# scheck-k/ste-gan

Measured on NVIDIA B200. Metric: GAN train samples/s, higher is better.
Workload: dtype bf16

## Files before the change

### include/stegan_b200.h

```cpp
#ifndef STEGAN_B200_H_
#define STEGAN_B200_H_

#include <stdint.h>

#ifdef __cplusplus
extern "C" {
#endif

typedef void* stg_stream_t;

enum { STG_F32 = 0, STG_BF16 = 1 };
enum { STG_ACT_NONE = 0, STG_ACT_RELU = 1, STG_ACT_LEAKY = 2, STG_ACT_TANH = 3 };
enum {
  STG_OK = 0,
  STG_EINVAL = -1,
  STG_ECUDA = -2,
  STG_EUNSUPPORTED = -3
};
enum { STG_ENGINE_AUTO = 0, STG_ENGINE_SIMT = 1, STG_ENGINE_TCGEN05 = 2, STG_ENGINE_MATVEC = 3  };

#define STG_MAX_TAPS 48

typedef struct StgConv {
  int32_t dtype;
  int32_t engine;
  int32_t n_samples;
  int32_t phases;
  int32_t t_src;
  int32_t t_dst;
  int32_t c_src;
  int32_t c_dst;
  int32_t groups;
  int32_t k, dilation, stride, pad;
  int32_t transposed;
  int32_t pair_sum;
  int32_t post_shift;
  int32_t mask_mode;
  int32_t act;
  int32_t dup_rows;
  int32_t out_f32;
  int32_t w_fwd_pack;
  const void* src;
  const void* w;
  const float* bias;
  const void* add_pre;
  const void* mask;
  const void* add_post;
  void* y_raw;
  void* y_act;
} StgConv;

int stg_conv(const StgConv* d, stg_stream_t stream);

int stg_conv_masked(const StgConv* d, const int32_t* valid_units, int32_t rows_per_unit, stg_stream_t stream);

typedef struct StgWgrad {
  int32_t dtype, engine;
  int32_t n_samples, phases, t_in, t_out, c_in, c_out, groups, k, dilation, stride, pad;
  const void* x;
  const void* dy;
  float* dw;
  float* dbias;
} StgWgrad;

int stg_conv_wgrad(const StgWgrad* d, stg_stream_t stream);
int stg_wgrad_layout(const StgWgrad* d, int* ld, int* span);

enum { STG_PACK_UNFOLD = 1 };
int stg_weightnorm_fold(const float* v, const float* g, int c_out, int cin_g, int k, int groups, int pack_groups,
                        int flags, int dtype, void* wf, void* wd, float* scale, stg_stream_t stream);
int stg_weightnorm_fold_bwd(const float* dw, int dw_ld, int dw_span, const float* v, const float* g, int c_out, int cin_g,
                            int k, int groups, float* dv, float* dg, int accumulate, stg_stream_t stream);

int stg_spectralnorm_fold(const float* w_orig, float* u, float* v, int c_out, int cin_g, int k, int groups,
                          int pack_groups, int flags, int training, int dtype, void* wf, void* wd, float* sigma_out,
                          float* scratch, float* u_used, float* v_used, stg_stream_t stream);
int stg_spectralnorm_fold_bwd(const float* dw, int dw_ld, int dw_span, const float* w_orig, const float* u, const float* v,
                              const float* sigma, int c_out, int cin_g, int k, int groups, float* dw_orig, int accumulate,
                              float* scratch, stg_stream_t stream);
typedef struct StgFoldItem {
  const float* v;
  const float* g;
  void* wf;
  void* wd;
  float* scale;
  const float* dw;
  float* dv;
  float* dg;
  int32_t c_out, cin_g, k, groups, pg, flags, dw_ld, dw_span;
  int32_t row0, tile0;
} StgFoldItem;
int stg_weightnorm_fold_multi(const StgFoldItem* items, int n_items, int total_rows, int total_tiles, int dtype,
                              stg_stream_t stream);
int stg_weightnorm_fold_bwd_multi(const StgFoldItem* items, int n_items, int total_rows, int accumulate,
                                  stg_stream_t stream);
int stg_weightnorm_fold_bwd_range(const StgFoldItem* items, int n_items, int row_base, int n_rows, int accumulate,
                                  stg_stream_t stream);

int stg_tc_pack_groups(int c_in, int c_out, int groups);

int stg_unfold(const void* src, int dtype, int B, int phases, int t_src, int t_dst, int C, int k, int dilation, int stride,
               int pad, void* out, stg_stream_t stream);
int stg_unfold_bwd(const void* dout, int dtype, int B, int phases, int t_src, int t_dst, int C, int k, int dilation,
                   int stride, int pad, float* dsrc, stg_stream_t stream);

int stg_period_first_layer(const float* x, const void* wf, const float* bias, int B, int T, int C, int period, int c_out,
                           int k, int stride, int pad, float slope, void* y, stg_stream_t stream);

int stg_embed_concat(const float* units, const float* emb, const int64_t* ids, int B, int T, int d_units, int d_emb,
                     int dtype, void* x0, stg_stream_t stream);
int stg_embed_concat_bwd(const void* dx0, const int64_t* ids, int B, int T, int d_units, int d_emb, int dtype,
                         float* demb, stg_stream_t stream);

int stg_reflect_pad_right(const float* x, int B, int T, int C, int T_pad, int dtype, void* out, stg_stream_t stream);
int stg_reflect_pad_right_bwd(const void* dout, int B, int T, int C, int T_pad, int dtype, float* dx, stg_stream_t stream);
int stg_avgpool4(const float* x, int B, int T, int C, float* out, stg_stream_t stream);
int stg_avgpool4_bwd(const float* dout, int B, int T, int C, float* dx, stg_stream_t stream);
int stg_cast(const void* src, int src_dtype, void* dst, int dst_dtype, int64_t n, stg_stream_t stream);
int stg_act_bwd(const float* dy, const float* y, int mode, int64_t n, int dtype, void* out, stg_stream_t stream);
int stg_relu_rows(const void* src, int dtype, int64_t rows, int C, int dup, void* out, stg_stream_t stream);
int stg_pair_sum_rows(const void* in, int64_t rows_out, int C, int dtype, void* out, stg_stream_t stream);
int stg_axpy_f32(float* y, const void* x, int x_dtype, float alpha, int64_t n, stg_stream_t stream);

int stg_td_loss(const float* x_real, const float* x_gen, int B, int T, int C, float* losses, const float* grad_scale,
                float* dx_gen, float* scratch, stg_stream_t stream);
int stg_td_loss_ex(const float* x_real, const float* x_gen, int B, int T, int C, int n_res, const int* wins,
                   const int* shifts, int pad_windows, int avg_window, float* losses, const float* grad_scale,
                   const float* grad_scale_dev, float* dx_gen, float* scratch, stg_stream_t stream);
int stg_td_features(const float* x, int B, int T, int C, int win, int shift, int pad_windows, int avg_window,
                    float* feats, float* scratch, stg_stream_t stream);
int stg_frame_stats(const float* x, int B, int T, int C, int win, int shift, int pad_windows, float* mean, float* power,
                    stg_stream_t stream);
int stg_window_signal(const float* x, int B, int T, int C, int win, int shift, int pad_windows, float* out,
                      stg_stream_t stream);
int stg_average_filter(const float* x, int64_t rows, int T, int window, int pad, float* out, stg_stream_t stream);

// ... 64 lines not shown
```

### ste_gan_b200/_lib.py

```python
from __future__ import annotations

import ctypes as C
import os

_HERE = os.path.dirname(os.path.abspath(__file__))
LIB_PATH = os.path.join(_HERE, "libstegan_b200.so")

F32, BF16 = 0, 1
ACT_NONE, ACT_RELU, ACT_LEAKY, ACT_TANH = 0, 1, 2, 3
ENGINE_AUTO, ENGINE_SIMT, ENGINE_TCGEN05 = 0, 1, 2
PACK_UNFOLD = 1
MAX_TAPS = 48


class StgConv(C.Structure):
    _fields_ = [(n, C.c_int32) for n in (
        "dtype", "engine", "n_samples", "phases", "t_src", "t_dst", "c_src", "c_dst", "groups", "k", "dilation",
        "stride", "pad", "transposed", "pair_sum", "post_shift", "mask_mode", "act", "dup_rows", "out_f32", "w_fwd_pack")] + [
        (n, C.c_void_p) for n in ("src", "w", "bias", "add_pre", "mask", "add_post", "y_raw", "y_act")]


class StgWgrad(C.Structure):
    _fields_ = [(n, C.c_int32) for n in (
        "dtype", "engine", "n_samples", "phases", "t_in", "t_out", "c_in", "c_out", "groups", "k", "dilation",
        "stride", "pad")] + [(n, C.c_void_p) for n in ("x", "dy", "dw", "dbias")]


class StgFoldItem(C.Structure):
    _fields_ = [(n, C.c_void_p) for n in ("v", "g", "wf", "wd", "scale", "dw", "dv", "dg")] + [
        (n, C.c_int32) for n in ("c_out", "cin_g", "k", "groups", "pg", "flags", "dw_ld", "dw_span", "row0", "tile0")]


class StgL1Item(C.Structure):
    _fields_ = [("a", C.c_void_p), ("b", C.c_void_p), ("da", C.c_void_p), ("n", C.c_int64)]


class StgMseItem(C.Structure):
    _fields_ = [("x", C.c_void_p), ("dx", C.c_void_p), ("n", C.c_int64), ("target", C.c_float), ("slot", C.c_int32)]


MAX_LOSS_ITEMS = 32
_P, _I, _L, _F = C.c_void_p, C.c_int, C.c_int64, C.c_float
_SIGS = {
    "stg_conv": [C.POINTER(StgConv), _P],
    "stg_conv_masked": [C.POINTER(StgConv), _P, C.c_int32, _P],
    "stg_conv_wgrad": [C.POINTER(StgWgrad), _P],
    "stg_conv_tc_supported": [C.POINTER(StgConv)],
    "stg_conv_route": [C.POINTER(StgConv)],
    "stg_wgrad_route": [C.POINTER(StgWgrad)],
    "stg_wgrad_tc_supported": [C.POINTER(StgWgrad)],
    "stg_weightnorm_fold": [_P, _P, _I, _I, _I, _I, _I, _I, _I, _P, _P, _P, _P],
    "stg_weightnorm_fold_bwd": [_P, _I, _I, _P, _P, _I, _I, _I, _I, _P, _P, _I, _P],
    "stg_wgrad_layout": [C.POINTER(StgWgrad), C.POINTER(C.c_int), C.POINTER(C.c_int)],
    "stg_spectralnorm_fold": [_P, _P, _P, _I, _I, _I, _I, _I, _I, _I, _I, _P, _P, _P, _P, _P, _P, _P],
    "stg_spectralnorm_fold_bwd": [_P, _I, _I, _P, _P, _P, _P, _I, _I, _I, _I, _P, _I, _P, _P],
    "stg_tc_pack_groups": [_I, _I, _I],
    "stg_l1_mean_multi": [_P, _I, _I, _P, _F, _P],
    "stg_mse_const_multi": [_P, _I, _I, _I, _P, _F, _P],
    "stg_weightnorm_fold_multi": [_P, _I, _I, _I, _I, _P],
    "stg_weightnorm_fold_bwd_multi": [_P, _I, _I, _I, _P],
    "stg_weightnorm_fold_bwd_range": [_P, _I, _I, _I, _I, _P],
    "stg_debug_set_trace": [_P],
    "stg_debug_rowshift": [_P, _P, _I, _I, _I, _P, _P],
    "stg_debug_row_classes": [_I, _P],
    "stg_debug_group_mma": [_P, _P, _I, _I, _P, _P],
    "stg_debug_conv_plan": [_P, _P],
    "stg_debug_tma_bw": [_P, C.c_longlong, _I, _I, _I, _I, _I, _P, _P],
    "stg_unfold": [_P, _I, _I, _I, _I, _I, _I, _I, _I, _I, _I, _P, _P],
    "stg_unfold_bwd": [_P, _I, _I, _I, _I, _I, _I, _I, _I, _I, _I, _P, _P],
    "stg_period_first_layer": [_P, _P, _P, _I, _I, _I, _I, _I, _I, _I, _I, C.c_float, _P, _P],
    "stg_embed_concat": [_P, _P, _P, _I, _I, _I, _I, _I, _P, _P],
    "stg_embed_concat_bwd": [_P, _P, _I, _I, _I, _I, _I, _P, _P],
    "stg_reflect_pad_right": [_P, _I, _I, _I, _I, _I, _P, _P],
    "stg_reflect_pad_right_bwd": [_P, _I, _I, _I, _I, _I, _P, _P],
    "stg_avgpool4": [_P, _I, _I, _I, _P, _P],
    "stg_avgpool4_bwd": [_P, _I, _I, _I, _P, _P],
    "stg_cast": [_P, _I, _P, _I, _L, _P],
    "stg_act_bwd": [_P, _P, _I, _L, _I, _P, _P],
    "stg_pair_sum_rows": [_P, _L, _I, _I, _P, _P],
    "stg_relu_rows": [_P, _I, _L, _I, _I, _P, _P],
    "stg_axpy_f32": [_P, _P, _I, _F, _L, _P],
    "stg_td_loss": [_P, _P, _I, _I, _I, _P, C.POINTER(C.c_float), _P, _P, _P],
    "stg_td_loss_ex": [_P, _P, _I, _I, _I, _I, C.POINTER(C.c_int), C.POINTER(C.c_int), _I, _I, _P, C.POINTER(C.c_float), _P, _P, _P, _P],
    "stg_td_features": [_P, _I, _I, _I, _I, _I, _I, _I, _P, _P, _P],
    "stg_frame_stats": [_P, _I, _I, _I, _I, _I, _I, _P, _P, _P],
    "stg_window_signal": [_P, _I, _I, _I, _I, _I, _I, _P, _P],
    "stg_average_filter": [_P, _L, _I, _I, _I, _P, _P],
    "stg_mse_const": [_P, _I, _L, _F, _P, _F, _P, _I, _P],
    "stg_l1_mean": [_P, _P, _I, _L, _P, _F, _P, _P],
    "stg_layernorm_fwd": [_P, _I, _P, _P, _I, _I, _F, _P, _P, _P],
    "stg_layernorm_bwd": [_P, _P, _I, _P, _P, _I, _I, _P, _P],
    "stg_relattn_fwd": [_P, _I, _P, _I, _I, _I, _I, _I, _F, _P, _P, _P],
    "stg_relattn_bwd": [_P, _I, _P, _P, _P, _I, _I, _I, _I, _I, _F, _P, _P],
    "stg_relattn_dense_supported": [_I, _I, _I],
    "stg_relattn_band_fwd": [_P, _I, _P, _I, _I, _I, _I, _I, _F, _P, _P, _P],
    "stg_relattn_band_bwd": [_P, _I, _P, _P, _P, _I, _I, _I, _I, _I, _F, _P, _P, _P],
    "stg_relattn_fwd_masked": [_P, _I, _P, _I, _I, _I, _I, _I, _F, _P, _P, _P, _P],
    "stg_relattn_band_fwd_masked": [_P, _I, _P, _I, _I, _I, _I, _I, _F, _P, _P, _P, _P],
    "stg_encoder_losses": [_P, _P, _P, _P, _I, _I, _I, _P, _F, _F, _P, _P, _I, _P],
    "stg_encoder_scores": [_P, _P, _P, _P, _P, _I, _I, _I, _I, _I, _P, _P, _P],
    "stg_adamw": [_P, _P, _P, _P, _L, _F, _P, _F, _F, _F, _F, _P, _F, _P, _I, _P],
}
EXPORTS = sorted(list(_SIGS) + ["stg_strerror", "stg_last_cuda_error", "stg_version", "stg_launch_count", "stg_set_sm_limit",
                                   "stg_debug_ingest_bytes"])

_lib = None


class StgError(RuntimeError):
    pass


def load(build_if_missing: bool = True):
    global _lib
    if _lib is not None:
        return _lib
    if not os.path.exists(LIB_PATH):
        if not build_if_missing:
            raise StgError(f"{LIB_PATH} is missing; run `python -m ste_gan_b200.build`")
        from . import build as _b
        _b.build()
    import torch
    lib = C.CDLL(LIB_PATH, mode=C.RTLD_GLOBAL)
    for name, argtypes in _SIGS.items():
        fn = getattr(lib, name)
        fn.argtypes = argtypes
        fn.restype = C.c_int
    lib.stg_strerror.argtypes = [C.c_int]
# ... 23 lines not shown
```

### ste_gan_b200/csrc/api.cu

```cuda
#include <stdlib.h>
#include <string.h>

#include <string>

#include "common.cuh"

namespace stg {

static thread_local std::string g_last_error;
unsigned long long g_launch_count = 0;
double g_ingest_bytes = 0.0;
int g_sm_limit = getenv("STG_SM_LIMIT") ? atoi(getenv("STG_SM_LIMIT")) : 0;

void set_cuda_error(cudaError_t e, const char* where) {
  g_last_error = std::string(cudaGetErrorName(e)) + ": " + cudaGetErrorString(e) + " at " + where;
}

int colsum(const void* dy, int dtype, int64_t rows, int C, float* out, cudaStream_t s);

static int validate_conv(const StgConv* d) {
  if (!d || !d->src || !d->w) return STG_EINVAL;
  if (d->dtype != STG_F32 && d->dtype != STG_BF16) return STG_EINVAL;
  if (d->n_samples < 1 || d->phases < 1 || d->t_src < 1 || d->t_dst < 1) return STG_EINVAL;
  if (d->groups < 1 || d->c_src % d->groups || d->c_dst % d->groups) return STG_EINVAL;
  if (d->k < 1 || d->dilation < 1 || d->stride < 1 || d->pad < 0) return STG_EINVAL;
  if (d->post_shift < 0 || d->post_shift > 1) return STG_EINVAL;
  if (d->dup_rows && d->pair_sum) return STG_EINVAL;
  if (!d->y_raw && !d->y_act) return STG_EINVAL;
  if (d->w_fwd_pack && !d->transposed) return STG_EINVAL;
  return STG_OK;
}

}

using namespace stg;

extern "C" int stg_conv(const StgConv* d, stg_stream_t stream) {
  int r = validate_conv(d);
  if (r) return r;
  cudaStream_t s = static_cast<cudaStream_t>(stream);
  switch (d->engine) {
    case STG_ENGINE_SIMT: return d->w_fwd_pack ? STG_EUNSUPPORTED : conv_simt(d, s);
    case STG_ENGINE_TCGEN05: return conv_tc(d, s);
    case STG_ENGINE_AUTO:
      if (conv_c1_supported(d)) return conv_c1(d, s);
      if (conv_tc_supported(d)) return conv_tc(d, s);
      return d->w_fwd_pack ? STG_EUNSUPPORTED : conv_simt(d, s);
    default: return STG_EINVAL;
  }
}

extern "C" int stg_conv_masked(const StgConv* d, const int32_t* valid_units, int32_t rows_per_unit, stg_stream_t stream) {
  int r = validate_conv(d);
  if (r) return r;
  if (!valid_units || rows_per_unit < 1 || d->transposed || d->pair_sum || d->phases != 1) return STG_EINVAL;
  cudaStream_t s = static_cast<cudaStream_t>(stream);
  switch (d->engine) {
    case STG_ENGINE_SIMT: return conv_simt(d, s, valid_units, rows_per_unit);
    case STG_ENGINE_TCGEN05: return conv_tc(d, s, valid_units, rows_per_unit);
    case STG_ENGINE_AUTO:
      return conv_tc_supported(d) ? conv_tc(d, s, valid_units, rows_per_unit) : conv_simt(d, s, valid_units, rows_per_unit);
    default: return STG_EINVAL;
  }
}

extern "C" int stg_conv_route(const StgConv* d) {
  if (!d || validate_conv(d) != STG_OK) return STG_EINVAL;
  if (d->engine == STG_ENGINE_SIMT) return STG_ENGINE_SIMT;
  if (d->engine == STG_ENGINE_TCGEN05) return STG_ENGINE_TCGEN05;
  if (conv_c1_supported(d)) return STG_ENGINE_MATVEC;
  return conv_tc_supported(d) ? STG_ENGINE_TCGEN05 : STG_ENGINE_SIMT;
}
extern "C" int stg_wgrad_route(const StgWgrad* d) {
  if (!d) return STG_EINVAL;
  if (d->engine == STG_ENGINE_SIMT) return STG_ENGINE_SIMT;
  if (d->engine == STG_ENGINE_TCGEN05) return STG_ENGINE_TCGEN05;
  if (wgrad_c1_supported(d)) return STG_ENGINE_MATVEC;
  return wgrad_tc_supported(d) ? STG_ENGINE_TCGEN05 : STG_ENGINE_SIMT;
}
extern "C" int stg_conv_tc_supported(const StgConv* d) { return (d && validate_conv(d) == STG_OK && conv_tc_supported(d)) ? 1 : 0; }
extern "C" int stg_tc_pack_groups(int c_in, int c_out, int groups) {
  if (groups < 1 || c_in % groups || c_out % groups) return groups;
  return tc_pack_groups(c_in, c_out, groups);
}
extern "C" int stg_wgrad_tc_supported(const StgWgrad* d) { return (d && wgrad_tc_supported(d)) ? 1 : 0; }

extern "C" int stg_conv_wgrad(const StgWgrad* d, stg_stream_t stream) {
  if (!d || !d->x || !d->dy) return STG_EINVAL;
  if (d->dtype != STG_F32 && d->dtype != STG_BF16) return STG_EINVAL;
  if (d->groups < 1 || d->c_in % d->groups || d->c_out % d->groups) return STG_EINVAL;
  cudaStream_t s = static_cast<cudaStream_t>(stream);
  int r = STG_OK;
  if (d->dw) {
    if (d->engine == STG_ENGINE_AUTO && wgrad_c1_supported(d)) return wgrad_c1(d, s);
    if (d->engine == STG_ENGINE_TCGEN05) return wgrad_tc(d, s);
    if (d->engine == STG_ENGINE_AUTO && wgrad_tc_supported(d)) return wgrad_tc(d, s);
    if (d->engine == STG_ENGINE_AUTO || d->engine == STG_ENGINE_SIMT) r = wgrad_simt(d, s);
    else r = STG_EINVAL;
    if (r) return r;
  }
  if (d->dbias) r = colsum(d->dy, d->dtype, (int64_t)d->n_samples * d->phases * d->t_out, d->c_out, d->dbias, s);
  return r;
}

extern "C" int stg_wgrad_layout(const StgWgrad* d, int* ld, int* span) {
  if (!d || !ld || !span || d->groups < 1 || d->c_in % d->groups) return STG_EINVAL;
  const bool tc = d->engine == STG_ENGINE_TCGEN05 ||
                  (d->engine == STG_ENGINE_AUTO && !wgrad_c1_supported(d) && wgrad_tc_supported(d));
  if (tc) { wgrad_tc_layout(d, ld, span); return STG_OK; }
  *span = d->c_in / d->groups;
  *ld = d->k * *span;
  return STG_OK;
}

extern "C" const char* stg_strerror(int code) {
  switch (code) {
    case STG_OK: return "ok";
    case STG_EINVAL: return "invalid argument or unsupported shape";
    case STG_ECUDA: return "CUDA error";
    case STG_EUNSUPPORTED: return "shape not supported by the requested engine";
    default: return "unknown error";
  }
}
extern "C" const char* stg_last_cuda_error(void) { return g_last_error.c_str(); }
extern "C" int stg_version(void) { return 100; }
extern "C" unsigned long long stg_launch_count(void) { return g_launch_count; }
extern "C" void stg_set_sm_limit(int n) { g_sm_limit = n > 0 ? n : 0; }
extern "C" double stg_debug_ingest_bytes(int reset) { const double v = g_ingest_bytes; if (reset) g_ingest_bytes = 0.0; return v; }

extern "C" int stg_debug_conv_plan(const StgConv* d, int* out) {
  if (!out) return STG_EINVAL;
  const int r = validate_conv(d);
  if (r != STG_OK) return r;
  return conv_tc_plan(d, out);
}

extern "C" int stg_debug_set_trace(void* buf) { conv_tc_set_trace(static_cast<long long*>(buf)); return STG_OK; }
```

### ste_gan_b200/csrc/common.cuh

```cuda
#pragma once
#include <cuda_bf16.h>
#include <cuda_runtime.h>
#include <stdint.h>

#include "../../include/stegan_b200.h"

namespace stg {

void set_cuda_error(cudaError_t e, const char* where);

#define STG_CUDA_CHECK(expr)                                   \
  do {                                                         \
    cudaError_t _e = (expr);                                   \
    if (_e != cudaSuccess) {                                   \
      ::stg::set_cuda_error(_e, #expr);                        \
      return STG_ECUDA;                                        \
    }                                                          \
  } while (0)

extern unsigned long long g_launch_count;
extern double g_ingest_bytes;
extern int g_sm_limit;
#define STG_LAUNCH_CHECK()                 \
  do {                                     \
    ++::stg::g_launch_count;               \
    STG_CUDA_CHECK(cudaGetLastError());    \
  } while (0)

using bf16 = __nv_bfloat16;

__device__ __forceinline__ float to_f(float v) { return v; }
__device__ __forceinline__ float to_f(bf16 v) { return __bfloat162float(v); }
template <typename T> __device__ __forceinline__ T from_f(float v);
template <> __device__ __forceinline__ float from_f<float>(float v) { return v; }
template <> __device__ __forceinline__ bf16 from_f<bf16>(float v) { return __float2bfloat16_rn(v); }

__device__ __forceinline__ void ld4(const float* p, float (&o)[4]) {
  float4 v = *reinterpret_cast<const float4*>(p);
  o[0] = v.x; o[1] = v.y; o[2] = v.z; o[3] = v.w;
}
__device__ __forceinline__ void ld4(const bf16* p, float (&o)[4]) {
  uint2 v = *reinterpret_cast<const uint2*>(p);
  __nv_bfloat162 a = *reinterpret_cast<__nv_bfloat162*>(&v.x);
  __nv_bfloat162 b = *reinterpret_cast<__nv_bfloat162*>(&v.y);
  o[0] = __low2float(a); o[1] = __high2float(a); o[2] = __low2float(b); o[3] = __high2float(b);
}
__device__ __forceinline__ void st4(float* p, const float (&v)[4]) {
  *reinterpret_cast<float4*>(p) = make_float4(v[0], v[1], v[2], v[3]);
}
__device__ __forceinline__ void st4(bf16* p, const float (&v)[4]) {
  __nv_bfloat162 a = __floats2bfloat162_rn(v[0], v[1]);
  __nv_bfloat162 b = __floats2bfloat162_rn(v[2], v[3]);
  uint2 u;
  u.x = *reinterpret_cast<uint32_t*>(&a);
  u.y = *reinterpret_cast<uint32_t*>(&b);
  *reinterpret_cast<uint2*>(p) = u;
}

__device__ __forceinline__ float act_apply(int act, float v) {
  switch (act) {
    case STG_ACT_RELU: return v > 0.f ? v : 0.f;
    case STG_ACT_LEAKY: return v > 0.f ? v : 0.1f * v;
    case STG_ACT_TANH: return tanhf(v);
    default: return v;
  }
}
__device__ __forceinline__ float act_grad_from_output(int mode, float m) {
  switch (mode) {
    case STG_ACT_RELU: return m > 0.f ? 1.f : 0.f;
    case STG_ACT_LEAKY: return m > 0.f ? 1.f : 0.1f;
    case STG_ACT_TANH: return 1.f - m * m;
    default: return 1.f;
  }
}

__device__ __forceinline__ float warp_sum(float v) {
#pragma unroll
  for (int o = 16; o > 0; o >>= 1) v += __shfl_xor_sync(0xffffffffu, v, o);
  return v;
}
__device__ __forceinline__ float block_sum(float v, float* red) {
  const int lane = threadIdx.x & 31, warp = threadIdx.x >> 5, nw = (blockDim.x + 31) >> 5;
  v = warp_sum(v);
  __syncthreads();
  if (lane == 0) red[warp] = v;
  __syncthreads();
  float r = (lane < nw) ? red[lane] : 0.f;
  r = warp_sum(r);
  return r;
}

static inline int64_t ceil_div64(int64_t a, int64_t b) { return (a + b - 1) / b; }
static inline int ceil_div(int a, int b) { return (a + b - 1) / b; }

int conv_simt(const StgConv* d, cudaStream_t s, const int32_t* valid_units = nullptr, int rows_per_unit = 1);
int conv_tc(const StgConv* d, cudaStream_t s, const int32_t* valid_units = nullptr, int rows_per_unit = 1);
int conv_tc_plan(const StgConv* d, int* out);
bool conv_tc_supported(const StgConv* d);
int wgrad_simt(const StgWgrad* d, cudaStream_t s);
int wgrad_tc(const StgWgrad* d, cudaStream_t s);
bool wgrad_tc_supported(const StgWgrad* d);
int tc_pack_groups(int c_in, int c_out, int groups);
bool conv_c1_supported(const StgConv* d);
int conv_c1(const StgConv* d, cudaStream_t s);
bool wgrad_c1_supported(const StgWgrad* d);
int wgrad_c1(const StgWgrad* d, cudaStream_t s);
void conv_tc_set_trace(long long* buf);
void wgrad_tc_layout(const StgWgrad* d, int* ld, int* span);

}
```

### ste_gan_b200/csrc/conv_tc.cu

```cuda
#include <stdio.h>
#include <stdlib.h>
#include <string.h>

#include "tc_common.cuh"

namespace stg {

namespace {

using namespace tc;

constexpr int TM = 128;
constexpr int KC = 64;
constexpr int MAX_STAGES = 8;
constexpr int ACC_COLS = 256;
constexpr int SUB = 32;
constexpr int SLOT = TM * SUB * 2;
constexpr int MAX_RES = 8;

struct TcEpi {
  int rows, c_dst, post_shift, mask_mode, act, dup_rows, out_f32, pair_sum;
  int n_in, n_out, has_pre, has_mask, has_post, has_raw, has_act;
  int in_sh;
  float act_slope, mask_slope;
// ... 140 lines not shown
  x.col0 = tn * p.bn;
  x.ch0 = (x.col0 / p.cd_g) * p.cs_g;
  x.wcol0 = x.col0 % p.cd_g;
  x.g0 = p.res_gfirst[x.res];
  x.n_iters = (p.res_gfirst[x.res + 1] - x.g0) * p.k_chunks;
  return x;
}
__device__ __forceinline__ int out_row(const TcP& p, const Tile& x, int m) {
  if (m >= p.mrows || x.b >= p.n_samples) return -1;
  const int hl = m / p.pack, ph = m - hl * p.pack;
  const int h = (x.h0 + hl) * p.n_res + x.res;
  return h < p.t_dst ? h * p.phases + ph : -1;
}

__device__ __forceinline__ bool row_kept(const TcEpi& e, int b, int row) {
  return (int64_t)row < (int64_t)max(e.valid_units[b], 0) * e.rows_per_unit;
}

struct EpiIn {
  float pre[16], mk[16], post[16];
};
__device__ __forceinline__ void epi_load(const TcEpi& e, int b, int row, int col, bool row_ok, EpiIn& in) {
  if (!row_ok || col >= e.c_dst) return;
  const int ncols = min(16, e.c_dst - col);
  const bool vec = (ncols == 16) && ((e.c_dst & 7) == 0);
  const int64_t off = ((int64_t)b * e.rows + row) * e.c_dst + col;
  if (e.add_pre) {
    if (vec) ld16(e.add_pre + off, in.pre); else for (int i = 0; i < 16; ++i) in.pre[i] = i < ncols ? to_f(e.add_pre[off + i]) : 0.f;
  }
  if (e.mask) {
    if (vec) ld16(e.mask + off, in.mk); else for (int i = 0; i < 16; ++i) in.mk[i] = i < ncols ? to_f(e.mask[off + i]) : 0.f;
  }
  if (e.add_post) {
    const int64_t o2 = ((int64_t)b * (e.rows >> e.post_shift) + (row >> e.post_shift)) * e.c_dst + col;
    if (vec) ld16(e.add_post + o2, in.post); else for (int i = 0; i < 16; ++i) in.post[i] = i < ncols ? to_f(e.add_post[o2 + i]) : 0.f;
  }
}
__device__ __forceinline__ void epi_store(const TcEpi& e, int b, int row, int col, float (&v)[16], const EpiIn& in, bool keep) {
  const int64_t off = ((int64_t)b * e.rows + row) * e.c_dst + col;
  const int ncols = min(16, e.c_dst - col);
  const bool vec = (ncols == 16) && ((e.c_dst & 7) == 0);
  if (e.add_pre) {
#pragma unroll
    for (int i = 0; i < 16; ++i) v[i] += in.pre[i];
  }
  if (e.mask) {
#pragma unroll
    for (int i = 0; i < 16; ++i) v[i] *= dact_fast(e, in.mk[i]);
  }
  if (e.add_post) {
#pragma unroll
    for (int i = 0; i < 16; ++i) v[i] += in.post[i];
  }
  if (!keep) {
#pragma unroll
    for (int i = 0; i < 16; ++i) v[i] = 0.f;
  }
  if (e.y_raw) {
    if (e.out_f32) {
      float* p = static_cast<float*>(e.y_raw) + off;
      if (vec) st16f(p, v); else for (int i = 0; i < ncols; ++i) p[i] = v[i];
    } else {
      bf16* p = static_cast<bf16*>(e.y_raw) + off;
      if (vec) st16(p, v); else for (int i = 0; i < ncols; ++i) p[i] = __float2bfloat16_rn(v[i]);
    }
  }
  if (e.y_act) {
    float a[16];
#pragma unroll
    for (int i = 0; i < 16; ++i) a[i] = act_fast(e, v[i]);
    const int64_t o0 = e.dup_rows ? ((int64_t)b * 2 * e.rows + 2 * row) * e.c_dst + col : off;
    if (e.out_f32) {
      float* p0 = static_cast<float*>(e.y_act) + o0;
      if (vec) st16f(p0, a); else for (int i = 0; i < ncols; ++i) p0[i] = a[i];
      if (e.dup_rows) { float* p1 = p0 + e.c_dst; if (vec) st16f(p1, a); else for (int i = 0; i < ncols; ++i) p1[i] = a[i]; }
    } else {
      bf16* p0 = static_cast<bf16*>(e.y_act) + o0;
      if (vec) st16(p0, a); else for (int i = 0; i < ncols; ++i) p0[i] = __float2bfloat16_rn(a[i]);
      if (e.dup_rows) { bf16* p1 = p0 + e.c_dst; if (vec) st16(p1, a); else for (int i = 0; i < ncols; ++i) p1[i] = __float2bfloat16_rn(a[i]); }
    }
  }
}

template <bool kStaged, bool kPair, bool kMask>
__global__ void __launch_bounds__(kStaged ? 384 : 352, (kStaged && !kPair) ? 2 : 1)
conv_tc_kernel(const __grid_constant__ TmA4 tmA4, const __grid_constant__ CUtensorMap tmW,
               const __grid_constant__ EpiMaps em, const TcP p) {
  constexpr int EPI_WARPS = 8;
  extern __shared__ uint8_t smem_raw[];
  const uint32_t smem_base = (smem_u32(smem_raw) + 1023u) & ~1023u;
  const int b_bytes = p.cu_k ? p.cu_fpc * p.cu_n * p.cu_k * 2 : (kPair ? p.bn / 2 : p.bn) * KC * 2;
  const int stage_bytes = p.a_bytes + p.max_ntaps * b_bytes;
  const TcEpi& e = p.e;
  const int rank = kPair ? __shfl_sync(0xffffffffu, (int)cluster_ctarank(), 0) : 0;
  const int tile0 = kPair ? (int)(blockIdx.x >> 1) : (int)blockIdx.x;
  const int tstep = kPair ? (int)(gridDim.x >> 1) : (int)gridDim.x;
  const uint32_t epi_base = smem_base + p.stages * stage_bytes;
  const uint32_t bias_base = epi_base + (kStaged ? ((e.n_in << e.in_sh) + p.out_ring * e.n_out) * SLOT : 0);
  const uint32_t bar_base = bias_base + (kStaged ? 2048 : 0);
  auto full_bar = [&](int s) { return bar_base + 8u * s; };
  auto empty_bar = [&](int s) { return bar_base + 8u * (MAX_STAGES + s); };
  auto tmem_full_bar = [&](int a) { return bar_base + 8u * (2 * MAX_STAGES + a); };
  auto tmem_empty_bar = [&](int a) { return bar_base + 8u * (2 * MAX_STAGES + 2 + a); };
  const uint32_t tmem_slot = bar_base + 8u * (2 * MAX_STAGES + 4);
  auto in_bar = [&](int a) { return bar_base + 8u * (2 * MAX_STAGES + 6 + a); };

  const int warp = __shfl_sync(0xffffffffu, (int)(threadIdx.x >> 5), 0), lane = threadIdx.x & 31;

  life_ev(p.trace, 30);
  pdl_trigger();
  if (warp == 0 && lane == 0) {
    for (int c = 0; c < p.n_cls; ++c) prefetch_tmap(&tmA4.m[c]);
    prefetch_tmap(&tmW);
    for (int s = 0; s < p.stages; ++s) { mbar_init(full_bar(s), 1); mbar_init(empty_bar(s), 1); }
    for (int a = 0; a < 2; ++a) { mbar_init(tmem_full_bar(a), 1); mbar_init(tmem_empty_bar(a), kPair ? 2 * EPI_WARPS : EPI_WARPS); }
    for (int a = 0; a < 8; ++a) mbar_init(in_bar(a), 1);
    fence_barrier_init();
  }
  if (warp == 1) {
    if constexpr (kPair) { tmem_alloc_2sm(tmem_slot, (uint32_t)p.tmem_cols); tmem_relinquish_2sm(); }
    else { tmem_alloc(tmem_slot, (uint32_t)p.tmem_cols); tmem_relinquish(); }
  }
  tc_fence_before();
  if constexpr (kPair) cluster_sync_all();
  else __syncthreads();
  tc_fence_after();
  life_ev(p.trace, 31);
  pdl_wait();
  life_ev(p.trace, 32);
  uint32_t tmem_base;
  asm volatile("ld.shared.b32 %0, [%1];" : "=r"(tmem_base) : "r"(tmem_slot));
  const uint32_t lead_bars = kPair ? mapa_u32(bar_base, 0) : bar_base;
  auto lead_full_bar = [&](int s) { return lead_bars + 8u * s; };
  auto lead_tmem_empty_bar = [&](int a) { return lead_bars + 8u * (2 * MAX_STAGES + 2 + a); };
  auto arrive_tmem_empty = [&](int a) {
    if constexpr (kPair) mbar_arrive_cluster(lead_tmem_empty_bar(a)); else mbar_arrive(tmem_empty_bar(a));
  };

  constexpr int WPROD = kStaged ? 11 : 10;
  if ((warp == 0 || warp == WPROD) && p.max_ntaps == 1) {
    const bool do_a = warp == 0;
    const bool lead = lane == 0;
    Tracer trc(lead && do_a ? p.trace : nullptr, 0);
    const uint32_t a_box_bytes = (uint32_t)(p.hb * p.pack * KC * 2);
    const uint32_t tx_bytes = (kPair ? 2u : 1u) * ((uint32_t)p.a_boxes * a_box_bytes + (uint32_t)b_bytes);
    const int row_step = p.hb * p.stride;
    int s = 0; uint32_t phs = 0;
#ifdef STG_PROF_LOOP
    long long prof[4] = {0, 0, 0, 0};
#endif
    for (int t = tile0; t < p.n_tiles; t += tstep) {
      const Tile x = decode_tile<kPair>(p, t, rank);
      trc.ev(1, t);
      const int n_groups = p.res_gfirst[x.res + 1] - x.g0;
      const int wc = p.b_mn == 0 ? x.col0 + (kPair ? rank * (p.bn / 2) : 0)
                   : p.b_mn == 2 ? x.wcol0 / 64 + (kPair ? rank * (p.bn / 128) : 0) : x.wcol0;
      for (int gi = 0; gi < n_groups; ++gi) {
        const int g = x.g0 + gi;
        const int row0 = x.h0 * p.stride + p.tt.g_off[g];
        const int tap = p.tt.tap_w[g];
        for (int chunk = 0; chunk < p.k_chunks; ++chunk) {
#ifdef STG_PROF_LOOP
          const long long pc0 = clock64();
#endif
          mbar_wait(empty_bar(s), phs ^ 1);
          trc.ev(4, chunk);
#ifdef STG_PROF_LOOP
          const long long pc1 = clock64();
#endif
          const uint32_t a_dst = smem_base + (uint32_t)(s * stage_bytes);
          const uint32_t fb = kPair ? lead_full_bar(s) : full_bar(s);
          const int c0 = x.ch0 + chunk * KC;
          if (do_a) {
            if (rank == 0) mbar_expect_tx_el(full_bar(s), tx_bytes);
#pragma unroll 1
            for (int bx = 0; bx < p.a_boxes; ++bx)
              tma_load_4d_el<kPair>(a_dst + bx * a_box_bytes, &tmA4.m[x.cls], fb, c0, 0, row0 + bx * row_step, x.b);
          }
#ifdef STG_PROF_LOOP
          const long long pc2 = clock64();
#endif
          if (do_a) {
          } else if (p.cu_k) {
            tma_load_3d_el<kPair>(a_dst + p.a_bytes, &tmW, fb, 0, x.col0 + chunk * p.cu_fpc * p.cu_n, tap);
          } else if (p.b_mn == 0) {
            tma_load_3d_el<kPair>(a_dst + p.a_bytes, &tmW, fb, chunk * KC, wc, tap);
          } else if (p.b_mn == 2) {
            tma_load_4d_el<kPair>(a_dst + p.a_bytes, &tmW, fb, 0, c0, wc, tap);
          } else {
#pragma unroll 1
            for (int nb = 0; nb < p.bn / 64; ++nb)
              tma_load_3d_el<kPair>(a_dst + p.a_bytes + nb * 8192, &tmW, fb, wc + nb * 64, c0, tap);
          }
          if (++s == p.stages) { s = 0; phs ^= 1u; }
#ifdef STG_PROF_LOOP
          const long long pc3 = clock64();
          prof[0] += pc1 - pc0; prof[1] += pc2 - pc1; prof[2] += pc3 - pc2; prof[3] += 1;
#endif
        }
      }
    }
#ifdef STG_PROF_LOOP
    if (lead && do_a && p.trace && blockIdx.x == 0) for (int i = 0; i < 4; ++i) p.trace[1 + 3 * 5200 + i] = prof[i];
#endif
  } else if (warp == 1 && p.max_ntaps == 1) {
    const bool lead = lane == 0;
    const uint32_t idesc = idesc_bf16_f32(kPair ? 2 * TM : TM, p.bn, 0, p.b_mn ? 1 : 0);
    const uint32_t idesc_u = idesc_bf16_f32(TM, p.cu_k ? p.cu_n : p.bn, 0, 0);
    const int cu_ks = p.cu_k == 16 ? 0 : (p.cu_k == 32 ? 1 : 2), cu_km = (1 << cu_ks) - 1;
    const uint64_t cu_bhi = smem_desc_kmajor_narrow(0, p.cu_k ? p.cu_k * 2 : 128);
    const int cu_bq = (p.cu_n * p.cu_k * 2) >> 4;
    Tracer trc(lead ? p.trace : nullptr, 1);
    const uint64_t adesc0 = smem_desc_kmajor_sw128(smem_base);
    const uint64_t bdesc0 = p.b_mn ? smem_desc_mnmajor_sw128(smem_base + p.a_bytes, 8192, 1024) : smem_desc_kmajor_sw128(smem_base + p.a_bytes);
    const uint32_t dstep = (uint32_t)stage_bytes >> 4;
    const uint32_t bstep = p.b_mn ? 128u : 2u;
    int s = 0, acc_i = 0; uint32_t phs = 0;
#ifdef STG_PROF_LOOP
    long long mprof[3] = {0, 0, 0};
#endif
    for (int t = tile0; t < p.n_tiles && rank == 0; t += tstep) {
      const Tile x = decode_tile<kPair>(p, t, rank);
      if (x.n_iters == 0) continue;
      const int as = acc_i & 1, aph = (acc_i >> 1) & 1;
      mbar_wait(tmem_empty_bar(as), aph ^ 1);
      tc_fence_after();
      trc.ev(2, t);
      const uint32_t d_tmem = tmem_base + (uint32_t)(as * p.acc_cols);
      int cu_chunk = 0;
      for (int it = 0; it < x.n_iters; ++it) {
#ifdef STG_PROF_LOOP
        const long long mc0 = clock64();
#endif
        mbar_wait(full_bar(s), phs);
        tc_fence_after();
        trc.ev(5, it);
#ifdef STG_PROF_LOOP
        const long long mc1 = clock64();
#endif
        const uint64_t ad = adesc0 + (uint64_t)((uint32_t)s * dstep), bd = bdesc0 + (uint64_t)((uint32_t)s * dstep);
        if (p.cu_k) {
          const uint32_t dcol = d_tmem + (uint32_t)(cu_chunk * p.cu_fpc * p.cu_n);
          if (++cu_chunk == p.k_chunks) cu_chunk = 0;
          const uint64_t bu = cu_bhi | (uint64_t)(((smem_base + (uint32_t)(s * stage_bytes) + (uint32_t)p.a_bytes) >> 4) & 0x3FFFu);
          const uint32_t acc0 = it >= p.k_chunks ? 1u : 0u;
#pragma unroll
          for (int i = 0; i < KC / 16; ++i) {
            const int q = i >> cu_ks, ks = i & cu_km;
            umma_bf16_el<kPair>(dcol + (uint32_t)(q * p.cu_n), ad + 2 * i, bu + (uint64_t)(q * cu_bq + 2 * ks), idesc_u, (acc0 | (uint32_t)(ks > 0)));
          }
        } else {
#pragma unroll
          for (int ks = 0; ks < KC / 16; ++ks)
            umma_bf16_el<kPair>(d_tmem, ad + 2 * ks, bd + bstep * ks, idesc, (it > 0 || ks > 0) ? 1u : 0u);
        }
        umma_commit_el<kPair>(empty_bar(s));
        if (it == x.n_iters - 1) umma_commit_el<kPair>(tmem_full_bar(as));
        if (++s == p.stages) { s = 0; phs ^= 1u; }
#ifdef STG_PROF_LOOP
        const long long mc2 = clock64();
        mprof[0] += mc1 - mc0; mprof[1] += mc2 - mc1; mprof[2] += 1;
#endif
      }
      trc.ev(3, t);
      ++acc_i;
    }
#ifdef STG_PROF_LOOP
    if (lead && p.trace && blockIdx.x == 0) for (int i = 0; i < 3; ++i) p.trace[1 + 3 * 5200 + 8 + i] = mprof[i];
#endif
  } else if (warp == 0 || warp == WPROD) {
    const bool do_a = warp == 0;
    int s = 0; uint32_t phs = 0;
    for (int t = tile0; t < p.n_tiles; t += tstep) {
      const Tile x = decode_tile<kPair>(p, t, rank);
      const int n_groups = p.res_gfirst[x.res + 1] - x.g0;
      for (int gi = 0; gi < n_groups; ++gi) {
       const int g = x.g0 + gi;
       const int nt = p.tt.g_ntaps[g], t0 = p.tt.g_tfirst[g];
       for (int chunk = 0; chunk < p.k_chunks; ++chunk) {
        mbar_wait(empty_bar(s), phs ^ 1);
        const uint32_t a_dst = smem_base + s * stage_bytes;
        if (do_a) {
          mbar_expect_tx_el(full_bar(s), (uint32_t)(p.a_boxes * p.hb * p.pack * KC * 2 + nt * b_bytes));
#pragma unroll 1
          for (int bx = 0; bx < p.a_boxes; ++bx)
            tma_load_4d_el(a_dst + bx * p.hb * p.pack * KC * 2, &tmA4.m[0], full_bar(s), x.ch0 + chunk * KC, 0,
                           (x.h0 + bx * p.hb) * p.stride + p.tt.g_off[g], x.b);
        }
#pragma unroll 1
        for (int tl = 0; tl < (do_a ? 0 : nt); ++tl) {
          if (p.cu_k) {
            tma_load_3d_el(a_dst + p.a_bytes + tl * b_bytes, &tmW, full_bar(s), 0, x.col0 + chunk * p.cu_fpc * p.cu_n,
                           p.tt.tap_w[t0 + tl]);
          } else if (!p.b_mn) {
            tma_load_3d_el(a_dst + p.a_bytes + tl * b_bytes, &tmW, full_bar(s), chunk * KC, x.col0, p.tt.tap_w[t0 + tl]);
          } else if (p.b_mn == 2) {
            tma_load_4d_el(a_dst + p.a_bytes + tl * b_bytes, &tmW, full_bar(s), 0, x.ch0 + chunk * KC, x.wcol0 / 64,
                           p.tt.tap_w[t0 + tl]);
          } else {
#pragma unroll 1
            for (int nb = 0; nb < p.bn / 64; ++nb)
              tma_load_3d_el(a_dst + p.a_bytes + tl * b_bytes + nb * 8192, &tmW, full_bar(s), x.wcol0 + nb * 64,
                             x.ch0 + chunk * KC, p.tt.tap_w[t0 + tl]);
          }
        }
        if (++s == p.stages) { s = 0; phs ^= 1u; }
       }
      }
    }
  } else if (warp == 1) {
    const uint32_t idesc = idesc_bf16_f32(TM, p.bn, 0, p.b_mn ? 1 : 0);
    const uint32_t idesc_u = idesc_bf16_f32(TM, p.cu_k ? p.cu_n : p.bn, 0, 0);
    const int cu_ks = p.cu_k == 16 ? 0 : (p.cu_k == 32 ? 1 : 2), cu_km = (1 << cu_ks) - 1;
    const uint64_t cu_bhi = smem_desc_kmajor_narrow(0, p.cu_k ? p.cu_k * 2 : 128);
    const int cu_bq = (p.cu_n * p.cu_k * 2) >> 4;
    int s = 0, acc_i = 0; uint32_t phs = 0;
    for (int t = tile0; t < p.n_tiles; t += tstep) {
      const Tile x = decode_tile<kPair>(p, t, rank);
      if (x.n_iters == 0) continue;
      const int as = acc_i & 1, aph = (acc_i >> 1) & 1;
      mbar_wait(tmem_empty_bar(as), aph ^ 1);
      tc_fence_after();
      const uint32_t d_tmem = tmem_base + (uint32_t)(as * p.acc_cols);
      int g = x.g0, chunk = 0;
      for (int it = 0; it < x.n_iters; ++it) {
        const int nt = p.tt.g_ntaps[g], t0 = p.tt.g_tfirst[g];
        mbar_wait(full_bar(s), phs);
        tc_fence_after();
        const uint32_t a_addr = smem_base + s * stage_bytes;
#pragma unroll 1
        for (int tl = 0; tl < nt; ++tl) {
          const uint64_t adesc = smem_desc_kmajor_sw128(a_addr + (uint32_t)(p.tt.tap_shift[t0 + tl] * p.pack * KC * 2));
          const uint32_t b_addr = a_addr + p.a_bytes + tl * b_bytes;
          if (p.cu_k) {
            const uint32_t dcol = d_tmem + (uint32_t)(chunk * p.cu_fpc * p.cu_n);
            const uint64_t bu = cu_bhi | (uint64_t)((b_addr >> 4) & 0x3FFFu);
            const uint32_t acc0 = (it >= p.k_chunks || tl > 0) ? 1u : 0u;
#pragma unroll
            for (int i = 0; i < KC / 16; ++i) {
              const int q = i >> cu_ks, ks = i & cu_km;
              umma_bf16_el(dcol + (uint32_t)(q * p.cu_n), adesc + 2 * i, bu + (uint64_t)(q * cu_bq + 2 * ks), idesc_u, (acc0 | (uint32_t)(ks > 0)));
            }
            continue;
          }
          const uint64_t bdesc = p.b_mn ? smem_desc_mnmajor_sw128(b_addr, 8192, 1024) : smem_desc_kmajor_sw128(b_addr);
          const uint64_t bstep = p.b_mn ? 128 : 2;
#pragma unroll
          for (int ks = 0; ks < KC / 16; ++ks)
            umma_bf16_el(d_tmem, adesc + 2 * ks, bdesc + bstep * ks, idesc, (it > 0 || tl > 0 || ks > 0) ? 1u : 0u);
        }
        umma_commit_el(empty_bar(s));
        if (it == x.n_iters - 1) umma_commit_el(tmem_full_bar(as));
        if (++s == p.stages) { s = 0; phs ^= 1u; }
        if (++chunk == p.k_chunks) { chunk = 0; ++g; }
      }
      ++acc_i;
    }
  } else if constexpr (kStaged) {
    const int n_sub = p.bn / SUB;
    const int in_mask = (1 << e.in_sh) - 1;
    auto ring = [&](int q) { return p.out_ring == 2 ? (q & 1) : q % 3; };
    auto in_slot = [&](int buf, int i) { return epi_base + (uint32_t)((buf * e.n_in + i) * SLOT); };
    auto out_slot = [&](int buf, int o) { return epi_base + (uint32_t)(((e.n_in << e.in_sh) + buf * e.n_out + o) * SLOT); };
    auto bar_full = [&](int b3) { return 2 + b3; };
    auto bar_free = [&](int b3) { return 5 + b3; };
    const int my_tiles = (p.n_tiles - tile0 + tstep - 1) / tstep;
    const int q_total = my_tiles * n_sub;
    if (warp == 10) {
      if (lane == 0) {
// ... 173 lines not shown
#pragma unroll
              for (int i = 0; i < 32; ++i) v[i] = fmaxf(v[i], e.act_slope * v[i]);
#pragma unroll
              for (int j = 0; j < 4; ++j) sts128(sl + sw64(r_in, j), pack8(&v[8 * j]));
            }
          }
          fence_proxy_async();
          asm volatile("bar.arrive %0, 160;" ::"r"(bar_full(obuf)) : "memory");
          trc.ev(12, s);
        }
        qbase += n_sub;
        if (x.n_iters > 0) ++acc_i;
      }
    }
  } else {
    const int ew = warp - 2;
    const int sub = warp & 3;
    const int half = ew >> 2;
    const int n_chunks = p.bn / 16;
    const int c_lo = (half == 0) ? 0 : (n_chunks + 1) / 2, c_hi = (half == 0) ? (n_chunks + 1) / 2 : n_chunks;
    int acc_i = 0;
    for (int t = tile0; t < p.n_tiles; t += tstep) {
      const Tile x = decode_tile<kPair>(p, t, rank);
      const int as = acc_i & 1, aph = (acc_i >> 1) & 1;
      const int arow = out_row(p, x, sub * 32 + lane);
      const bool row_ok = arow >= 0 && (!e.pair_sum || (lane & 1) == 0);
      const int orow = e.pair_sum ? (arow >> 1) : arow;
      const bool keep = !kMask || (row_ok && row_kept(e, x.b, orow));
      EpiIn inA, inB;
      if (c_lo < c_hi) epi_load(e, x.b, orow, x.col0 + c_lo * 16, row_ok, inA);
      if (x.n_iters > 0) {
        mbar_wait(tmem_full_bar(as), aph);
        tc_fence_after();
      }
      const uint32_t t_addr = tmem_base + ((uint32_t)(sub * 32) << 16) + (uint32_t)(as * p.acc_cols);
      auto process = [&](int c, const EpiIn& in) {
        float v[16];
        if (x.n_iters > 0) {
          tmem_ld16(t_addr + (uint32_t)(c * 16), v);
        } else {
#pragma unroll
          for (int i = 0; i < 16; ++i) v[i] = 0.f;
        }
        const int col = x.col0 + c * 16;
        if (col >= e.c_dst) return;
        if (e.bias) {
#pragma unroll
          for (int i = 0; i < 16; ++i) v[i] += (col + i < e.c_dst) ? e.bias[col + i] : 0.f;
        }
        if (e.pair_sum) {
#pragma unroll
          for (int i = 0; i < 16; ++i) v[i] += __shfl_xor_sync(0xffffffffu, v[i], 1);
        }
        if (row_ok) epi_store(e, x.b, orow, col, v, in, keep);
      };
#pragma unroll 1
      for (int c = c_lo; c < c_hi; c += 2) {
        if (c + 1 < c_hi) epi_load(e, x.b, orow, x.col0 + (c + 1) * 16, row_ok, inB);
        process(c, inA);
        if (c + 1 < c_hi) {
          if (c + 2 < c_hi) epi_load(e, x.b, orow, x.col0 + (c + 2) * 16, row_ok, inA);
          process(c + 1, inB);
        }
      }
      if (x.n_iters > 0) {
        tc_fence_before();
        __syncwarp();
        if (lane == 0) arrive_tmem_empty(as);
        ++acc_i;
      }
    }
  }
  tc_fence_before();
  if constexpr (kPair) {
    cluster_sync_all();
    if (warp == 1) tmem_dealloc_2sm(tmem_base, (uint32_t)p.tmem_cols);
  } else {
    __syncthreads();
    if (warp == 1) tmem_dealloc(tmem_base, (uint32_t)p.tmem_cols);
  }
  life_ev(p.trace, 33);
}

}

PFN_encodeTiled get_encode_tiled() {
  static PFN_encodeTiled fn = nullptr;
  if (!fn) {
    void* ptr = nullptr;
    cudaDriverEntryPointQueryResult q;
    if (cudaGetDriverEntryPoint("cuTensorMapEncodeTiled", &ptr, cudaEnableDefault, &q) == cudaSuccess &&
        q == cudaDriverEntryPointSuccess)
      fn = reinterpret_cast<PFN_encodeTiled>(ptr);
  }
  return fn;
}

int make_tmap_bf16(CUtensorMap* out, const void* base, int rank, const uint64_t* dims, const uint64_t* strides_bytes,
                   const uint32_t* box, const uint32_t* elem_strides, int swizzle_bytes) {
  PFN_encodeTiled enc = get_encode_tiled();
  if (!enc) { set_cuda_error(cudaErrorNotSupported, "cuTensorMapEncodeTiled entry point"); return STG_ECUDA; }
  cuuint64_t gd[5]; cuuint64_t gs[4]; cuuint32_t bx[5]; cuuint32_t es[5];
  for (int i = 0; i < rank; ++i) { gd[i] = dims[i]; bx[i] = box[i]; es[i] = elem_strides ? elem_strides[i] : 1; }
  for (int i = 0; i + 1 < rank; ++i) gs[i] = strides_bytes[i];
  const CUtensorMapSwizzle sw = swizzle_bytes == 32 ? CU_TENSOR_MAP_SWIZZLE_32B
                              : swizzle_bytes == 64 ? CU_TENSOR_MAP_SWIZZLE_64B : CU_TENSOR_MAP_SWIZZLE_128B;
  CUresult r = enc(out, CU_TENSOR_MAP_DATA_TYPE_BFLOAT16, (cuuint32_t)rank, const_cast<void*>(base), gd, gs, bx, es,
                   CU_TENSOR_MAP_INTERLEAVE_NONE, sw, CU_TENSOR_MAP_L2_PROMOTION_L2_256B,
                   CU_TENSOR_MAP_FLOAT_OOB_FILL_NONE);
  if (r != CUDA_SUCCESS) {
    set_cuda_error(cudaErrorInvalidValue, "cuTensorMapEncodeTiled failed");
    return STG_ECUDA;
  }
  return STG_OK;
}

static int sm_count() {
  static int n = 0;
  if (!n) {
    int dev = 0;
    if (cudaGetDevice(&dev) != cudaSuccess || cudaDeviceGetAttribute(&n, cudaDevAttrMultiProcessorCount, dev) != cudaSuccess || n < 1)
      n = 148;
  }
  return (g_sm_limit > 0 && g_sm_limit < n) ? g_sm_limit : n;
}

static int pick_bn_model(int cd_g, int groups, int64_t row_tiles, int n_stages, int step) {
  static const double feed = getenv("STG_BN_FEED") ? atof(getenv("STG_BN_FEED")) : 0.0;
  static const double alpha = getenv("STG_BN_ALPHA") ? atof(getenv("STG_BN_ALPHA")) : 0.0;
  int best = 0;
  double best_t = 0;
  for (int bn = 256; bn >= step; bn -= step) {
    if (cd_g % bn) continue;
    const int64_t tiles = row_tiles * (cd_g / bn) * groups;
    const double waves = (double)((tiles + sm_count() - 1) / sm_count());
    double mma = 2.0 * bn > 200.0 ? 2.0 * bn : 200.0;
    if (feed > 0.0) { const double ld = (TM * KC * 2 + bn * KC * 2) / feed; if (ld > mma) mma = ld; }
    const double stage = mma + 60.0;
    const double epi = (bn / 32.0) * 200.0;
    const double makespan = waves * n_stages * stage + epi;
    const double smtime = (double)tiles * (n_stages * stage + epi) / sm_count();
    const double t = alpha * smtime + (1.0 - alpha) * makespan;
    if (best == 0 || t < best_t * 0.999) { best = bn; best_t = t; }
  }
  return best;
}
static bool bn_model_on() {
  static const bool on = !(getenv("STG_BN_MODEL") && atoi(getenv("STG_BN_MODEL")) == 0);
  return on;
}

static int pick_bn(int cd_g, int groups, int64_t row_tiles, int n_stages) {
  if (groups == 1 && (cd_g % 16) != 0) return cd_g <= 16 ? 16 : (cd_g <= 128 ? ((cd_g + 15) / 16) * 16 : 128);
  static const int env_bn = getenv("STG_BN") ? atoi(getenv("STG_BN")) : 0;
  static const int min_tiles = getenv("STG_MIN_TILES") ? atoi(getenv("STG_MIN_TILES")) : 128;
  if (env_bn > 0 && cd_g % env_bn == 0) return env_bn;
  if (bn_model_on()) {
    const int b = pick_bn_model(cd_g, groups, row_tiles, n_stages, 32);
    if (b > 0) return b;
  }
  int best = 0;
  for (int bn = 256; bn >= 16; bn -= 16) {
    if (cd_g % bn) continue;
    if (best != 0 && bn < 128) break;
    best = bn;
    if (row_tiles * (cd_g / bn) * groups >= min_tiles) break;
// ... 45 lines not shown
  *n_res = (d->transposed && d->stride > 1) ? d->stride : 1;
  *tiles_m = ceil_div(ceil_div(d->t_dst, *n_res), *nh);
}

static int compact_merge(int ku, int nu, int groups) {
  if ((ku != 16 && ku != 32 && ku != 64) || (nu % 16) != 0) return 0;
  for (int f = 1; f <= groups; ++f) {
    if (groups % f) continue;
    if ((ku * f) % KC == 0 && (nu * f) % KC == 0) return nu * f <= 256 ? f : 0;
  }
  return 0;
}

bool conv_tc_supported(const StgConv* d) {
  if (d->dtype != STG_BF16) return false;
  if (d->k > STG_MAX_TAPS || d->k < 1) return false;
  if ((d->c_src % 8) != 0) return false;
  if (d->phases > 64) return false;
  if (d->groups > 1) {
    if (((d->c_dst / d->groups) % 16) != 0) return false;
    if ((d->c_src / d->groups) % KC) {
      if (d->transposed && d->w_fwd_pack) return false;
      if (compact_merge(d->c_src / d->groups, d->c_dst / d->groups, d->groups) == 0) return false;
    } else if (d->transposed && !d->w_fwd_pack && d->c_src / d->groups != KC) {
      return false;
    }
  }
  if (d->transposed && !d->w_fwd_pack && d->groups == 1) return false;
  if (d->transposed && ((d->c_dst / d->groups) % 8) != 0) return false;
  if (d->transposed && d->w_fwd_pack && d->groups > 1 && ((d->c_dst / d->groups) % 64) != 0) return false;
  if (d->transposed && d->stride > MAX_RES) return false;
  if (d->transposed && d->stride > 1 && d->pair_sum) return false;
  if (!d->transposed && d->stride > 4) return false;
  if (!d->transposed && d->stride > 2 && d->phases > 1 && (TM / d->phases) * d->stride > 256) return false;
  if ((d->pair_sum || d->dup_rows || d->post_shift) && d->phases != 1) return false;
  if (d->pair_sum && (d->t_dst & 1)) return false;
  if (d->add_pre == nullptr && d->mask == nullptr && d->add_post == nullptr && d->y_raw == nullptr && d->y_act == nullptr)
    return false;
  return true;
}

int tc_pack_groups(int c_in, int c_out, int groups) {
  if (groups <= 1) return 1;
  const int cin_g = c_in / groups, cout_g = c_out / groups;
  auto side_ok = [](int c) { return c == 16 || c == 32 || (c % KC) == 0; };
  static const int env_legacy = getenv("STG_GROUP_MERGE") ? atoi(getenv("STG_GROUP_MERGE")) : 0;
  for (int m = 1; m <= groups && !env_legacy; ++m) {
    if (groups % m) continue;
    if (side_ok(cin_g * m) && side_ok(cout_g * m)) return groups / m;
  }
  for (int f = 1; f <= groups; ++f) {
    if (groups % f) continue;
    if ((cin_g * f) % KC == 0 && (cout_g * f) % KC == 0) return groups / f;
  }
  return groups;
}

static int epi_map(CUtensorMap* m, const void* base, int C, int P, int T, int B, int res, int n_res, int pack, int box_h,
                   bool dup, int box_b = 1) {
  if (dup) {
    const uint64_t dims[4] = {(uint64_t)C, 2, (uint64_t)T, (uint64_t)B};
    const uint64_t strides[3] = {(uint64_t)C * 2, (uint64_t)C * 4, (uint64_t)T * C * 4};
    const uint32_t box[4] = {SUB, 1, (uint32_t)box_h, (uint32_t)box_b};
    return make_tmap_bf16(m, base, 4, dims, strides, box, nullptr, 64);
  }
  const int h_ext = (T - res + n_res - 1) / n_res;
  const uint64_t dims[4] = {(uint64_t)C, (uint64_t)P, (uint64_t)h_ext, (uint64_t)B};
  const uint64_t strides[3] = {(uint64_t)C * 2, (uint64_t)n_res * P * C * 2, (uint64_t)T * P * C * 2};
  const uint32_t box[4] = {SUB, (uint32_t)pack, (uint32_t)box_h, (uint32_t)box_b};
  const bf16* b0 = static_cast<const bf16*>(base) + (int64_t)res * P * C;
  return make_tmap_bf16(m, b0, 4, dims, strides, box, nullptr, 64);
}

static long long* g_trace = nullptr;
void conv_tc_set_trace(long long* buf) { g_trace = buf; }
static int* g_plan_out = nullptr;
int conv_tc_plan(const StgConv* d, int* out) {
  g_plan_out = out;
  const int r = conv_tc(d, nullptr);
  g_plan_out = nullptr;
  return r;
}

int conv_tc(const StgConv* d, cudaStream_t s, const int32_t* valid_units, int rows_per_unit) {
  if (!conv_tc_supported(d)) return STG_EUNSUPPORTED;
  TcP p;
  p.trace = g_trace;
  p.phases = d->phases; p.t_dst = d->t_dst; p.stride = d->transposed ? 1 : d->stride;
  p.cs_g = d->c_src / d->groups; p.cd_g = d->c_dst / d->groups;
  int tile_groups = d->groups;
  p.cu_k = p.cu_n = p.cu_fpc = 0;
  if (d->groups > 1 && (p.cs_g % KC) != 0) {
    const int f = compact_merge(p.cs_g, p.cd_g, d->groups);
    if (f == 0) return STG_EUNSUPPORTED;
    p.cu_k = p.cs_g; p.cu_n = p.cd_g; p.cu_fpc = KC / p.cs_g;
    p.cs_g *= f; p.cd_g *= f; tile_groups = d->groups / f;
  }
  p.k_chunks = ceil_div(p.cs_g, KC);
  tile_geometry(d, &p.pack, &p.nh, &p.n_res, &p.tiles_m);
  p.mrows = p.nh * p.pack;
  p.b_mn = (d->transposed && d->w_fwd_pack) ? 1 : 0;
  const int n_stages_est = ceil_div(d->k, p.n_res) * p.k_chunks;
  p.bn = p.cu_k ? p.cd_g
       : p.b_mn ? pick_bn_mn(p.cd_g, tile_groups, (int64_t)d->n_samples * p.n_res * p.tiles_m, n_stages_est)
                : pick_bn(p.cd_g, tile_groups, (int64_t)d->n_samples * p.n_res * p.tiles_m, n_stages_est);
  if (p.bn <= 0) return STG_EUNSUPPORTED;
  p.tmem_cols = 512;
  struct Tap { int off, w; };
  Tap taps[MAX_RES][STG_MAX_TAPS]; int ntap[MAX_RES];
  if (p.n_res > 1) {
    for (int r = 0; r < p.n_res; ++r) {
      ntap[r] = 0;
      for (int j = 0; j < d->k; ++j) {
        const int num = r + d->pad - j * d->dilation;
        if (((num % d->stride) + d->stride) % d->stride != 0) continue;
        taps[r][ntap[r]++] = Tap{(num >= 0) ? num / d->stride : -((-num) / d->stride), j};
      }
    }
  } else {
    ntap[0] = d->k;
    for (int j = 0; j < d->k; ++j) taps[0][j] = Tap{d->transposed ? (d->pad - j * d->dilation) : (j * d->dilation - d->pad), j};
  }
  TcEpi& e = p.e;
  const int rows_per_phase = d->pair_sum ? d->t_dst / 2 : d->t_dst;
  e.rows = rows_per_phase * d->phases; e.c_dst = d->c_dst;
  e.post_shift = d->post_shift; e.mask_mode = d->mask_mode; e.act = d->act; e.dup_rows = d->dup_rows;
  e.out_f32 = d->out_f32; e.pair_sum = d->pair_sum; e.bias = d->bias;
  e.add_pre = static_cast<const bf16*>(d->add_pre); e.mask = static_cast<const bf16*>(d->mask);
  e.add_post = static_cast<const bf16*>(d->add_post); e.y_raw = d->y_raw; e.y_act = d->y_act;
  e.has_pre = d->add_pre != nullptr; e.has_mask = d->mask != nullptr; e.has_post = d->add_post != nullptr;
  e.has_raw = d->y_raw != nullptr; e.has_act = d->y_act != nullptr;
  e.valid_units = valid_units; e.rows_per_unit = rows_per_unit;
  e.n_in = e.has_pre + e.has_mask + e.has_post; e.n_out = e.has_raw + e.has_act;
  e.act_slope = d->act == STG_ACT_RELU ? 0.f : (d->act == STG_ACT_LEAKY ? 0.1f : 1.f);
  e.mask_slope = d->mask_mode == STG_ACT_RELU ? 0.f : (d->mask_mode == STG_ACT_LEAKY ? 0.1f : 1.f);
  const bool staged = !d->out_f32 && d->act != STG_ACT_TANH && d->mask_mode != STG_ACT_TANH && (d->c_dst % 8) == 0 &&
                      p.n_res <= MAX_STAGED_RES && (p.n_res == 1 || (!d->add_post && !d->y_act)) && (p.bn % SUB) == 0 &&
                      (!d->post_shift || (rows_per_phase % 2) == 0);

  RowCls rc[4];
  int n_rc = 0;
  int64_t cls_tiles = 0;
  static const int env_cls = getenv("STG_ROWCLS") ? atoi(getenv("STG_ROWCLS")) : 1;
  if (env_cls && staged && d->phases == 1 && p.n_res == 1 && d->stride == 1) {
    n_rc = row_classes(d->t_dst, rc);
    for (int c = 0; c < n_rc; ++c)
      cls_tiles += rc[c].tps > 0 ? (int64_t)d->n_samples * rc[c].tps : ceil_div(d->n_samples, TM / rc[c].seg);
    const int64_t classic = (int64_t)d->n_samples * p.tiles_m;
    if (n_rc < 2 || cls_tiles >= classic) n_rc = 0;
    if (n_rc) {
      const int bn2 = p.cu_k ? p.cd_g : p.b_mn ? pick_bn_mn(p.cd_g, tile_groups, cls_tiles, n_stages_est) : pick_bn(p.cd_g, tile_groups, cls_tiles, n_stages_est);
      if (bn2 > 0 && (bn2 % SUB) == 0) p.bn = bn2; else n_rc = 0;
    }
  }

  static const int env_pair = getenv("STG_PAIR") ? atoi(getenv("STG_PAIR")) : 0;
  p.n_samples = d->n_samples;
  const int n_mt = d->n_samples * p.tiles_m;
  bool pair = env_pair != 0 && p.cu_k == 0 && n_rc == 0 && n_mt >= 2 && (p.b_mn ? (p.cd_g % 64 == 0 && p.bn % 128 == 0) : (p.bn % 32 == 0));
  p.pairs_per_res = (n_mt + 1) / 2;
  int b_bytes = p.cu_k ? p.cu_fpc * p.cu_n * p.cu_k * 2 : (pair ? p.bn / 2 : p.bn) * KC * 2;
  static const int env_insh = getenv("STG_IN_DEPTH_SH") ? atoi(getenv("STG_IN_DEPTH_SH")) : -1;
  static const int smem_budget = (getenv("STG_SMEM_BUDGET_KB") ? atoi(getenv("STG_SMEM_BUDGET_KB")) : 224) * 1024;
  static const int win_min_stages = getenv("STG_WIN_MIN_STAGES") ? atoi(getenv("STG_WIN_MIN_STAGES")) : 3;
  e.in_sh = 1;
  if (staged && e.n_in > 0) {
    const int stage1 = TM * KC * 2 + (p.cu_k ? p.cu_fpc * p.cu_n * p.cu_k * 2 : p.bn * KC * 2);
    const int want = n_stages_est < 4 ? n_stages_est : 4;
    for (int sh = 3; sh >= 2; --sh) {
// ... 42 lines not shown
        }
        if (out) { out->tt.g_off[n_groups] = (short)lo; out->tt.g_tfirst[n_groups] = (unsigned char)(n_taps_out - nm); out->tt.g_ntaps[n_groups] = (unsigned char)nm; }
        ++n_groups;
      }
    }
    if (out) out->res_gfirst[p.n_res] = n_groups;
    const int win_h = p.nh + max_shift;
    int a_boxes = ceil_div(win_h * p.stride, 256), hb = ceil_div(win_h, a_boxes);
    if (a_boxes > 1) {
      const int align = 8 / (p.pack >= 8 ? 8 : (8 % p.pack == 0 ? p.pack : 1));
      hb = ceil_div(hb, align) * align;
      if ((hb * p.pack) % 8 != 0) return pl;
      while (hb * p.stride > 256) { ++a_boxes; hb = ceil_div(ceil_div(win_h, a_boxes), align) * align; }
    }
    if (hb * p.stride > 256 || p.pack > 256) return pl;
    int a_rows = a_boxes * hb * p.pack;
    if (a_rows < TM + max_shift * p.pack) a_rows = TM + max_shift * p.pack;
    pl.hb = hb; pl.a_boxes = a_boxes; pl.a_bytes = ceil_div(a_rows * KC * 2, 1024) * 1024; pl.n_groups = n_groups;
    const int stage_bytes = pl.a_bytes + ng * b_bytes;
    pl.stages = avail / stage_bytes;
    if (pl.stages > MAX_STAGES) pl.stages = MAX_STAGES;
    pl.traffic = (long long)n_groups * (a_boxes * hb * p.pack * KC * 2) + (long long)n_taps_out * b_bytes;
    pl.ok = pl.stages >= 2;
    return pl;
  };
  static const int env_ng = getenv("STG_NG") ? atoi(getenv("STG_NG")) : 0;
  Plan best{0, 0, 0, 0, 0, 0, 0, false};
  const long long base_traffic = build(1, nullptr).traffic;
  const int cands[] = {1, 2, 3, 4, 5, 6, 8, 10};
  for (int ci = 0; ci < 8; ++ci) {
    const int ng = cands[ci];
    if (env_ng > 0 && ng != env_ng && d->k >= env_ng) continue;
    if (ng > d->k && ng != 1) continue;
    Plan pl = build(ng, nullptr);
    if (!pl.ok) continue;
    if (!best.ok) { best = pl; continue; }
    if (pl.stages >= win_min_stages && pl.traffic * 100 <= base_traffic * 65 && pl.traffic < best.traffic) best = pl;
  }
  if (!best.ok) return STG_EUNSUPPORTED;
  if (pair && best.ng != 1) {
    pair = false;
    b_bytes = p.bn * KC * 2;
    best = Plan{0, 0, 0, 0, 0, 0, 0, false};
    for (int ci = 0; ci < 8; ++ci) {
      const int ng = cands[ci];
      if (env_ng > 0 && ng != env_ng && d->k >= env_ng) continue;
      if (ng > d->k && ng != 1) continue;
      Plan pl = build(ng, nullptr);
      if (!pl.ok) continue;
      if (!best.ok) { best = pl; continue; }
      if (pl.stages >= win_min_stages && pl.traffic * 100 <= base_traffic * 65 && pl.traffic < best.traffic) best = pl;
    }
    if (!best.ok) return STG_EUNSUPPORTED;
  }
  if (n_rc && best.ng != 1) n_rc = 0;
  p.n_cls = n_rc ? n_rc : 1;
  p.cls_mt0[0] = 0;
  for (int c = 0; c < p.n_cls; ++c) {
    p.cls_seg[c] = n_rc ? rc[c].seg : TM; p.cls_h0[c] = n_rc ? rc[c].h0 : 0; p.cls_tps[c] = n_rc ? rc[c].tps : p.tiles_m;
    p.cls_mt0[c + 1] = p.cls_mt0[c] + (n_rc ? (rc[c].tps > 0 ? d->n_samples * rc[c].tps : ceil_div(d->n_samples, TM / rc[c].seg)) : 0);
  }
  build(best.ng, &p);
  p.hb = best.hb; p.a_boxes = best.a_boxes; p.a_bytes = best.a_bytes; p.max_ntaps = best.ng; p.stages = best.stages;
  const int stage_bytes = p.a_bytes + p.max_ntaps * b_bytes;
  const size_t smem = (size_t)p.stages * stage_bytes + epi_bytes + 1024  + 8 * (2 * MAX_STAGES + 16) + sizeof(TapTables) + 16;
  static const bool dbg_plan = getenv("STG_DEBUG_PLAN") != nullptr;
  if (dbg_plan)
    fprintf(stderr, "[conv_tc] c %d->%d k%d s%d d%d g%d ph%d T %d->%d tr%d | bn %d staged %d ng %d stages %d hb %d a_boxes %d a_bytes %d "
            "groups %d tiles_m %d res %d smem %zu occ2 %d\n", d->c_src, d->c_dst, d->k, d->stride, d->dilation, d->groups, d->phases, d->t_src,
            d->t_dst, d->transposed, p.bn, (int)staged, p.max_ntaps, p.stages, p.hb, p.a_boxes, p.a_bytes, p.res_gfirst[p.n_res],
            p.tiles_m, p.n_res, smem, (int)occ2);
  if (g_plan_out) {
    const int tiles_n = ceil_div(d->c_dst, p.bn);
    const int64_t nt = pair ? (int64_t)p.n_res * p.pairs_per_res * tiles_n
                     : n_rc ? (int64_t)p.cls_mt0[p.n_cls] * tiles_n : (int64_t)d->n_samples * p.n_res * p.tiles_m * tiles_n;
    const int64_t slots = pair ? sm_count() / 2 : (occ2 ? 2 : 1) * sm_count();
    int* o = g_plan_out;
    o[0] = p.bn; o[1] = staged; o[2] = p.max_ntaps; o[3] = p.stages; o[4] = (int)smem; o[5] = occ2; o[6] = pair; o[7] = p.n_cls;
    o[8] = (int)nt; o[9] = (int)((nt < slots ? nt : slots) * (pair ? 2 : 1)); o[10] = p.cu_k; o[11] = p.k_chunks; o[12] = p.tmem_cols;
    o[13] = staged && e.n_in > 0 ? 1 << e.in_sh : 0; o[14] = p.out_ring; o[15] = p.n_res;
    return STG_OK;
  }

  CUtensorMap tmW;
  TmA4 tmA;
  EpiMaps em;
  memset(&em, 0, sizeof(em));
  memset(&tmA, 0, sizeof(tmA));
  for (int c = 0; c < p.n_cls; ++c) {
    const uint64_t C = d->c_src, P = d->phases, T = d->t_src, B = d->n_samples;
    const uint64_t dims[4] = {C, P, T, B};
    const uint64_t strides[3] = {C * 2, P * C * 2, T * P * C * 2};
    const uint32_t box_h = n_rc ? (uint32_t)rc[c].seg : (uint32_t)(p.hb * p.stride);
    const uint32_t box_b = n_rc && rc[c].tps == 0 ? (uint32_t)(TM / rc[c].seg) : 1u;
    const uint32_t box[4] = {(uint32_t)KC, (uint32_t)p.pack, box_h, box_b};
    const uint32_t es[4] = {1, 1, (uint32_t)p.stride, 1};
    int r = make_tmap_bf16(&tmA.m[c], d->src, 4, dims, strides, box, es);
    if (r) return r;
  }
  if (p.cu_k) {
    const uint64_t C = p.cu_k, N = d->c_dst, K = d->k;
    const uint64_t dims[3] = {C, N, K};
    const uint64_t strides[2] = {C * 2, N * C * 2};
    const uint32_t box[3] = {(uint32_t)p.cu_k, (uint32_t)(p.cu_fpc * p.cu_n), 1};
    int r = make_tmap_bf16(&tmW, d->w, 3, dims, strides, box, nullptr, p.cu_k * 2);
    if (r) return r;
  } else if (!p.b_mn) {
    const uint64_t C = p.cs_g, N = d->c_dst, K = d->k;
    const uint64_t dims[3] = {C, N, K};
    const uint64_t strides[2] = {C * 2, N * C * 2};
    const uint32_t box[3] = {(uint32_t)KC, (uint32_t)(pair ? p.bn / 2 : p.bn), 1};
    int r = make_tmap_bf16(&tmW, d->w, 3, dims, strides, box, nullptr);
    if (r) return r;
  } else if (p.cd_g % 64 == 0) {
    p.b_mn = 2;
    const uint64_t N = p.cd_g, R = d->c_src, K = d->k;
    const uint64_t dims[4] = {64, R, N / 64, K};
    const uint64_t strides[3] = {N * 2, 128, R * N * 2};
    const uint32_t box[4] = {64, (uint32_t)KC, (uint32_t)((pair ? p.bn / 2 : p.bn) / 64), 1};
    int r = make_tmap_bf16(&tmW, d->w, 4, dims, strides, box, nullptr);
    if (r) return r;
  } else {
    const uint64_t N = p.cd_g, R = d->c_src, K = d->k;
    const uint64_t dims[3] = {N, R, K};
    const uint64_t strides[2] = {N * 2, R * N * 2};
    const uint32_t box[3] = {64, (uint32_t)KC, 1};
    int r = make_tmap_bf16(&tmW, d->w, 3, dims, strides, box, nullptr);
    if (r) return r;
  }
  if (staged) {
    const int box_h = d->pair_sum ? 64 : p.nh;
    const int t_rows = rows_per_phase;
    int r = 0;
    for (int res = 0; res < (n_rc ? 0 : p.n_res); ++res) {
      if (e.has_pre) r |= epi_map(&em.pre[res], d->add_pre, d->c_dst, d->phases, t_rows, d->n_samples, res, p.n_res, p.pack, box_h, false);
      if (e.has_mask) r |= epi_map(&em.mask[res], d->mask, d->c_dst, d->phases, t_rows, d->n_samples, res, p.n_res, p.pack, box_h, false);
      if (e.has_raw) r |= epi_map(&em.raw[res], d->y_raw, d->c_dst, d->phases, t_rows, d->n_samples, res, p.n_res, p.pack, box_h, false);
    }
    if (!n_rc) {
      if (e.has_post) r |= epi_map(&em.post[0], d->add_post, d->c_dst, d->phases, t_rows >> d->post_shift, d->n_samples, 0, 1, p.pack, box_h >> d->post_shift, false);
      if (e.has_act) r |= epi_map(&em.act[0], d->y_act, d->c_dst, d->phases, t_rows, d->n_samples, 0, 1, p.pack, box_h, d->dup_rows != 0);
    }
    for (int c = 0; c < n_rc; ++c) {
      const int bh = d->pair_sum ? rc[c].seg / 2 : rc[c].seg, bb = rc[c].tps == 0 ? TM / rc[c].seg : 1;
      if (e.has_pre) r |= epi_map(&em.pre[c], d->add_pre, d->c_dst, 1, t_rows, d->n_samples, 0, 1, 1, bh, false, bb);
      if (e.has_mask) r |= epi_map(&em.mask[c], d->mask, d->c_dst, 1, t_rows, d->n_samples, 0, 1, 1, bh, false, bb);
      if (e.has_raw) r |= epi_map(&em.raw[c], d->y_raw, d->c_dst, 1, t_rows, d->n_samples, 0, 1, 1, bh, false, bb);
      if (e.has_post) r |= epi_map(&em.post[c], d->add_post, d->c_dst, 1, t_rows >> d->post_shift, d->n_samples, 0, 1, 1, bh >> d->post_shift, false, bb);
      if (e.has_act) r |= epi_map(&em.act[c], d->y_act, d->c_dst, 1, t_rows, d->n_samples, 0, 1, 1, bh, d->dup_rows != 0, bb);
    }
    if (r) return STG_ECUDA;
  }
  using Kernel = decltype(&conv_tc_kernel<true, false, false>);
  static const Kernel kernels[2][2][2] = {
      {{conv_tc_kernel<false, false, false>, conv_tc_kernel<false, false, true>},
       {conv_tc_kernel<true, false, false>, conv_tc_kernel<true, false, true>}},
      {{conv_tc_kernel<false, true, false>, conv_tc_kernel<false, true, true>},
       {conv_tc_kernel<true, true, false>, conv_tc_kernel<true, true, true>}}};
  static bool attr_set = false;
  if (!attr_set) {
    for (int i = 0; i < 8; ++i) {
      const Kernel k = kernels[i >> 2][(i >> 1) & 1][i & 1];
      STG_CUDA_CHECK(cudaFuncSetAttribute(k, cudaFuncAttributeMaxDynamicSharedMemorySize, 227 * 1024));
      if ((i >> 1) == 1)
        STG_CUDA_CHECK(cudaFuncSetAttribute(k, cudaFuncAttributePreferredSharedMemoryCarveout, cudaSharedmemCarveoutMaxShared));
    }
    attr_set = true;
  }
  const bool masked = valid_units != nullptr;
  p.tiles_n = ceil_div(d->c_dst, p.bn);
  if (pair) {
    const int64_t n_tiles = (int64_t)p.n_res * p.pairs_per_res * p.tiles_n;
    if (n_tiles > 0x7fffffff) return STG_EINVAL;
    p.n_tiles = (int)n_tiles;
    const int max_pairs = sm_count() / 2;
    const int n_pairs = p.n_tiles < max_pairs ? p.n_tiles : max_pairs;
    cudaLaunchConfig_t cfg = {};
    cfg.gridDim = dim3(2 * n_pairs); cfg.blockDim = dim3(staged ? 384 : 352); cfg.dynamicSmemBytes = smem; cfg.stream = s;
    cudaLaunchAttribute at[2];
    cfg.attrs = at; cfg.numAttrs = tc_launch_attrs(at, true);
    STG_CUDA_CHECK(cudaLaunchKernelEx(&cfg, kernels[1][staged][masked], tmA, tmW, em, p));
    STG_LAUNCH_CHECK();
    return STG_OK;
  }
  const int64_t n_tiles = n_rc ? (int64_t)p.cls_mt0[p.n_cls] * p.tiles_n : (int64_t)d->n_samples * p.n_res * p.tiles_m * p.tiles_n;
  if (n_tiles > 0x7fffffff) return STG_EINVAL;
  p.n_tiles = (int)n_tiles;
  g_ingest_bytes += (double)n_tiles * ((double)best.traffic * p.k_chunks / p.n_res + (staged ? (double)e.n_in * p.mrows * p.bn * 2 : 0.0));
  static const int env_cap = getenv("STG_GRID_CAP") ? atoi(getenv("STG_GRID_CAP")) : 0;
  const int slots = (occ2 ? 2 : 1) * sm_count();
  int grid = p.n_tiles < slots ? p.n_tiles : slots;
  if (env_cap > 0 && grid > env_cap) grid = env_cap;
  cudaLaunchConfig_t cfg = {};
  cfg.gridDim = dim3(grid); cfg.blockDim = dim3(staged ? 384 : 352); cfg.dynamicSmemBytes = smem; cfg.stream = s;
  cudaLaunchAttribute at[2];
  cfg.attrs = at; cfg.numAttrs = tc_launch_attrs(at, false);
  STG_CUDA_CHECK(cudaLaunchKernelEx(&cfg, kernels[0][staged][masked], tmA, tmW, em, p));
  STG_LAUNCH_CHECK();
  return STG_OK;
}

}
```

### ste_gan_b200/ops.py

```python
from __future__ import annotations

import ctypes as C
from typing import Optional, Tuple

import torch

from . import _lib
from ._lib import (ACT_LEAKY, ACT_NONE, ACT_RELU, ACT_TANH, BF16, ENGINE_AUTO, ENGINE_SIMT, ENGINE_TCGEN05, F32,
                   StgConv, StgWgrad, check)

Tensor = torch.Tensor
_engine_override: Optional[int] = None
profile = None
flop_log = None


def set_engine(engine: Optional[int]) -> None:
    global _engine_override
    _engine_override = engine


def code_of(dtype: torch.dtype) -> int:
    if dtype == torch.float32:
        return F32
    if dtype == torch.bfloat16:
        return BF16
    raise TypeError(f"unsupported dtype {dtype}")


def _ptr(t: Optional[Tensor]) -> Optional[int]:
    return None if t is None else t.data_ptr()


def _stream() -> int:
    return torch.cuda.current_stream().cuda_stream


def _need(t: Optional[Tensor], numel: int, dtype: Optional[torch.dtype], name: str) -> None:
    if t is None:
        return
    if not t.is_cuda:
        raise _lib.StgError(f"{name}: expected a CUDA tensor (there is no CPU fallback)")
    if not t.is_contiguous():
        raise _lib.StgError(f"{name}: expected a contiguous tensor")
    if dtype is not None and t.dtype != dtype:
        raise _lib.StgError(f"{name}: expected {dtype}, got {t.dtype}")
    if t.numel() < numel:
        raise _lib.StgError(f"{name}: buffer too small ({t.numel()} < {numel})")


def conv(src: Tensor, w: Tensor, *, n_samples: int, t_src: int, t_dst: int, c_src: int, c_dst: int, k: int,
         phases: int = 1, groups: int = 1, dilation: int = 1, stride: int = 1, pad: int = 0, transposed: bool = False,
         pair_sum: bool = False, post_shift: int = 0, mask: Optional[Tensor] = None, mask_mode: int = ACT_NONE,
         act: int = ACT_NONE, dup_rows: bool = False, bias: Optional[Tensor] = None, add_pre: Optional[Tensor] = None,
         add_post: Optional[Tensor] = None, y_raw: Optional[Tensor] = None, y_act: Optional[Tensor] = None,
         engine: int = ENGINE_AUTO, w_fwd_pack: bool = False, acct_groups: Optional[int] = None,
         valid_units: Optional[Tensor] = None, rows_per_unit: int = 1) -> None:
    dt = src.dtype
    nv = n_samples * phases
    t_out = t_dst // 2 if pair_sum else t_dst
    _need(src, nv * t_src * c_src, None, "src")
    _need(w, k * c_dst * (c_src // groups), dt, "w")
    _need(bias, c_dst, torch.float32, "bias")
    _need(add_pre, nv * t_out * c_dst, dt, "add_pre")
    _need(mask, nv * t_out * c_dst, dt, "mask")
    _need(add_post, nv * (t_out >> post_shift) * c_dst, dt, "add_post")
    outs = [t for t in (y_raw, y_act) if t is not None]
    out_f32 = dt != torch.float32 and len(outs) > 0 and all(t.dtype == torch.float32 for t in outs)
    odt = torch.float32 if out_f32 else dt
    _need(y_raw, nv * t_out * c_dst, odt, "y_raw")
    _need(y_act, nv * t_out * c_dst * (2 if dup_rows else 1), odt, "y_act")
    _need(valid_units, n_samples, torch.int32, "valid_units")
    d = StgConv(dtype=code_of(dt), engine=_engine_override if _engine_override is not None else engine,
                n_samples=n_samples, phases=phases, t_src=t_src, t_dst=t_dst, c_src=c_src, c_dst=c_dst, groups=groups,
                k=k, dilation=dilation, stride=stride, pad=pad, transposed=int(transposed), pair_sum=int(pair_sum),
                post_shift=post_shift, mask_mode=mask_mode, act=act, dup_rows=int(dup_rows), out_f32=int(out_f32),
                w_fwd_pack=int(w_fwd_pack), src=_ptr(src), w=_ptr(w), bias=_ptr(bias), add_pre=_ptr(add_pre), mask=_ptr(mask),
                add_post=_ptr(add_post), y_raw=_ptr(y_raw), y_act=_ptr(y_act))
    lib = _lib.load()

    def launch():
        if valid_units is None:
            check(lib.stg_conv(C.byref(d), _stream()), "stg_conv")
        else:
            check(lib.stg_conv_masked(C.byref(d), _ptr(valid_units), rows_per_unit, _stream()), "stg_conv_masked")

    if profile is None and flop_log is None:
        launch()
        return
    if valid_units is None:
        route = {1: "simt", 2: "tcgen05", 3: "matvec"}[lib.stg_conv_route(C.byref(d))]
    else:
        eng = d.engine if d.engine != ENGINE_AUTO else (ENGINE_TCGEN05 if lib.stg_conv_tc_supported(C.byref(d)) else ENGINE_SIMT)
        route = "tcgen05" if eng == ENGINE_TCGEN05 else "simt"
    ag = acct_groups if acct_groups is not None else groups
    flops = 2.0 * nv * t_src * c_src * k * (c_dst // ag) if transposed else 2.0 * nv * t_dst * c_dst * k * (c_src // ag)
    esz = 2 if dt == torch.bfloat16 else 4
    nbytes = esz * (nv * t_src * c_src + k * c_dst * (c_src // ag)) + sum(
        t.numel() * t.element_size() for t in (add_pre, mask, add_post, y_raw, y_act) if t is not None)
    rec = dict(kind=("dgrad" if transposed else "fwd"), engine=route, flops=flops, bytes=nbytes,
               shape=(n_samples, phases, t_src, t_dst, c_src, c_dst, k, dilation, stride, ag))
    if flop_log is not None:
        flop_log.append(rec)
    if profile is None:
        launch()
        return
    e0, e1 = torch.cuda.Event(enable_timing=True), torch.cuda.Event(enable_timing=True)
    e0.record()
    launch()
    e1.record()
    rec["ingest"] = _ingest(lib)
    fn, args = ("stg_conv", ()) if valid_units is None else ("stg_conv_masked", (_ptr(valid_units), rows_per_unit))
    profile.append(dict(rec, events=(e0, e1), desc=d, fn=fn, args=args,
                        keep=(src, w, bias, add_pre, mask, add_post, y_raw, y_act, valid_units)))


def _ingest(lib) -> float:
    return float(lib.stg_debug_ingest_bytes(1))


def conv_tc_supported(**kw) -> bool:
    d = StgConv(**kw)
    return bool(_lib.load().stg_conv_tc_supported(C.byref(d)))


def wgrad_layout(dtype: torch.dtype, *, c_in: int, c_out: int, k: int, groups: int = 1, stride: int = 1,
                 engine: int = ENGINE_AUTO) -> tuple:
    d = StgWgrad(dtype=code_of(dtype), engine=_engine_override if _engine_override is not None else engine, n_samples=1,
                 phases=1, t_in=1, t_out=1, c_in=c_in, c_out=c_out, groups=groups, k=k, dilation=1, stride=stride, pad=0)
    ld, span = C.c_int(0), C.c_int(0)
    check(_lib.load().stg_wgrad_layout(C.byref(d), C.byref(ld), C.byref(span)), "stg_wgrad_layout")
    return ld.value, span.value


def wgrad(x: Tensor, dy: Tensor, dw: Optional[Tensor], dbias: Optional[Tensor], *, n_samples: int, t_in: int,
          t_out: int, c_in: int, c_out: int, k: int, phases: int = 1, groups: int = 1, dilation: int = 1,
          stride: int = 1, pad: int = 0, engine: int = ENGINE_AUTO) -> None:
    nv = n_samples * phases
    _need(x, nv * t_in * c_in, None, "x")
    _need(dy, nv * t_out * c_out, x.dtype, "dy")
    if dw is not None:
        ld, _ = wgrad_layout(x.dtype, c_in=c_in, c_out=c_out, k=k, groups=groups, stride=stride, engine=engine)
        _need(dw, c_out * ld, torch.float32, "dw")
    _need(dbias, c_out, torch.float32, "dbias")
    d = StgWgrad(dtype=code_of(x.dtype), engine=_engine_override if _engine_override is not None else engine,
                 n_samples=n_samples, phases=phases, t_in=t_in, t_out=t_out, c_in=c_in, c_out=c_out, groups=groups,
                 k=k, dilation=dilation, stride=stride, pad=pad, x=_ptr(x), dy=_ptr(dy), dw=_ptr(dw), dbias=_ptr(dbias))
    lib = _lib.load()
    if profile is None and flop_log is None:
        check(lib.stg_conv_wgrad(C.byref(d), _stream()), "stg_conv_wgrad")
        return
    route = {1: "simt", 2: "tcgen05", 3: "matvec"}[lib.stg_wgrad_route(C.byref(d))]
    esz = 2 if x.dtype == torch.bfloat16 else 4
    rec = dict(kind="wgrad", engine=route, flops=2.0 * nv * t_out * c_out * k * (c_in // groups),
               bytes=esz * nv * (t_in * c_in + t_out * c_out) + 4 * c_out * k * (c_in // groups),
               shape=(n_samples, phases, t_in, t_out, c_in, c_out, k, dilation, stride, groups))
    if flop_log is not None:
        flop_log.append(rec)
    if profile is None:
        check(lib.stg_conv_wgrad(C.byref(d), _stream()), "stg_conv_wgrad")
        return
    e0, e1 = torch.cuda.Event(enable_timing=True), torch.cuda.Event(enable_timing=True)
    e0.record()
    check(lib.stg_conv_wgrad(C.byref(d), _stream()), "stg_conv_wgrad")
    e1.record()
    rec["ingest"] = _ingest(lib)
    profile.append(dict(rec, events=(e0, e1), desc=d, fn="stg_conv_wgrad", keep=(x, dy, dw, dbias)))


def tc_pack_groups(c_in: int, c_out: int, groups: int) -> int:
    return int(_lib.load().stg_tc_pack_groups(c_in, c_out, groups))


def round_up8(n: int) -> int:
    return (n + 7) // 8 * 8


def _pack_shapes(c_out: int, cin_g: int, k: int, groups: int, pack_groups: int, unfold: bool):
    if unfold:
        kp = round_up8(k * cin_g)
        return (c_out, kp), (kp, c_out)
    c_in = cin_g * groups
    return (k, c_out, c_in // pack_groups), (k, c_in, c_out // pack_groups)


def weightnorm_fold(v: Tensor, g: Tensor, groups: int, dtype: torch.dtype, want_dgrad: bool = True, out=None,
                    pack_groups: Optional[int] = None, unfold: bool = False):
    c_out, cin_g, k = v.shape[0], v.shape[1], v.shape[2]
    pg = groups if pack_groups is None else pack_groups
    sf, sd = _pack_shapes(c_out, cin_g, k, groups, pg, unfold)
    nf = sf[0] * sf[1] * (sf[2] if len(sf) > 2 else 1)
    _need(v, c_out * cin_g * k, torch.float32, "v"); _need(g, c_out, torch.float32, "g")
    if out is not None:
        wf, wd, scale = out
        _need(wf, nf, dtype, "wf"); _need(wd, nf, dtype, "wd"); _need(scale, c_out, torch.float32, "scale")
    else:
        wf = torch.empty(sf, device=v.device, dtype=dtype)
# ... 433 lines not shown
```

### ste_gan_b200/passes.py

```python
from __future__ import annotations

from dataclasses import dataclass, field
from typing import Dict, List, Optional, Sequence, Tuple

import torch

from . import ops
from .ops import ACT_LEAKY, ACT_NONE, ACT_RELU, ACT_TANH

Tensor = torch.Tensor


@dataclass
class Folded:
    mod: torch.nn.Module
    wf: Tensor
    wd: Optional[Tensor]
    dtype: torch.dtype
    scale: Optional[Tensor] = None
    u: Optional[Tensor] = None
    v: Optional[Tensor] = None
    sigma: Optional[Tensor] = None
    pg: int = 1
    unfold: bool = False
# ... 131 lines not shown
            nf_al = (nf + 63) // 64 * 64
            metas.append((m, pg, unf, sf, sd, nf, nf_al))
            n_pack += (2 if need_wd(m) else 1) * nf_al; n_scale += (m.out_channels + 3) // 4 * 4
        self._packs = torch.zeros(n_pack, device=dev, dtype=dtype)
        self._scales = torch.zeros(n_scale, device=dev, dtype=torch.float32)
        po = so = 0
        for (m, pg, unf, sf, sd, nf, nf_al) in metas:
            wf = self._packs[po:po + nf].view(sf); po += nf_al
            wd = None
            if need_wd(m):
                wd = self._packs[po:po + nf].view(sd); po += nf_al
            scale = self._scales[so:so + m.out_channels]; so += (m.out_channels + 3) // 4 * 4
            kp = ops.round_up8(m.kernel * m.in_channels) if unf else 0
            self.folds[id(m)] = Folded(m, wf, wd, dtype, scale=scale, pg=pg, unfold=unf, kp=kp)
        self._dw_off = {}
        for m in self.wn:
            n = dw_layout(self.folds[id(m)])[0]
            self._dw_off[id(m)] = (n_dw, n); n_dw += (n + 3) // 4 * 4
        self.arena = torch.zeros(n_dw, device=dev, dtype=torch.float32)
        items, row0, tile0 = [], 0, 0
        for m in self.wn:
            f = self.folds[id(m)]
            cin_g = m.in_channels // m.groups
            _, ld, span = dw_layout(f)
            off, n = self._dw_off[id(m)]
            gv, gg = _grad_of(m.weight_v), _grad_of(m.weight_g)
            items.append(_lib.StgFoldItem(
                v=m.weight_v.data.data_ptr(), g=m.weight_g.data.data_ptr(), wf=f.wf.data_ptr(), wd=f.wd.data_ptr() if f.wd is not None else None,
                scale=f.scale.data_ptr(), dw=self.arena[off:off + n].data_ptr(), dv=gv.data_ptr(), dg=gg.data_ptr(),
                c_out=m.out_channels, cin_g=cin_g, k=m.kernel, groups=m.groups, pg=f.pg,
                flags=_lib.PACK_UNFOLD if f.unfold else 0, dw_ld=ld, dw_span=span, row0=row0, tile0=tile0))
            row0 += m.out_channels
            if not self.need_wd:
                tile0 += m.kernel * f.pg if f.wd is not None else 0
            elif f.unfold:
                tile0 += -(-m.out_channels // 32) * -(-f.kp // 32)
            else:
                tile0 += m.kernel * f.pg * -(-(m.out_channels // f.pg) // 32) * -(-(m.in_channels // f.pg) // 32)
        self.n_items, self.total_rows, self.total_tiles = len(items), row0, (tile0 if self.need_wd else -tile0)
        self.item_row0 = [it.row0 for it in items] + [row0]
        self.table = ops.fold_table(items, dev)
        self._ptrs = [(p.data_ptr(), p.grad.data_ptr()) for m in self.wn for p in (m.weight_v, m.weight_g)]

    def _check_ptrs(self) -> None:
        cur = [(p.data_ptr(), p.grad.data_ptr() if p.grad is not None else 0) for m in self.wn for p in (m.weight_v, m.weight_g)]
        if cur != self._ptrs:
            raise RuntimeError("FoldPlan: parameter / gradient storage moved after the plan was built")

    def fold(self) -> Dict[int, Folded]:
        self._check_ptrs()
        ops.weightnorm_fold_multi(self.table, self.n_items, self.total_rows, self.total_tiles, self.dtype)
        return self.folds

    def zero(self) -> None:
        self.arena.zero_()

    def take(self, f: Folded) -> Tensor:
        ent = self._dw_off.get(id(f.mod))
        if ent is None:
            return torch.zeros(dw_layout(f)[0], device=self.device, dtype=torch.float32)
        return self.arena[ent[0]:ent[0] + ent[1]]

    def backward(self, accumulate: bool = True) -> None:
        self._check_ptrs()
        ops.weightnorm_fold_bwd_multi(self.table, self.n_items, self.total_rows, accumulate)


    def backward_range(self, item_lo: int, item_hi: int, accumulate: bool = True) -> None:
        self._check_ptrs()
        r0, r1 = self.item_row0[item_lo], self.item_row0[item_hi]
        if r1 > r0:
            ops.weightnorm_fold_bwd_range(self.table, self.n_items, r0, r1 - r0, accumulate)


def unfold_input(f: Folded, src: Tensor, B: int, t_src: int, phases: int = 1) -> Tensor:
    m = f.mod
    return ops.unfold(src, n_samples=B, phases=phases, t_src=t_src, t_dst=m.t_out(t_src), channels=m.in_channels,
                      k=m.kernel, dilation=m.dilation, stride=m.stride, pad=m.pad)


def _fwd(f: Folded, src: Tensor, B: int, t_src: int, *, phases: int = 1, act: int = ACT_NONE, want_raw: bool = False,
         want_act: bool = False, dup: bool = False, add_post: Optional[Tensor] = None, post_shift: int = 0,
         out_f32: bool = False, lengths: Optional[Tensor] = None, rate: int = 1) -> Tuple[Optional[Tensor], Optional[Tensor], int]:
    m = f.mod
    t_dst = m.t_out(t_src)
    odt = torch.float32 if out_f32 else f.dtype
    y_raw = torch.empty((B, t_dst * phases, m.out_channels), device=src.device, dtype=odt) if want_raw else None
    y_act = torch.empty((B, t_dst * phases * (2 if dup else 1), m.out_channels), device=src.device, dtype=odt) if want_act else None
    if f.unfold:
        ops.conv(src, f.wf, n_samples=B, phases=phases, t_src=t_dst, t_dst=t_dst, c_src=f.kp, c_dst=m.out_channels, k=1,
                 bias=m.bias.data, act=act, dup_rows=dup, add_post=add_post, post_shift=post_shift, y_raw=y_raw, y_act=y_act,
                 valid_units=lengths, rows_per_unit=rate)
    else:
        ops.conv(src, f.wf, n_samples=B, phases=phases, t_src=t_src, t_dst=t_dst, c_src=m.in_channels, c_dst=m.out_channels,
                 groups=f.pg, k=m.kernel, dilation=m.dilation, stride=m.stride, pad=m.pad, bias=m.bias.data, act=act,
                 dup_rows=dup, add_post=add_post, post_shift=post_shift, y_raw=y_raw, y_act=y_act, acct_groups=m.groups,
                 valid_units=lengths, rows_per_unit=rate)
    return y_raw, y_act, t_dst


def _dgrad(f: Folded, dy: Tensor, B: int, t_dy: int, t_x: int, *, phases: int = 1, mask: Optional[Tensor] = None,
           mask_mode: int = ACT_NONE, add_pre: Optional[Tensor] = None, add_post: Optional[Tensor] = None,
           pair_sum: bool = False, out_f32: bool = False) -> Tensor:
    m = f.mod
    if f.unfold:
        assert mask is None and add_pre is None and add_post is None and not pair_sum
        du = torch.empty((B, t_dy * phases, f.kp), device=dy.device, dtype=f.dtype)
        fwd_pack = f.dtype == torch.bfloat16
        ops.conv(dy, f.wf if fwd_pack else f.wd, n_samples=B, phases=phases, t_src=t_dy, t_dst=t_dy, c_src=m.out_channels,
                 c_dst=f.kp, k=1, transposed=True, y_raw=du, w_fwd_pack=fwd_pack)
        dx = torch.zeros((B, t_x * phases, m.in_channels), device=dy.device, dtype=torch.float32)
        ops.unfold_bwd(du, dx, n_samples=B, phases=phases, t_src=t_x, t_dst=t_dy, channels=m.in_channels, k=m.kernel,
                       dilation=m.dilation, stride=m.stride, pad=m.pad)
        return dx if out_f32 else ops.cast(dx, f.dtype)
    rows = t_x // 2 if pair_sum else t_x
    dx = torch.empty((B, rows * phases, m.in_channels), device=dy.device, dtype=torch.float32 if out_f32 else f.dtype)
    fwd_pack = f.dtype == torch.bfloat16 and not (m.groups > 1 and f.wd is not None)
    ops.conv(dy, f.wf if fwd_pack else f.wd, n_samples=B, phases=phases, t_src=t_dy, t_dst=t_x, c_src=m.out_channels,
             c_dst=m.in_channels, groups=f.pg, k=m.kernel, dilation=m.dilation, stride=m.stride, pad=m.pad, transposed=True,
             pair_sum=pair_sum, mask=mask, mask_mode=mask_mode, add_pre=add_pre, add_post=add_post, y_raw=dx,
             w_fwd_pack=fwd_pack, acct_groups=m.groups)
    return dx


def _wgrad(f: Folded, x: Tensor, dy: Tensor, B: int, t_x: int, t_dy: int, ws: _Workspace, phases: int = 1) -> None:
    m = f.mod
    side = ws.side_for_current() if getattr(ws, "wgrad_stream", None) is not None else None
    if side is not None:
        ev = torch.cuda.Event()
        ev.record(torch.cuda.current_stream())
        side.wait_event(ev)
        ws._keep.append((x, dy))
        with torch.cuda.stream(side):
            _wgrad_here(f, x, dy, B, t_x, t_dy, ws, phases)
        return
    _wgrad_here(f, x, dy, B, t_x, t_dy, ws, phases)


def _wgrad_here(f: Folded, x: Tensor, dy: Tensor, B: int, t_x: int, t_dy: int, ws, phases: int) -> None:
    m = f.mod
    dw = ws.take(f)
    if f.unfold:
        ops.wgrad(x, dy, dw, _grad_of(m.bias), n_samples=B, phases=phases, t_in=t_dy, t_out=t_dy, c_in=f.kp,
                  c_out=m.out_channels, k=1)
    else:
        ops.wgrad(x, dy, dw, _grad_of(m.bias), n_samples=B, phases=phases, t_in=t_x, t_out=t_dy, c_in=m.in_channels,
                  c_out=m.out_channels, groups=m.groups, k=m.kernel, dilation=m.dilation, stride=m.stride, pad=m.pad)
    if not (ws.deferred and m.norm == "weight_norm"):
        fold_backward(f, dw)


def generator_convs(model) -> List:
    convs = [model.gblocks[0]]
    for blk in list(model.gblocks)[1:]:
        c = blk.convs()
        convs += [c["c1"], c["c2"], c["res"], c["c3"], c["c4"]]
    convs.append(model.last_conv[1])
    return convs


def gblock_fwd(blk, folds: Dict[int, Folded], x_raw: Tensor, x_act: Tensor, B: int, t: int, *, want_raw: bool,
               want_act: bool, dup_next: bool, side=None, lengths: Optional[Tensor] = None, rate: int = 1):
    c = blk.convs()
    up = blk.upsample
    t_hi = t * up
    lo = dict(lengths=lengths, rate=rate)
    hi = dict(lengths=lengths, rate=rate * up)
    (r, _, _), (_, a1, _) = fork_join(
        side, lambda: _fwd(folds[id(c["res"])], x_raw, B, t, want_raw=True, **lo),
        lambda: _fwd(folds[id(c["c1"])], x_act, B, t_hi, act=ACT_RELU, want_act=True, **hi))
    h_raw, h_act, _ = _fwd(folds[id(c["c2"])], a1, B, t_hi, act=ACT_RELU, want_raw=True, want_act=True,
                           add_post=r, post_shift=1 if up > 1 else 0, **hi)
    _, a3, _ = _fwd(folds[id(c["c3"])], h_act, B, t_hi, act=ACT_RELU, want_act=True, **hi)
    y_raw, y_act, _ = _fwd(folds[id(c["c4"])], a3, B, t_hi, act=ACT_RELU, want_raw=want_raw, want_act=want_act,
                           add_post=h_raw, dup=dup_next, **hi)
    saved = dict(x_raw=x_raw, x_act=x_act, a1=a1, h_act=h_act, a3=a3, t_lo=t, t_hi=t_hi, up=up)
    return y_raw, y_act, saved


def gblock_bwd(blk, folds: Dict[int, Folded], s: dict, dy: Tensor, B: int, ws: _Workspace, out_f32: bool = False,
               side=None) -> Tensor:
    c = blk.convs()
    t_lo, t_hi, up = s["t_lo"], s["t_hi"], s["up"]
    f1, f2, fr, f3, f4 = (folds[id(c[k])] for k in ("c1", "c2", "res", "c3", "c4"))
    _wgrad(f4, s["a3"], dy, B, t_hi, t_hi, ws)
    da3 = _dgrad(f4, dy, B, t_hi, t_hi, mask=s["a3"], mask_mode=ACT_RELU)
    _wgrad(f3, s["h_act"], da3, B, t_hi, t_hi, ws)
    dh = _dgrad(f3, da3, B, t_hi, t_hi, mask=s["h_act"], mask_mode=ACT_RELU, add_post=dy)
    _wgrad(f2, s["a1"], dh, B, t_hi, t_hi, ws)

    def res_branch():
        dr = dh if up == 1 else ops.pair_sum_rows(dh, B * t_lo, fr.mod.out_channels).view(B, t_lo, -1)
        _wgrad(fr, s["x_raw"], dr, B, t_lo, t_lo, ws)
        return _dgrad(fr, dr, B, t_lo, t_lo), dr

    (dx_res, dr), da1 = fork_join(side, res_branch, lambda: _dgrad(f2, dh, B, t_hi, t_hi, mask=s["a1"], mask_mode=ACT_RELU))
    _wgrad(f1, s["x_act"], da1, B, t_hi, t_hi, ws)
    return _dgrad(f1, da1, B, t_hi, t_hi, pair_sum=up > 1, mask=s["x_raw"], mask_mode=ACT_RELU, add_post=dx_res,
                  out_f32=out_f32)


def fold_generator(model, dtype: torch.dtype, want_dgrad: bool = True, plan: Optional[FoldPlan] = None) -> Dict[int, Folded]:
    if plan is not None:
        return plan.fold()
    return {id(c): fold(c, dtype, want_dgrad=want_dgrad) for c in generator_convs(model)}
# ... 139 lines not shown
        e2 = torch.cuda.Event()
        e2.record(st)
        cur.wait_event(e2)


def fork_join(side: Optional["torch.cuda.Stream"], fn_side, fn_main):
    if side is None:
        return fn_side(), fn_main()
    ev = torch.cuda.Event()
    ev.record(torch.cuda.current_stream())
    side.wait_event(ev)
    with torch.cuda.stream(side):
        ra = fn_side()
    rb = fn_main()
    ev2 = torch.cuda.Event()
    ev2.record(side)
    torch.cuda.current_stream().wait_event(ev2)
    return ra, rb


def disc_subnets(model) -> List[Tuple[str, object]]:
    return [("P", d) for d in model.multi_pooled_disc] + [("S", d) for d in model.multi_scale_disc]


def discriminator_convs(model) -> List:
    out = []
    for _, d in disc_subnets(model):
        out += list(d.layers) + [d.output]
    return out


def fold_discriminator(model, dtype: torch.dtype, training: bool = True, want_dgrad: bool = True,
                       reuse: Optional[Dict[int, Folded]] = None,
                       persist: Optional[Dict[int, Folded]] = None,
                       plan: Optional[FoldPlan] = None, refold: bool = True, sn_streams=None) -> Dict[int, Folded]:
    if plan is not None:
        sn = [c for c in discriminator_convs(model) if c.norm != "weight_norm"]
        if sn_streams and sn:
            cur = torch.cuda.current_stream()
            ev = torch.cuda.Event()
            ev.record(cur)
            out = dict(plan.fold() if refold else plan.folds)
            used = []
            for i, c in enumerate(sn):
                st = sn_streams[i % len(sn_streams)]
                if st not in used:
                    st.wait_event(ev)
                    used.append(st)
                with torch.cuda.stream(st):
                    out[id(c)] = fold(c, dtype, training=training, want_dgrad=want_dgrad)
            for st in used:
                e2 = torch.cuda.Event()
                e2.record(st)
                cur.wait_event(e2)
            return out
        out = dict(plan.fold() if refold else plan.folds)
        for c in sn:
            out[id(c)] = fold(c, dtype, training=training, want_dgrad=want_dgrad)
        return out
    out = {}
    for c in discriminator_convs(model):
        if reuse is not None and c.norm == "weight_norm" and id(c) in reuse:
            out[id(c)] = reuse[id(c)]
        else:
            out[id(c)] = fold(c, dtype, training=training, want_dgrad=want_dgrad, persist=persist)
    return out


@dataclass
class DiscCtx:
    B: int = 0
    T: int = 0
    C: int = 0
    dtype: torch.dtype = torch.float32
    folds: Dict[int, Folded] = field(default_factory=dict)
    subs: List[dict] = field(default_factory=list)


def _heavy_split(subs: Sequence) -> Tuple[List[int], List[int]]:
    heavy = [i for i, (kind, _) in enumerate(subs) if kind == "S"][:1]
    return heavy, [i for i in range(len(subs)) if i not in heavy]


def discriminator_forward(model, x: Tensor, dtype: torch.dtype, folds: Dict[int, Folded], side=None,
                          subset: Optional[Sequence[int]] = None, spread: Optional[Sequence] = None):
    x = x.contiguous().float()
    B, T, Cc = x.shape
    ctx = DiscCtx(B=B, T=T, C=Cc, dtype=dtype, folds=folds)
    subs = disc_subnets(model)
    wanted = set(range(len(subs)) if subset is None else subset)
    last_scale = max([i for i in wanted if subs[i][0] == "S"], default=-1)
    scale_in, xs = {}, x
    for i, (kind, d) in enumerate(subs):
        if kind == "S":
            scale_in[i] = xs
            if subset is None or i < last_scale:
                xs = ops.avgpool4(xs)
    results: List = [None] * len(subs)
    sub_ctx: List = [None] * len(subs)

    def run(idx: List[int]) -> None:
        for i in idx:
            kind, d = subs[i]
            fused0 = False
            if kind == "P":
                p = d.period
                t_pad = T + (p - T % p)
                phases, t = p, t_pad // p
                l0, f0_ = d.layers[0], folds[id(d.layers[0])]
                fused0 = (f0_.unfold and dtype == torch.bfloat16 and l0.groups == 1 and l0.dilation == 1 and
                          l0.out_channels % 8 == 0 and t_pad - T < T)
                src = None if fused0 else ops.reflect_pad_right(x, t_pad, dtype)
            else:
                src = ops.cast(scale_in[i], dtype)
                phases, t = 1, scale_in[i].shape[1]
            f0 = folds[id(d.layers[0])]
            if f0.unfold and not fused0:
                src = unfold_input(f0, src, B, t, phases)
            sub = dict(kind=kind, phases=phases, inputs=[src], ts=[t], t_in0=scale_in[i].shape[1] if kind == "S" else T, mod=d)
            fmaps = []
            h = src
            layers = list(d.layers)
            if fused0:
                l0 = layers[0]
                h, t = ops.period_first_layer(x, f0.wf, l0.bias.data, period=phases, c_out=l0.out_channels, k=l0.kernel,
                                              stride=l0.stride, pad=l0.pad, slope=0.1)
                fmaps.append(h); sub["inputs"].append(h); sub["ts"].append(t)
                sub["x0"] = x
                layers = layers[1:]
            for layer in layers:
                _, h, t = _fwd(folds[id(layer)], h, B, t, phases=phases, act=ACT_LEAKY, want_act=True)
                fmaps.append(h); sub["inputs"].append(h); sub["ts"].append(t)
            logits, _, t = _fwd(folds[id(d.output)], h, B, t, phases=phases, want_raw=True, out_f32=True)
            sub["ts"].append(t)
            fmaps.append(logits)
            if kind == "S":
                sub["x_scale"] = scale_in[i]
            results[i], sub_ctx[i] = fmaps, sub

    heavy, rest = _heavy_split(subs)
    heavy, rest = [i for i in heavy if i in wanted], [i for i in rest if i in wanted]
    if spread:
        todo = heavy + rest
        lanes = [todo[j::len(spread) + 1] for j in range(len(spread) + 1)]
        fork_many(list(spread), [(lambda idx=idx: run(idx)) for idx in lanes if idx])
    elif side is not None and heavy and rest:
        fork_join(side, lambda: run(heavy), lambda: run(rest))
    else:
        run(heavy + rest)
    ctx.subs = sub_ctx
    ctx.keep = (scale_in, xs)
    return results, ctx


def first_layer_input(sub: dict, f: Folded, B: int, dtype: torch.dtype) -> Tensor:
    x, p, t = sub["x0"], sub["phases"], sub["ts"][0]
    src = ops.reflect_pad_right(x, t * p, dtype)
    return unfold_input(f, src, B, t, p)


def split_disc_batch(results: List, ctx: DiscCtx, idx: Sequence[int], n_first: int):
    res_a: List = [None] * len(results)
    res_b: List = [None] * len(results)
    sub_a: List = [None] * len(results)
    for i in idx:
        res_a[i] = [fm[:n_first] for fm in results[i]]
        res_b[i] = [fm[n_first:] for fm in results[i]]
        sub = dict(ctx.subs[i])
        sub["inputs"] = [t[:n_first] if t is not None else None for t in sub["inputs"]]
        if "x0" in sub:
            sub["x0"] = sub["x0"][:n_first]
        if "x_scale" in sub:
            sub["x_scale"] = sub["x_scale"][:n_first]
        sub_a[i] = sub
    return res_a, res_b, sub_a


def discriminator_backward(model, ctx: DiscCtx, dlogits: Sequence[Optional[Tensor]],
                           dfmaps: Optional[Sequence[Sequence[Optional[Tensor]]]] = None, want_input_grad: bool = False,
                           want_weight_grad: bool = True, plan: Optional[FoldPlan] = None, side=None,
                           spread: Optional[Sequence] = None) -> Optional[Tensor]:
    B, T, Cc, dtype, folds = ctx.B, ctx.T, ctx.C, ctx.dtype, ctx.folds
    dev = next(sub for sub in ctx.subs if sub is not None)["inputs"][1].device
    if plan is not None and want_weight_grad:
        ws = plan
    else:
        ws = _Workspace([folds[id(c)] for c in discriminator_convs(model)], dev) if want_weight_grad else None
        if ws is not None:
            side = None
    dx = torch.zeros((B, T, Cc), device=dev, dtype=torch.float32) if want_input_grad else None
    n_sub = len(ctx.subs)
    scale_grad: List = [None] * n_sub

    def run(idx: List[int]) -> None:
        for di in idx:
            sub = ctx.subs[di]
            if sub is None:
                continue
            d, phases, inputs, ts = sub["mod"], sub["phases"], sub["inputs"], sub["ts"]
            convs = list(d.layers) + [d.output]
            g = dlogits[di]
            fm_g = dfmaps[di] if dfmaps is not None else None
            if g is None and (fm_g is None or all(t is None for t in fm_g)):
                continue
            if g is None:
                g = torch.zeros((B, ts[-1] * phases, 1), device=dev, dtype=dtype)
            dxin = None
            for j in reversed(range(len(convs))):
                f = folds[id(convs[j])]
                if want_weight_grad:
                    xin = inputs[j] if inputs[j] is not None else first_layer_input(sub, f, B, dtype)
                    _wgrad(f, xin, g, B, ts[j], ts[j + 1], ws, phases=phases)
                if j == 0:
                    if want_input_grad:
                        dxin = _dgrad(f, g, B, ts[1], ts[0], phases=phases, out_f32=True)
                    break
                g = _dgrad(f, g, B, ts[j + 1], ts[j], phases=phases, mask=inputs[j], mask_mode=ACT_LEAKY,
                           add_pre=fm_g[j - 1] if fm_g is not None else None)
            if want_input_grad:
                if sub["kind"] == "P":
                    ops.reflect_pad_right_bwd(dxin, T, dx)
                else:
                    scale_grad[di] = dxin

    heavy, rest = _heavy_split([(sub["kind"] if sub is not None else "-", None) for sub in ctx.subs])
    if spread and (plan is not None or not want_weight_grad):
        h_here = [i for i in heavy if ctx.subs[i] is not None] if side is not None else []
        todo = [i for i in range(n_sub) if ctx.subs[i] is not None and i not in h_here]
        lanes = [l for l in (todo[j::len(spread) + 1] for j in range(len(spread) + 1)) if l]
        fns = [(lambda idx=idx: run(idx)) for idx in lanes] or [lambda: None]
        streams = list(spread)[:len(fns) - 1]
        if h_here:
            fns.append(lambda: run(h_here)); streams.append(side)
        fork_many(streams, fns)
    elif side is not None and heavy and any(ctx.subs[i] is not None for i in rest):
        fork_join(side, lambda: run(heavy), lambda: run(rest))
    else:
        run(list(range(n_sub)))
    if want_input_grad:
        carry = None
        for di in reversed([i for i, sub in enumerate(ctx.subs) if sub is not None and sub["kind"] == "S"]):
            t_in, cur = ctx.subs[di]["t_in0"], scale_grad[di]
            if carry is not None:
                if cur is None:
                    cur = torch.zeros((B, t_in, Cc), device=dev, dtype=torch.float32)
                ops.avgpool4_bwd(carry, t_in, cur)
            carry = cur
        if carry is not None:
            ops.axpy_f32(dx, carry, 1.0)
    return dx


def to_reference_layout(fm: Tensor, kind: str, phases: int) -> Tensor:
    B, HP, Cc = fm.shape
    if kind == "P":
        return fm.view(B, HP // phases, phases, Cc).permute(0, 3, 1, 2)
    return fm.transpose(1, 2)


def single_conv_forward(mod, x: Tensor) -> Tensor:
    from .autograd import SingleConvFn
    return SingleConvFn.apply(mod, x, *[p for p in mod.parameters()])


def gblock_forward_torch_layout(blk, x: Tensor) -> Tensor:
    from .autograd import GBlockFn
    return GBlockFn.apply(blk, x, *[p for p in blk.parameters()])
```

### ste_gan_b200/trainer.py

```python
from __future__ import annotations

from typing import Dict, List, Optional

import torch
from . import ops, passes
from .dist import GradReducer

Tensor = torch.Tensor

W_TD_DEFAULT, W_FM_DEFAULT = 15.0, 7.0
LOSS_NAMES = ["loss_d", "loss_adv", "loss_fm", "loss_td_20_8", "loss_td_51_13", "loss_td_80_16", "loss_speech_unit", "loss_phoneme"]
W_SU_DEFAULT, W_PH_DEFAULT = 1.0, 1.0


class FlatParams:

    def __init__(self, module: torch.nn.Module):
        self.params = [p for p in module.parameters()]
        dev = self.params[0].device
        if dev.type != "cuda":
            raise RuntimeError("FlatParams: move the module to a CUDA device first")
        al = lambda k: (k + 3) // 4 * 4
        n = sum(al(p.numel()) for p in self.params)
        self.flat = torch.zeros(n, device=dev, dtype=torch.float32)
        self.grad = torch.zeros(n, device=dev, dtype=torch.float32)
        off = 0
        self.offsets: Dict[str, int] = {}
        names = [nm for nm, _ in module.named_parameters()]
        for nm, p in zip(names, self.params):
            k = p.numel()
            self.flat[off:off + k].copy_(p.data.reshape(-1))
            p.data = self.flat[off:off + k].view(p.shape)
            p.grad = self.grad[off:off + k].view(p.shape)
            self.offsets[nm] = off
            off += al(k)
        self.m = torch.zeros_like(self.flat)
        self.v = torch.zeros_like(self.flat)
        self.step = torch.zeros(1, device=dev, dtype=torch.int64)
        self.numel = n

    def zero_grad(self) -> None:
        self.grad.zero_()

    def adamw(self, lr, betas=(0.8, 0.99), eps: float = 1e-8, weight_decay: float = 1e-2,
              grad_scale: float = 1.0, enable: Optional[Tensor] = None, lo: int = 0, hi: Optional[int] = None,
              keep_step: bool = False) -> None:
        hi = self.numel if hi is None else hi
        ops.adamw(self.flat[lo:hi], self.grad[lo:hi], self.m[lo:hi], self.v[lo:hi], self.step, lr, betas[0], betas[1], eps,
                  weight_decay, grad_scale, enable, keep_step)


def generator_grad_buckets(offsets: Dict[str, int], numel: int, nblk: int) -> list:
    first = [offsets[next(nm for nm in offsets if nm.startswith(f"gblocks.{i + 1}."))] for i in range(nblk)]
    last = offsets[next(nm for nm in offsets if nm.startswith("last_conv."))]
    near = lambda frac, lo: min(range(lo, nblk), key=lambda i: abs(first[i] - frac * numel), default=nblk)
    k1 = near(1.0 / 3.0, 1)
    k2 = near(2.0 / 3.0, k1)
    n_conv = 5 * nblk + 2
    cut = lambda i: first[i] if i < nblk else last
    return [(k2, nblk, 1 + 5 * k2, n_conv, (cut(k2), numel)),
            (k1, k2, 1 + 5 * k1, 1 + 5 * k2, (cut(k1), cut(k2))),
            (0, k1, 0, 1 + 5 * k1, (0, cut(k1)))]


class GanTrainer:
    def __init__(self, net_g, net_d, precision: str = "bf16", lr: float = 2e-4, w_td: float = W_TD_DEFAULT,
                 w_fm: float = W_FM_DEFAULT, loss_adversarial: bool = True, loss_multi_td: bool = True,
                 loss_feat_match: bool = True, group=None, grad_buckets: Optional[int] = None, data_parallel: bool = True,
                 emg_encoder=None, loss_speech_unit: Optional[bool] = None, loss_phoneme: Optional[bool] = None,
                 w_su: float = W_SU_DEFAULT, w_ph: float = W_PH_DEFAULT):
        self.net_g, self.net_d = net_g, net_d
        self.dtype = torch.bfloat16 if precision == "bf16" else torch.float32
        self.w_td, self.w_fm = w_td, w_fm
        self.use_adv, self.use_td, self.use_fm = loss_adversarial, loss_multi_td, loss_feat_match
        self.emg_encoder = emg_encoder
        self.use_su = (emg_encoder is not None) if loss_speech_unit is None else bool(loss_speech_unit)
        self.use_ph = (emg_encoder is not None) if loss_phoneme is None else bool(loss_phoneme)
        if (self.use_su or self.use_ph) and emg_encoder is None:
            raise ValueError("loss_speech_unit / loss_phoneme need an emg_encoder")
        self.w_su, self.w_ph = w_su, w_ph
        self._enc_plan = None
        if emg_encoder is not None:
            if emg_encoder.training:
                raise ValueError("the EMG encoder of the perceptual losses is frozen: call emg_encoder.eval() (emg_encoder_loss.py:61)")
            self._enc_plan = emg_encoder.plan(self.dtype)
        self._cur_su = self._cur_ph = None
        self.G, self.D = FlatParams(net_g), FlatParams(net_d)
        self.g_plan = passes.FoldPlan(passes.generator_convs(net_g), self.dtype)
        self.d_plan = passes.FoldPlan(passes.discriminator_convs(net_d), self.dtype)
        self._d_folded = False
        self.reducer = GradReducer(group, enabled=data_parallel)
        self._inline = self.reducer.comm is not None
        dev = self.G.flat.device
        self.device = dev
        self.base_lr = float(lr)
        self._lr = float(lr)
        self.lr_dev = torch.full((1,), float(lr), device=dev, dtype=torch.float32)
        self.slots = torch.zeros(8, device=dev, dtype=torch.float32)
        self.d_folds: Optional[Dict[int, passes.Folded]] = None
        self._d_persist: Dict[int, passes.Folded] = {}
        self._graphs = None
        self._d_graphs = None
        self._pending_g = None
        self._static = None
        self.x_pred: Optional[Tensor] = None
        self._side = torch.cuda.Stream(device=dev)
        self._side2 = [torch.cuda.Stream(device=dev), torch.cuda.Stream(device=dev)]
        self._wg = [torch.cuda.Stream(device=dev) for _ in range(7)]
        self._ps = [torch.cuda.Stream(device=dev) for _ in range(2)]
        self._ss = [torch.cuda.Stream(device=dev)]
        self._sn = [torch.cuda.Stream(device=dev) for _ in range(4)]
        self._aux = torch.cuda.Stream(device=dev)
        self._enc = torch.cuda.Stream(device=dev)
        self._comm = torch.cuda.Stream(device=dev)
        self._pend = torch.zeros(1, device=dev, dtype=torch.int32)
        self._fused = None
        self._pending_host = False
        self._sm_reserve, self._n_sm = 0, torch.cuda.get_device_properties(dev).multi_processor_count
        self.concurrent_d = True
        import os
        self._d_slices = self._disc_grad_slices() if os.environ.get("STG_D_BUCKETS", "1") != "0" else None
        self.g_buckets = generator_grad_buckets(self.G.offsets, self.G.numel, len(list(net_g.gblocks)) - 1)
        if grad_buckets is None and os.environ.get("STG_G_BUCKETS"):
            grad_buckets = int(os.environ["STG_G_BUCKETS"])
        if (grad_buckets if grad_buckets is not None else (3 if self.reducer.enabled else 1)) == 1:
            nblk = len(list(net_g.gblocks)) - 1
            self.g_buckets = [(0, nblk, 0, 5 * nblk + 2, (0, self.G.numel))]

    @property
    def lr(self) -> float:
        return self._lr

    @lr.setter
    def lr(self, value: float) -> None:
        self.flush()
        self._lr = float(value)
        self.lr_dev.fill_(self._lr)

    def scheduler_step(self, gamma: float = 0.999) -> float:
        self.lr = self._lr * gamma
        return self._lr

    def _disc_grad_slices(self):
        subs = passes.disc_subnets(self.net_d)
        heavy, rest = passes._heavy_split(subs)
        if len(heavy) != 1 or any(i > heavy[0] for i in rest if subs[i][0] == "P") or any(i < heavy[0] for i in rest if subs[i][0] == "S"):
            return None
        wn = self.d_plan.wn
        def item_range(mods):
            ids = [k for k, m in enumerate(wn) if any(m is c for d_ in mods for c in list(d_.layers) + [d_.output])]
            return (ids[0], ids[-1] + 1) if ids and ids == list(range(ids[0], ids[-1] + 1)) else None
        def grad_range(prefixes):
            offs = [o for nm, o in self.D.offsets.items() if nm.startswith(tuple(prefixes))]
            nxt = [o for nm, o in self.D.offsets.items() if o > max(offs) and not nm.startswith(tuple(prefixes))]
            return min(offs), (min(nxt) if nxt else self.D.numel)
        p_mods = [subs[i][1] for i in rest if subs[i][0] == "P"]
        s_mods = [subs[i][1] for i in rest if subs[i][0] == "S"]
        h_mods = [subs[heavy[0]][1]]
        names = {id(m): nm for nm, m in self.net_d.named_modules()}
        pre = lambda mods: [names[id(m)] + "." for m in mods]
        out = dict(early=[], late=None)
        for mods in (p_mods, s_mods):
            if mods:
                ir = item_range(mods)
                if ir is None:
                    return None
                out["early"].append((ir, grad_range(pre(mods))))
        ir = item_range(h_mods)
        if ir is None:
            return None
        out["late"] = (ir, grad_range(pre(h_mods)))
        cover = sorted([g for _, g in out["early"]] + [out["late"][1]])
        if cover[0][0] != 0 or cover[-1][1] != self.D.numel or any(a[1] != b[0] for a, b in zip(cover, cover[1:])):
            return None
        return out

    def _s2(self, i: int):
        return self._side2[i] if self.concurrent_d else None

    def _fold_d(self, refold: bool):
        return passes.fold_discriminator(self.net_d, self.dtype, training=True, plan=self.d_plan, refold=refold,
                                         sn_streams=self._sn if self.concurrent_d else None)

    def _reduce(self, flat_slice: Tensor):
        if not self.reducer.enabled or flat_slice.numel() == 0:
            return None
        ev = torch.cuda.Event()
        ev.record(torch.cuda.current_stream())
        self._comm.wait_event(ev)
        self.reducer.all_reduce_on(flat_slice, self._comm)
        done = torch.cuda.Event()
        done.record(self._comm)
        return done

    @staticmethod
    def _wait_events(evs) -> None:
        for e in evs:
            if e is not None:
                torch.cuda.current_stream().wait_event(e)

    def _sm_scope(self, on: bool) -> None:
        if self._sm_reserve > 0:
            from . import _lib as _l
            _l.load().stg_set_sm_limit(self._n_sm - self._sm_reserve if on else 0)

    def _fork(self) -> None:
        ev = torch.cuda.Event()
        ev.record(torch.cuda.current_stream())
        self._side.wait_event(ev)

    def _join(self) -> None:
        ev = torch.cuda.Event()
        ev.record(self._side)
        torch.cuda.current_stream().wait_event(ev)

    def _d_folds(self) -> None:
        refold_d = not self._d_folded
        self._d_folded = True
        self._f1 = self._fold_d(refold_d)
        self._ev_f1 = torch.cuda.Event()
        self._ev_f1.record(torch.cuda.current_stream())
        self._f2 = self._fold_d(False)

    def _split_subs(self):
        subs = passes.disc_subnets(self.net_d)
        heavy, rest = passes._heavy_split(subs)
        return subs, heavy, [i for i in rest if subs[i][0] == "P"], [i for i in rest if subs[i][0] == "S"]

    def _d_real(self, x_real: Tensor) -> None:
        self._x_real = x_real
        if self.concurrent_d:
            _, heavy, _, _ = self._split_subs()
            self._real = passes.discriminator_forward(self.net_d, x_real, self.dtype, self._f2, subset=heavy) if heavy else (None, None)
        else:
            self._real = passes.discriminator_forward(self.net_d, x_real, self.dtype, self._f2)

    def _g_forward(self, su: Tensor, sess: Tensor, mode: Optional[Tensor], x_pred: Optional[Tensor] = None) -> None:
        self.slots.zero_()
        self.G.zero_grad(); self.D.zero_grad()
        self._gctx = None
        self._cur_su = su
        if x_pred is not None:
            self.x_pred = x_pred
            return
        self.x_pred, self._gctx = passes.generator_forward(self.net_g, su, sess, mode, self.dtype, True, folds=self.g_plan.fold(),
                                                           side=self._s2(1) if self.use_adv else None)

    def _d_fake(self) -> None:
        dt = self.dtype
        if not self.concurrent_d:
            self._fake = passes.discriminator_forward(self.net_d, self.x_pred, dt, self._f1)
            return
        _, heavy, p_idx, s_idx = self._split_subs()
        fwd = lambda x, idx: passes.discriminator_forward(self.net_d, x, dt, self._f1, subset=idx,
                                                          spread=self._ps if idx is p_idx else (self._ss if idx is s_idx else None)) if idx else (None, None)
        x_cat = torch.cat([self.x_pred, self._x_real], 0)
        ((rs, cs), (rp, cp)), (rh, ch) = passes.fork_join(
            self._s2(1), lambda: passes.fork_join(self._s2(0), lambda: fwd(x_cat, p_idx), lambda: fwd(x_cat, s_idx))[::-1],
            lambda: fwd(self.x_pred, heavy))
        self._fake = (rh, ch)
        self._batched = (rp, cp, rs, cs, x_cat)

    def _d_update(self) -> None:
        dt = self.dtype
        if not self.concurrent_d:
            (res_f, ctx_f), (res_r, ctx_r) = self._fake, self._real
            self._fake = self._real = None
            self._last_d_fmaps = (res_f, res_r, ctx_f)
            nd = len(res_f)
            dl = ops.mse_const_multi([fm[-1] for fm in res_f] + [fm[-1] for fm in res_r], [0.0] * nd + [1.0] * nd, self.slots,
                                     [0] * (2 * nd), 1.0, dt)
            self.d_plan.zero()
            passes.discriminator_backward(self.net_d, ctx_f, dl[:nd], None, want_input_grad=False, want_weight_grad=True, plan=self.d_plan)
            passes.discriminator_backward(self.net_d, ctx_r, dl[nd:], None, want_input_grad=False, want_weight_grad=True, plan=self.d_plan)
            self.d_plan.backward(accumulate=False)
            self._reduce_d()
            return
        subs, heavy, p_idx, s_idx = self._split_subs()
        (rh_f, ch_f), (rh_r, ch_r) = self._fake, self._real
        rp, cp, rs, cs, x_cat = self._batched
        self._fake = self._real = self._batched = None
        Bq, nd = self.x_pred.shape[0], len(subs)
        res_f, res_r = [None] * nd, [None] * nd
        for r_b, c_b, idx in ((rp, cp, p_idx), (rs, cs, s_idx)):
            if idx:
                a, b, _ = passes.split_disc_batch(r_b, c_b, idx, Bq)
                for i in idx:
                    res_f[i], res_r[i] = a[i], b[i]
        for i in heavy:
            res_f[i], res_r[i] = rh_f[i], rh_r[i]
        self._last_d_fmaps = (res_f, res_r, ch_f)
        dcat = {i: torch.empty((2 * Bq,) + tuple(res_f[i][-1].shape[1:]), device=self.device, dtype=dt) for i in p_idx + s_idx}
        outs = [dcat[i][:Bq] if i in dcat else None for i in range(nd)] + [dcat[i][Bq:] if i in dcat else None for i in range(nd)]
        dl = ops.mse_const_multi([fm[-1] for fm in res_f] + [fm[-1] for fm in res_r], [0.0] * nd + [1.0] * nd, self.slots,
                                 [0] * (2 * nd), 1.0, dt, outs=outs)
        dl_f, dl_r = dl[:nd], dl[nd:]
        dl_b = [dcat.get(i) for i in range(nd)]
        self.d_plan.zero()
        cur = torch.cuda.current_stream()
        self.d_plan.async_wgrads({st.cuda_stream: w for st, w in zip((cur, self._side, self._side2[0], self._side2[1], *self._ps, *self._ss), self._wg)})
        bwd = lambda ctx, dlog: passes.discriminator_backward(self.net_d, ctx, dlog, None, want_input_grad=False,
                                                              want_weight_grad=True, plan=self.d_plan,
                                                              spread=self._ps if ctx is cp else (self._ss if ctx is cs else None)) if ctx is not None else None
        only = lambda dlog, idx: [dlog[i] if i in idx else None for i in range(nd)]
        self._fork()
        with torch.cuda.stream(self._side):
            passes.fork_join(self._s2(0), lambda: bwd(ch_r, only(dl_r, heavy)), lambda: bwd(ch_f, only(dl_f, heavy)))
        passes.fork_join(self._s2(1), lambda: bwd(cs, only(dl_b, s_idx)), lambda: bwd(cp, only(dl_b, p_idx)))
        early = []
        if self._inline and heavy and self._d_slices is not None:
            self.d_plan.join_wgrads_of([cur, self._side2[1], *self._ps, *self._ss])
            for (i_lo, i_hi), (g_lo, g_hi) in self._d_slices["early"]:
                self.d_plan.backward_range(i_lo, i_hi, accumulate=False)
                early.append(self._reduce(self.D.grad[g_lo:g_hi]))
        self._join()
        self.d_plan.join_wgrads()
        if early:
            (i_lo, i_hi), (g_lo, g_hi) = self._d_slices["late"]
            self.d_plan.backward_range(i_lo, i_hi, accumulate=False)
            self._wait_events(early + [self._reduce(self.D.grad[g_lo:g_hi])])
            return
        self.d_plan.backward(accumulate=False)
        self._reduce_d()

    def _reduce_d(self) -> None:
        if self._inline:
            self._wait_events([self._reduce(self.D.grad)])

    def _phase_d(self, su: Tensor, sess: Tensor, mode: Optional[Tensor], x_real: Tensor, x_pred: Optional[Tensor] = None,
                 head=None) -> None:
        head = head or (lambda: None)
        if not self.use_adv:
            head()
            self._g_forward(su, sess, mode, x_pred)
            return
        if self.concurrent_d:
            cur = torch.cuda.current_stream()
            self._fork()
            self._sm_scope(True)
            with torch.cuda.stream(self._side):
                self._d_folds()
                self._d_real(x_real)
            head()
            self._sm_scope(False)
            self._g_forward(su, sess, mode, x_pred)
            cur.wait_event(self._ev_f1)
            self._d_fake()
            self._join()
        else:
            self._d_folds()
            head()
            self._g_forward(su, sess, mode, x_pred)
            self._d_fake()
            self._d_real(x_real)
        self._sm_scope(True)
        self._d_update()
        self._sm_scope(False)

    def _phase_g_head(self, x_real: Tensor, update_d: bool = True) -> None:
        dx_pred = self._g_losses(x_real, update_d)
        self._last_gctx = self._gctx
        self._gb = passes.GenBackward(self.net_g, self._gctx, dx_pred, plan=self.g_plan, side=self._s2(1), res_side=self._s2(0),
                                      overwrite_grads=True)
        self._g_bucket(0)

    def _g_losses(self, x_real: Tensor, update_d: bool = True) -> Tensor:
        dt = self.dtype
        x_pred = self.x_pred
        dx_pred = torch.zeros_like(x_pred)
        td_ev = None
        enc_ev, dx_enc = None, None
        if self.use_su or self.use_ph:
            from . import passes_encoder as pe
            if self._cur_ph is None:
                raise ValueError("the phoneme loss needs phoneme_targets ([B, frames] int64) in step() / step_graph()")
            ev = torch.cuda.Event()
            ev.record(torch.cuda.current_stream())
            self._enc.wait_event(ev)
            with torch.cuda.stream(self._enc if self.concurrent_d else torch.cuda.current_stream()):
                dx_enc, self._enc_units, self._enc_logits = pe.encoder_losses(
                    self._enc_plan, x_pred, self._cur_su, self._cur_ph, self.slots[6:8], self.w_su, self.w_ph, True,
                    self.use_su, self.use_ph)
                enc_ev = torch.cuda.Event()
                enc_ev.record(torch.cuda.current_stream())
        if self.use_td and self.use_adv and self.concurrent_d:
            ev = torch.cuda.Event()
            ev.record(torch.cuda.current_stream())
            self._aux.wait_event(ev)
            with torch.cuda.stream(self._aux):
                ops.td_loss(x_real, x_pred, self.slots[3:6], [self.w_td] * 3, dx_pred)
                td_ev = torch.cuda.Event()
                td_ev.record(self._aux)
        if self.use_adv:
            if update_d:
                self.D.adamw(self.lr_dev, grad_scale=self.reducer.grad_scale)
            refold_d = update_d or not self._d_folded
            self._d_folded = True
            if self.concurrent_d:
                subs = passes.disc_subnets(self.net_d)
                heavy, rest = passes._heavy_split(subs)
                p_idx = [i for i in rest if subs[i][0] == "P"]
                s_idx = [i for i in rest if subs[i][0] == "S"]
                Bq = x_pred.shape[0]
                f3 = self._fold_d(refold_d)
                x_cat = torch.cat([x_pred, x_real], 0)
                fwd = lambda x, f, idx: passes.discriminator_forward(self.net_d, x, dt, f, subset=idx,
                                                                     spread=self._ps if idx is p_idx else (self._ss if idx is s_idx else None)) if idx else (None, None)
                self._fork()
                with torch.cuda.stream(self._side):
                    (rs, cs), (rh_f, ch_f) = passes.fork_join(self._s2(0), lambda: fwd(x_cat, f3, s_idx), lambda: fwd(x_pred, f3, heavy))
                f4 = self._fold_d(False)
                (rh_r, _), (rp, cp) = passes.fork_join(self._s2(1), lambda: fwd(x_real, f4, heavy), lambda: fwd(x_cat, f3, p_idx))
                self._join()
                res_f, res_r, sub_f = [None] * len(subs), [None] * len(subs), [None] * len(subs)
                for r_b, c_b, idx in ((rp, cp, p_idx), (rs, cs, s_idx)):
                    if idx:
                        a, b, sa = passes.split_disc_batch(r_b, c_b, idx, Bq)
                        for i in idx:
                            res_f[i], res_r[i], sub_f[i] = a[i], b[i], sa[i]
                for i in heavy:
                    res_f[i], res_r[i], sub_f[i] = rh_f[i], rh_r[i], ch_f.subs[i]
                assert all(r is not None for r in res_f)
                ctx_f = passes.DiscCtx(B=Bq, T=x_pred.shape[1], C=x_pred.shape[2], dtype=dt, folds=f3, subs=sub_f)
                ctx_f.keep = (ch_f, cp, cs, x_cat)
            else:
                f3 = self._fold_d(refold_d)
                f4 = self._fold_d(False)
                res_f, ctx_f = passes.discriminator_forward(self.net_d, x_pred, dt, f3)
                res_r, _ = passes.discriminator_forward(self.net_d, x_real, dt, f4)
            self.d_folds = f4
            self._last_g_fmaps = (res_f, res_r)
            nd = len(res_f)
            dlog = ops.mse_const_multi([fm[-1] for fm in res_f], [1.0] * nd, self.slots, [1] * nd, 1.0, dt)
            if self.use_fm:
                pairs = [(a, b) for fm_f, fm_r in zip(res_f, res_r) for a, b in zip(fm_f[:-1], fm_r[:-1])]
                grads = ops.l1_mean_multi(pairs, self.slots[2:3], self.w_fm)
                dfm, i = [], 0
                for fm_f in res_f:
                    dfm.append(grads[i:i + len(fm_f) - 1]); i += len(fm_f) - 1
            else:
                dfm = [[None] * (len(fm_f) - 1) for fm_f in res_f]
            dx_d = passes.discriminator_backward(self.net_d, ctx_f, dlog, dfm, want_input_grad=True, want_weight_grad=False,
                                                 side=self._s2(0), spread=self._ps if self.concurrent_d else None)
            if td_ev is not None:
                torch.cuda.current_stream().wait_event(td_ev)
            ops.axpy_f32(dx_pred, dx_d, 1.0)
        if self.use_td and td_ev is None:
            ops.td_loss(x_real, x_pred, self.slots[3:6], [self.w_td] * 3, dx_pred)
        if dx_enc is not None:
            torch.cuda.current_stream().wait_event(enc_ev)
            ops.axpy_f32(dx_pred, dx_enc, 1.0)
        return dx_pred

    def _g_bucket(self, i: int) -> None:
        lo, hi, c_lo, c_hi, _ = self.g_buckets[i]
        gb = self._gb
        gb.blocks(lo, hi)
        if i == len(self.g_buckets) - 1:
            gb.finish()
        gb.bucket(c_lo, c_hi, last=i == len(self.g_buckets) - 1)
        if i == len(self.g_buckets) - 1:
            self._gb = self._gctx = None

    def _phase_g(self, x_real: Tensor, update_d: bool = True, reduce: bool = False, defer_last: bool = False) -> list:
        handles = []
        self._phase_g_head(x_real, update_d)
        n = len(self.g_buckets)
        for i in range(n):
            if i > 0:
                self._g_bucket(i)
            if reduce and not (defer_last and i == n - 1):
                handles += self._reduce_g_bucket(i)
        return handles

    def _reduce_g_bucket(self, i: int) -> list:
        lo, hi = self.g_buckets[i][4]
        if self._inline:
            return [self._reduce(self.G.grad[lo:hi])]
        return self.reducer.all_reduce_async(self.G.grad[lo:hi]) if hi > lo else []

    def _wait_handles(self, handles) -> None:
        if self._inline:
            self._wait_events(handles)
        else:
            self.reducer.wait(handles)

    def _phase_opt_g(self) -> None:
        self.G.adamw(self.lr_dev, grad_scale=self.reducer.grad_scale)

    def _opt_g_head(self) -> None:
        n = len(self.g_buckets)
        lo, hi = self.g_buckets[n - 1][4]
        if self._inline:
            self._wait_events(self._reduce_g_bucket(n - 1))
        self.G.adamw(self.lr_dev, grad_scale=self.reducer.grad_scale, enable=self._pend, lo=lo, hi=hi, keep_step=n > 1)

    def _fused_step(self, s: dict) -> None:
        self._phase_d(s["su"], s["sess"], s["mode"], s["x_real"], head=self._opt_g_head)
        self._phase_g_head(s["x_real"])
        n, evs = len(self.g_buckets), []
        for i in range(n - 1):
            if i > 0:
                self._g_bucket(i)
            lo, hi = self.g_buckets[i][4]
            ev = self._reduce(self.G.grad[lo:hi])
            self._sm_scope(True)
            if ev is None:
                ev = torch.cuda.Event()
                ev.record(torch.cuda.current_stream())
                self._comm.wait_event(ev)
            with torch.cuda.stream(self._comm):
                self.G.adamw(self.lr_dev, grad_scale=self.reducer.grad_scale, lo=lo, hi=hi, keep_step=i > 0)
                done = torch.cuda.Event()
                done.record(self._comm)
            evs.append(done)
        if n > 1:
            self._g_bucket(n - 1)
        self._sm_scope(False)
        self._wait_events(evs)
        self._pend.fill_(1)

    def step(self, speech_units: Tensor, session_ids: Tensor, x_real: Tensor,
             speaking_mode_ids: Optional[Tensor] = None, phoneme_targets: Optional[Tensor] = None) -> Tensor:
        self.flush()
        su = speech_units.contiguous().float()
        xr = x_real.contiguous().float()
# ... 212 lines not shown
```

Baseline: 4030.

## Batch same-geometry period-discriminator convs into one grouped tcgen05 launch

Adds a stg_conv_multi API and a grouped tensor-core conv kernel. It runs up to eight same-geometry convolutions in one launch and splits CTAs between problems using a per-tile cost estimate. The period sub-discriminators' forward and backward layers are now issued together through this path instead of being spread across extra side streams, and the dedicated period streams are removed. The goal is fewer launches and less stream fan-out for small convs. The risk is a worse load balance than separate concurrent streams, plus extra block-to-problem lookup cost in the kernel.

New measurement: 4051 (median of 6 runs). Within noise of the previous version (+0.5%).

```diff
diff --git a/include/stegan_b200.h b/include/stegan_b200.h
--- a/include/stegan_b200.h
+++ b/include/stegan_b200.h
@@ -52,6 +52,13 @@
 
 int stg_conv(const StgConv* d, stg_stream_t stream);
 
+#define STG_MAX_MULTI 8
+typedef struct StgConvMulti {
+  int32_t n;
+  StgConv item[STG_MAX_MULTI];
+} StgConvMulti;
+int stg_conv_multi(const StgConvMulti* d, stg_stream_t stream);
+
 int stg_conv_masked(const StgConv* d, const int32_t* valid_units, int32_t rows_per_unit, stg_stream_t stream);
 
 typedef struct StgWgrad {
diff --git a/ste_gan_b200/_lib.py b/ste_gan_b200/_lib.py
--- a/ste_gan_b200/_lib.py
+++ b/ste_gan_b200/_lib.py
@@ -18,6 +18,13 @@
         "dtype", "engine", "n_samples", "phases", "t_src", "t_dst", "c_src", "c_dst", "groups", "k", "dilation",
         "stride", "pad", "transposed", "pair_sum", "post_shift", "mask_mode", "act", "dup_rows", "out_f32", "w_fwd_pack")] + [
         (n, C.c_void_p) for n in ("src", "w", "bias", "add_pre", "mask", "add_post", "y_raw", "y_act")]
+
+
+MAX_MULTI = 8
+
+
+class StgConvMulti(C.Structure):
+    _fields_ = [("n", C.c_int32), ("item", StgConv * MAX_MULTI)]
 
 
 class StgWgrad(C.Structure):
@@ -44,6 +51,7 @@
 _SIGS = {
     "stg_conv": [C.POINTER(StgConv), _P],
     "stg_conv_masked": [C.POINTER(StgConv), _P, C.c_int32, _P],
+    "stg_conv_multi": [C.POINTER(StgConvMulti), _P],
     "stg_conv_wgrad": [C.POINTER(StgWgrad), _P],
     "stg_conv_tc_supported": [C.POINTER(StgConv)],
     "stg_conv_route": [C.POINTER(StgConv)],
diff --git a/ste_gan_b200/csrc/api.cu b/ste_gan_b200/csrc/api.cu
--- a/ste_gan_b200/csrc/api.cu
+++ b/ste_gan_b200/csrc/api.cu
@@ -31,14 +31,7 @@
   return STG_OK;
 }
 
-}
-
-using namespace stg;
-
-extern "C" int stg_conv(const StgConv* d, stg_stream_t stream) {
-  int r = validate_conv(d);
-  if (r) return r;
-  cudaStream_t s = static_cast<cudaStream_t>(stream);
+static int conv_one(const StgConv* d, cudaStream_t s) {
   switch (d->engine) {
     case STG_ENGINE_SIMT: return d->w_fwd_pack ? STG_EUNSUPPORTED : conv_simt(d, s);
     case STG_ENGINE_TCGEN05: return conv_tc(d, s);
@@ -48,6 +41,55 @@
       return d->w_fwd_pack ? STG_EUNSUPPORTED : conv_simt(d, s);
     default: return STG_EINVAL;
   }
+}
+
+static int conv_route(const StgConv* d) {
+  if (d->engine == STG_ENGINE_SIMT) return STG_ENGINE_SIMT;
+  if (d->engine == STG_ENGINE_TCGEN05) return STG_ENGINE_TCGEN05;
+  if (conv_c1_supported(d)) return STG_ENGINE_MATVEC;
+  return conv_tc_supported(d) ? STG_ENGINE_TCGEN05 : STG_ENGINE_SIMT;
+}
+
+static bool same_geometry(const StgConv* a, const StgConv* b) {
+  return a->dtype == b->dtype && a->engine == b->engine && a->c_src == b->c_src && a->c_dst == b->c_dst &&
+         a->groups == b->groups && a->k == b->k && a->dilation == b->dilation && a->stride == b->stride && a->pad == b->pad &&
+         a->transposed == b->transposed && a->pair_sum == b->pair_sum && a->post_shift == b->post_shift &&
+         a->mask_mode == b->mask_mode && a->act == b->act && a->dup_rows == b->dup_rows && a->out_f32 == b->out_f32 &&
+         a->w_fwd_pack == b->w_fwd_pack;
+}
+
+}
+
+using namespace stg;
+
+extern "C" int stg_conv(const StgConv* d, stg_stream_t stream) {
+  if (!d) return STG_EINVAL;
+  StgConvMulti m;
+  m.n = 1;
+  m.item[0] = *d;
+  return stg_conv_multi(&m, stream);
+}
+
+extern "C" int stg_conv_multi(const StgConvMulti* m, stg_stream_t stream) {
+  if (!m || m->n < 1 || m->n > STG_MAX_MULTI) return STG_EINVAL;
+  const StgConv* items[STG_MAX_MULTI];
+  for (int i = 0; i < m->n; ++i) {
+    items[i] = &m->item[i];
+    const int r = validate_conv(items[i]);
+    if (r) return r;
+    if (i > 0 && !same_geometry(items[0], items[i])) return STG_EINVAL;
+  }
+  cudaStream_t s = static_cast<cudaStream_t>(stream);
+  if (m->n == 1) return conv_one(items[0], s);
+  const int route = conv_route(items[0]);
+  for (int i = 1; i < m->n; ++i)
+    if (conv_route(items[i]) != route) return STG_EINVAL;
+  if (route == STG_ENGINE_TCGEN05) return conv_tc_multi(items, m->n, s);
+  for (int i = 0; i < m->n; ++i) {
+    const int r = conv_one(items[i], s);
+    if (r) return r;
+  }
+  return STG_OK;
 }
 
 extern "C" int stg_conv_masked(const StgConv* d, const int32_t* valid_units, int32_t rows_per_unit, stg_stream_t stream) {
@@ -66,10 +108,7 @@
 
 extern "C" int stg_conv_route(const StgConv* d) {
   if (!d || validate_conv(d) != STG_OK) return STG_EINVAL;
-  if (d->engine == STG_ENGINE_SIMT) return STG_ENGINE_SIMT;
-  if (d->engine == STG_ENGINE_TCGEN05) return STG_ENGINE_TCGEN05;
-  if (conv_c1_supported(d)) return STG_ENGINE_MATVEC;
-  return conv_tc_supported(d) ? STG_ENGINE_TCGEN05 : STG_ENGINE_SIMT;
+  return conv_route(d);
 }
 extern "C" int stg_wgrad_route(const StgWgrad* d) {
   if (!d) return STG_EINVAL;
diff --git a/ste_gan_b200/csrc/common.cuh b/ste_gan_b200/csrc/common.cuh
--- a/ste_gan_b200/csrc/common.cuh
+++ b/ste_gan_b200/csrc/common.cuh
@@ -95,6 +95,7 @@
 
 int conv_simt(const StgConv* d, cudaStream_t s, const int32_t* valid_units = nullptr, int rows_per_unit = 1);
 int conv_tc(const StgConv* d, cudaStream_t s, const int32_t* valid_units = nullptr, int rows_per_unit = 1);
+int conv_tc_multi(const StgConv* const* items, int n, cudaStream_t s);
 int conv_tc_plan(const StgConv* d, int* out);
 bool conv_tc_supported(const StgConv* d);
 int wgrad_simt(const StgWgrad* d, cudaStream_t s);
diff --git a/ste_gan_b200/csrc/conv_tc.cu b/ste_gan_b200/csrc/conv_tc.cu
--- a/ste_gan_b200/csrc/conv_tc.cu
+++ b/ste_gan_b200/csrc/conv_tc.cu
@@ -246,10 +246,9 @@
   }
 }
 
-template <bool kStaged, bool kPair, bool kMask>
-__global__ void __launch_bounds__(kStaged ? 384 : 352, (kStaged && !kPair) ? 2 : 1)
-conv_tc_kernel(const __grid_constant__ TmA4 tmA4, const __grid_constant__ CUtensorMap tmW,
-               const __grid_constant__ EpiMaps em, const TcP p) {
+template <bool kStaged, bool kPair, bool kMask, bool kMulti>
+__device__ __forceinline__ void conv_tc_body(const CUtensorMap* tmA, const CUtensorMap& tmW, const EpiMaps& em, const TcP& p,
+                                             int cta, int n_ctas) {
   constexpr int EPI_WARPS = 8;
   extern __shared__ uint8_t smem_raw[];
   const uint32_t smem_base = (smem_u32(smem_raw) + 1023u) & ~1023u;
@@ -257,8 +256,8 @@
   const int stage_bytes = p.a_bytes + p.max_ntaps * b_bytes;
   const TcEpi& e = p.e;
   const int rank = kPair ? __shfl_sync(0xffffffffu, (int)cluster_ctarank(), 0) : 0;
-  const int tile0 = kPair ? (int)(blockIdx.x >> 1) : (int)blockIdx.x;
-  const int tstep = kPair ? (int)(gridDim.x >> 1) : (int)gridDim.x;
+  const int tile0 = kMulti ? cta : kPair ? (int)(blockIdx.x >> 1) : (int)blockIdx.x;
+  const int tstep = kMulti ? n_ctas : kPair ? (int)(gridDim.x >> 1) : (int)gridDim.x;
   const uint32_t epi_base = smem_base + p.stages * stage_bytes;
   const uint32_t bias_base = epi_base + (kStaged ? ((e.n_in << e.in_sh) + p.out_ring * e.n_out) * SLOT : 0);
   const uint32_t bar_base = bias_base + (kStaged ? 2048 : 0);
@@ -274,7 +273,7 @@
   life_ev(p.trace, 30);
   pdl_trigger();
   if (warp == 0 && lane == 0) {
-    for (int c = 0; c < p.n_cls; ++c) prefetch_tmap(&tmA4.m[c]);
+    for (int c = 0; c < p.n_cls; ++c) prefetch_tmap(&tmA[c]);
     prefetch_tmap(&tmW);
     for (int s = 0; s < p.stages; ++s) { mbar_init(full_bar(s), 1); mbar_init(empty_bar(s), 1); }
     for (int a = 0; a < 2; ++a) { mbar_init(tmem_full_bar(a), 1); mbar_init(tmem_empty_bar(a), kPair ? 2 * EPI_WARPS : EPI_WARPS); }
@@ -339,7 +338,7 @@
             if (rank == 0) mbar_expect_tx_el(full_bar(s), tx_bytes);
 #pragma unroll 1
             for (int bx = 0; bx < p.a_boxes; ++bx)
-              tma_load_4d_el<kPair>(a_dst + bx * a_box_bytes, &tmA4.m[x.cls], fb, c0, 0, row0 + bx * row_step, x.b);
+              tma_load_4d_el<kPair>(a_dst + bx * a_box_bytes, &tmA[x.cls], fb, c0, 0, row0 + bx * row_step, x.b);
           }
 #ifdef STG_PROF_LOOP
           const long long pc2 = clock64();
@@ -448,7 +447,7 @@
           mbar_expect_tx_el(full_bar(s), (uint32_t)(p.a_boxes * p.hb * p.pack * KC * 2 + nt * b_bytes));
 #pragma unroll 1
           for (int bx = 0; bx < p.a_boxes; ++bx)
-            tma_load_4d_el(a_dst + bx * p.hb * p.pack * KC * 2, &tmA4.m[0], full_bar(s), x.ch0 + chunk * KC, 0,
+            tma_load_4d_el(a_dst + bx * p.hb * p.pack * KC * 2, &tmA[0], full_bar(s), x.ch0 + chunk * KC, 0,
                            (x.h0 + bx * p.hb) * p.stride + p.tt.g_off[g], x.b);
         }
 #pragma unroll 1
@@ -788,6 +787,33 @@
   life_ev(p.trace, 33);
 }
 
+template <bool kStaged, bool kPair, bool kMask>
+__global__ void __launch_bounds__(kStaged ? 384 : 352, (kStaged && !kPair) ? 2 : 1)
+conv_tc_kernel(const __grid_constant__ TmA4 tmA4, const __grid_constant__ CUtensorMap tmW,
+               const __grid_constant__ EpiMaps em, const TcP p) {
+  conv_tc_body<kStaged, kPair, kMask, false>(tmA4.m, tmW, em, p, 0, 0);
+}
+
+struct TcProblem {
+  CUtensorMap a, w;
+  EpiMaps em;
+  TcP p;
+};
+struct TcMulti {
+  TcProblem q[STG_MAX_MULTI];
+  int n, cta0[STG_MAX_MULTI + 1];
+};
+static_assert(sizeof(TcMulti) <= 32764, "kernel parameters are limited to 32764 bytes");
+
+template <bool kStaged>
+__global__ void __launch_bounds__(kStaged ? 384 : 352, kStaged ? 2 : 1)
+conv_tc_kernel(const __grid_constant__ TcMulti m) {
+  int i = 0;
+  while (i + 1 < m.n && (int)blockIdx.x >= m.cta0[i + 1]) ++i;
+  const TcProblem& q = m.q[i];
+  conv_tc_body<kStaged, false, false, true>(&q.a, q.w, q.em, q.p, (int)blockIdx.x - m.cta0[i], m.cta0[i + 1] - m.cta0[i]);
+}
+
 }
 
 PFN_encodeTiled get_encode_tiled() {
@@ -999,9 +1025,20 @@
   return r;
 }
 
-int conv_tc(const StgConv* d, cudaStream_t s, const int32_t* valid_units, int rows_per_unit) {
+struct TcLaunch {
+  TcP p;
+  TmA4 tmA;
+  CUtensorMap tmW;
+  EpiMaps em;
+  bool staged, pair, occ2;
+  size_t smem;
+  double ingest;
+  double tile_cost;
+};
+
+static int conv_tc_prepare(const StgConv* d, const int32_t* valid_units, int rows_per_unit, TcLaunch& L) {
   if (!conv_tc_supported(d)) return STG_EUNSUPPORTED;
-  TcP p;
+  TcP& p = L.p;
   p.trace = g_trace;
   p.phases = d->phases; p.t_dst = d->t_dst; p.stride = d->transposed ? 1 : d->stride;
   p.cs_g = d->c_src / d->groups; p.cd_g = d->c_dst / d->groups;
@@ -1210,9 +1247,9 @@
     return STG_OK;
   }
 
-  CUtensorMap tmW;
-  TmA4 tmA;
-  EpiMaps em;
+  CUtensorMap& tmW = L.tmW;
+  TmA4& tmA = L.tmA;
+  EpiMaps& em = L.em;
   memset(&em, 0, sizeof(em));
   memset(&tmA, 0, sizeof(tmA));
   for (int c = 0; c < p.n_cls; ++c) {
@@ -1279,51 +1316,126 @@
     }
     if (r) return STG_ECUDA;
   }
-  using Kernel = decltype(&conv_tc_kernel<true, false, false>);
+  p.tiles_n = ceil_div(d->c_dst, p.bn);
+  const int64_t n_tiles = pair ? (int64_t)p.n_res * p.pairs_per_res * p.tiles_n
+                        : n_rc ? (int64_t)p.cls_mt0[p.n_cls] * p.tiles_n : (int64_t)d->n_samples * p.n_res * p.tiles_m * p.tiles_n;
+  if (n_tiles > 0x7fffffff) return STG_EINVAL;
+  p.n_tiles = (int)n_tiles;
+  L.staged = staged; L.pair = pair; L.occ2 = occ2; L.smem = smem;
+  L.ingest = pair ? 0.0 : (double)n_tiles * ((double)best.traffic * p.k_chunks / p.n_res + (staged ? (double)e.n_in * p.mrows * p.bn * 2 : 0.0));
+  const double stage = (2.0 * p.bn > 200.0 ? 2.0 * p.bn : 200.0) + 60.0;
+  L.tile_cost = (double)p.res_gfirst[p.n_res] / p.n_res * p.k_chunks * stage + (p.bn / 32.0) * 200.0;
+  return STG_OK;
+}
+
+using Kernel = decltype(&conv_tc_kernel<true, false, false>);
+using MultiKernel = void (*)(TcMulti);
+
+static int set_kernel_attrs() {
+  static bool attr_set = false;
+  if (attr_set) return STG_OK;
+  const Kernel kernels[2][2][2] = {
+      {{conv_tc_kernel<false, false, false>, conv_tc_kernel<false, false, true>},
+       {conv_tc_kernel<true, false, false>, conv_tc_kernel<true, false, true>}},
+      {{conv_tc_kernel<false, true, false>, conv_tc_kernel<false, true, true>},
+       {conv_tc_kernel<true, true, false>, conv_tc_kernel<true, true, true>}}};
+  for (int i = 0; i < 8; ++i) {
+    const Kernel k = kernels[i >> 2][(i >> 1) & 1][i & 1];
+    STG_CUDA_CHECK(cudaFuncSetAttribute(k, cudaFuncAttributeMaxDynamicSharedMemorySize, 227 * 1024));
+    if ((i >> 1) == 1)
+      STG_CUDA_CHECK(cudaFuncSetAttribute(k, cudaFuncAttributePreferredSharedMemoryCarveout, cudaSharedmemCarveoutMaxShared));
+  }
+  const MultiKernel mk[2] = {conv_tc_kernel<false>, conv_tc_kernel<true>};
+  for (int i = 0; i < 2; ++i) STG_CUDA_CHECK(cudaFuncSetAttribute(mk[i], cudaFuncAttributeMaxDynamicSharedMemorySize, 227 * 1024));
+  STG_CUDA_CHECK(cudaFuncSetAttribute(mk[1], cudaFuncAttributePreferredSharedMemoryCarveout, cudaSharedmemCarveoutMaxShared));
+  attr_set = true;
+  return STG_OK;
+}
+
+int conv_tc(const StgConv* d, cudaStream_t s, const int32_t* valid_units, int rows_per_unit) {
+  TcLaunch L;
+  int r = conv_tc_prepare(d, valid_units, rows_per_unit, L);
+  if (r != STG_OK || g_plan_out) return r;
+  r = set_kernel_attrs();
+  if (r) return r;
   static const Kernel kernels[2][2][2] = {
       {{conv_tc_kernel<false, false, false>, conv_tc_kernel<false, false, true>},
        {conv_tc_kernel<true, false, false>, conv_tc_kernel<true, false, true>}},
       {{conv_tc_kernel<false, true, false>, conv_tc_kernel<false, true, true>},
        {conv_tc_kernel<true, true, false>, conv_tc_kernel<true, true, true>}}};
-  static bool attr_set = false;
-  if (!attr_set) {
-    for (int i = 0; i < 8; ++i) {
-      const Kernel k = kernels[i >> 2][(i >> 1) & 1][i & 1];
-      STG_CUDA_CHECK(cudaFuncSetAttribute(k, cudaFuncAttributeMaxDynamicSharedMemorySize, 227 * 1024));
-      if ((i >> 1) == 1)
-        STG_CUDA_CHECK(cudaFuncSetAttribute(k, cudaFuncAttributePreferredSharedMemoryCarveout, cudaSharedmemCarveoutMaxShared));
-    }
-    attr_set = true;
-  }
   const bool masked = valid_units != nullptr;
-  p.tiles_n = ceil_div(d->c_dst, p.bn);
-  if (pair) {
-    const int64_t n_tiles = (int64_t)p.n_res * p.pairs_per_res * p.tiles_n;
-    if (n_tiles > 0x7fffffff) return STG_EINVAL;
-    p.n_tiles = (int)n_tiles;
+  const TcP& p = L.p;
+  cudaLaunchConfig_t cfg = {};
+  cfg.blockDim = dim3(L.staged ? 384 : 352); cfg.dynamicSmemBytes = L.smem; cfg.stream = s;
+  cudaLaunchAttribute at[2];
+  cfg.attrs = at; cfg.numAttrs = tc_launch_attrs(at, L.pair);
+  if (L.pair) {
     const int max_pairs = sm_count() / 2;
     const int n_pairs = p.n_tiles < max_pairs ? p.n_tiles : max_pairs;
-    cudaLaunchConfig_t cfg = {};
-    cfg.gridDim = dim3(2 * n_pairs); cfg.blockDim = dim3(staged ? 384 : 352); cfg.dynamicSmemBytes = smem; cfg.stream = s;
-    cudaLaunchAttribute at[2];
-    cfg.attrs = at; cfg.numAttrs = tc_launch_attrs(at, true);
-    STG_CUDA_CHECK(cudaLaunchKernelEx(&cfg, kernels[1][staged][masked], tmA, tmW, em, p));
+    cfg.gridDim = dim3(2 * n_pairs);
+    STG_CUDA_CHECK(cudaLaunchKernelEx(&cfg, kernels[1][L.staged][masked], L.tmA, L.tmW, L.em, p));
     STG_LAUNCH_CHECK();
     return STG_OK;
   }
-  const int64_t n_tiles = n_rc ? (int64_t)p.cls_mt0[p.n_cls] * p.tiles_n : (int64_t)d->n_samples * p.n_res * p.tiles_m * p.tiles_n;
-  if (n_tiles > 0x7fffffff) return STG_EINVAL;
-  p.n_tiles = (int)n_tiles;
-  g_ingest_bytes += (double)n_tiles * ((double)best.traffic * p.k_chunks / p.n_res + (staged ? (double)e.n_in * p.mrows * p.bn * 2 : 0.0));
+  g_ingest_bytes += L.ingest;
   static const int env_cap = getenv("STG_GRID_CAP") ? atoi(getenv("STG_GRID_CAP")) : 0;
-  const int slots = (occ2 ? 2 : 1) * sm_count();
+  const int slots = (L.occ2 ? 2 : 1) * sm_count();
   int grid = p.n_tiles < slots ? p.n_tiles : slots;
   if (env_cap > 0 && grid > env_cap) grid = env_cap;
+  cfg.gridDim = dim3(grid);
+  STG_CUDA_CHECK(cudaLaunchKernelEx(&cfg, kernels[0][L.staged][masked], L.tmA, L.tmW, L.em, p));
+  STG_LAUNCH_CHECK();
+  return STG_OK;
+}
+
+int conv_tc_multi(const StgConv* const* items, int n, cudaStream_t s) {
+  if (n < 2 || n > STG_MAX_MULTI) return STG_EINVAL;
+  static thread_local TcMulti m;
+  static thread_local TcLaunch L[STG_MAX_MULTI];
+  memset(&m, 0, sizeof(m));
+  bool staged = false, occ2 = true;
+  size_t smem = 0;
+  int64_t total_tiles = 0;
+  for (int i = 0; i < n; ++i) {
+    const int r = conv_tc_prepare(items[i], nullptr, 1, L[i]);
+    if (r) return r;
+    if (L[i].pair || L[i].p.n_cls > 1) return STG_EUNSUPPORTED;
+    if (i > 0 && L[i].staged != staged) return STG_EUNSUPPORTED;
+    staged = L[i].staged;
+    occ2 = occ2 && L[i].occ2;
+    if (L[i].smem > smem) smem = L[i].smem;
+    total_tiles += L[i].p.n_tiles;
+  }
+  const int slots = (occ2 ? 2 : 1) * sm_count();
+  const int grid = total_tiles < slots ? (int)total_tiles : slots;
+  int ctas[STG_MAX_MULTI];
+  for (int i = 0; i < n; ++i) ctas[i] = 1;
+  for (int used = n; used < grid; ++used) {
+    int best = -1;
+    double best_t = -1.0;
+    for (int i = 0; i < n; ++i) {
+      if (ctas[i] >= L[i].p.n_tiles) continue;
+      const double t = (double)((L[i].p.n_tiles + ctas[i] - 1) / ctas[i]) * L[i].tile_cost;
+      if (t > best_t) { best_t = t; best = i; }
+    }
+    if (best < 0) break;
+    ++ctas[best];
+  }
+  m.n = n;
+  m.cta0[0] = 0;
+  for (int i = 0; i < n; ++i) {
+    m.q[i].a = L[i].tmA.m[0]; m.q[i].w = L[i].tmW; m.q[i].em = L[i].em; m.q[i].p = L[i].p;
+    m.cta0[i + 1] = m.cta0[i] + ctas[i];
+    g_ingest_bytes += L[i].ingest;
+  }
+  const int r = set_kernel_attrs();
+  if (r) return r;
+  static const MultiKernel kernels[2] = {conv_tc_kernel<false>, conv_tc_kernel<true>};
   cudaLaunchConfig_t cfg = {};
-  cfg.gridDim = dim3(grid); cfg.blockDim = dim3(staged ? 384 : 352); cfg.dynamicSmemBytes = smem; cfg.stream = s;
+  cfg.gridDim = dim3(m.cta0[n]); cfg.blockDim = dim3(staged ? 384 : 352); cfg.dynamicSmemBytes = smem; cfg.stream = s;
   cudaLaunchAttribute at[2];
   cfg.attrs = at; cfg.numAttrs = tc_launch_attrs(at, false);
-  STG_CUDA_CHECK(cudaLaunchKernelEx(&cfg, kernels[0][staged][masked], tmA, tmW, em, p));
+  STG_CUDA_CHECK(cudaLaunchKernelEx(&cfg, kernels[staged], m));
   STG_LAUNCH_CHECK();
   return STG_OK;
 }
diff --git a/ste_gan_b200/ops.py b/ste_gan_b200/ops.py
--- a/ste_gan_b200/ops.py
+++ b/ste_gan_b200/ops.py
@@ -49,13 +49,13 @@
         raise _lib.StgError(f"{name}: buffer too small ({t.numel()} < {numel})")
 
 
-def conv(src: Tensor, w: Tensor, *, n_samples: int, t_src: int, t_dst: int, c_src: int, c_dst: int, k: int,
-         phases: int = 1, groups: int = 1, dilation: int = 1, stride: int = 1, pad: int = 0, transposed: bool = False,
-         pair_sum: bool = False, post_shift: int = 0, mask: Optional[Tensor] = None, mask_mode: int = ACT_NONE,
-         act: int = ACT_NONE, dup_rows: bool = False, bias: Optional[Tensor] = None, add_pre: Optional[Tensor] = None,
-         add_post: Optional[Tensor] = None, y_raw: Optional[Tensor] = None, y_act: Optional[Tensor] = None,
-         engine: int = ENGINE_AUTO, w_fwd_pack: bool = False, acct_groups: Optional[int] = None,
-         valid_units: Optional[Tensor] = None, rows_per_unit: int = 1) -> None:
+def _conv_item(src: Tensor, w: Tensor, *, n_samples: int, t_src: int, t_dst: int, c_src: int, c_dst: int, k: int,
+               phases: int = 1, groups: int = 1, dilation: int = 1, stride: int = 1, pad: int = 0, transposed: bool = False,
+               pair_sum: bool = False, post_shift: int = 0, mask: Optional[Tensor] = None, mask_mode: int = ACT_NONE,
+               act: int = ACT_NONE, dup_rows: bool = False, bias: Optional[Tensor] = None, add_pre: Optional[Tensor] = None,
+               add_post: Optional[Tensor] = None, y_raw: Optional[Tensor] = None, y_act: Optional[Tensor] = None,
+               engine: int = ENGINE_AUTO, w_fwd_pack: bool = False, acct_groups: Optional[int] = None,
+               valid_units: Optional[Tensor] = None) -> Tuple[StgConv, float, float, tuple, tuple]:
     dt = src.dtype
     nv = n_samples * phases
     t_out = t_dst // 2 if pair_sum else t_dst
@@ -77,6 +77,20 @@
                 post_shift=post_shift, mask_mode=mask_mode, act=act, dup_rows=int(dup_rows), out_f32=int(out_f32),
                 w_fwd_pack=int(w_fwd_pack), src=_ptr(src), w=_ptr(w), bias=_ptr(bias), add_pre=_ptr(add_pre), mask=_ptr(mask),
                 add_post=_ptr(add_post), y_raw=_ptr(y_raw), y_act=_ptr(y_act))
+    ag = acct_groups if acct_groups is not None else groups
+    flops = 2.0 * nv * t_src * c_src * k * (c_dst // ag) if transposed else 2.0 * nv * t_dst * c_dst * k * (c_src // ag)
+    esz = 2 if dt == torch.bfloat16 else 4
+    nbytes = esz * (nv * t_src * c_src + k * c_dst * (c_src // ag)) + sum(
+        t.numel() * t.element_size() for t in (add_pre, mask, add_post, y_raw, y_act) if t is not None)
+    shape = (n_samples, phases, t_src, t_dst, c_src, c_dst, k, dilation, stride, ag)
+    return d, flops, nbytes, shape, (src, w, bias, add_pre, mask, add_post, y_raw, y_act, valid_units)
+
+
+_ROUTES = {1: "simt", 2: "tcgen05", 3: "matvec"}
+
+
+def conv(src: Tensor, w: Tensor, *, valid_units: Optional[Tensor] = None, rows_per_unit: int = 1, **kw) -> None:
+    d, flops, nbytes, shape, keep = _conv_item(src, w, valid_units=valid_units, **kw)
     lib = _lib.load()
 
     def launch():
@@ -89,17 +103,11 @@
         launch()
         return
     if valid_units is None:
-        route = {1: "simt", 2: "tcgen05", 3: "matvec"}[lib.stg_conv_route(C.byref(d))]
+        route = _ROUTES[lib.stg_conv_route(C.byref(d))]
     else:
         eng = d.engine if d.engine != ENGINE_AUTO else (ENGINE_TCGEN05 if lib.stg_conv_tc_supported(C.byref(d)) else ENGINE_SIMT)
         route = "tcgen05" if eng == ENGINE_TCGEN05 else "simt"
-    ag = acct_groups if acct_groups is not None else groups
-    flops = 2.0 * nv * t_src * c_src * k * (c_dst // ag) if transposed else 2.0 * nv * t_dst * c_dst * k * (c_src // ag)
-    esz = 2 if dt == torch.bfloat16 else 4
-    nbytes = esz * (nv * t_src * c_src + k * c_dst * (c_src // ag)) + sum(
-        t.numel() * t.element_size() for t in (add_pre, mask, add_post, y_raw, y_act) if t is not None)
-    rec = dict(kind=("dgrad" if transposed else "fwd"), engine=route, flops=flops, bytes=nbytes,
-               shape=(n_samples, phases, t_src, t_dst, c_src, c_dst, k, dilation, stride, ag))
+    rec = dict(kind=("dgrad" if d.transposed else "fwd"), engine=route, flops=flops, bytes=nbytes, shape=shape)
     if flop_log is not None:
         flop_log.append(rec)
     if profile is None:
@@ -111,8 +119,36 @@
     e1.record()
     rec["ingest"] = _ingest(lib)
     fn, args = ("stg_conv", ()) if valid_units is None else ("stg_conv_masked", (_ptr(valid_units), rows_per_unit))
-    profile.append(dict(rec, events=(e0, e1), desc=d, fn=fn, args=args,
-                        keep=(src, w, bias, add_pre, mask, add_post, y_raw, y_act, valid_units)))
+    profile.append(dict(rec, events=(e0, e1), desc=d, fn=fn, args=args, keep=keep))
+
+
+def conv_multi(items) -> None:
+    items = list(items)
+    if not 1 <= len(items) <= _lib.MAX_MULTI:
+        raise _lib.StgError(f"conv_multi: {len(items)} items (1..{_lib.MAX_MULTI})")
+    parts = [_conv_item(**kw) for kw in items]
+    m = _lib.StgConvMulti(n=len(parts))
+    for i, part in enumerate(parts):
+        m.item[i] = part[0]
+    lib = _lib.load()
+    if profile is None and flop_log is None:
+        check(lib.stg_conv_multi(C.byref(m), _stream()), "stg_conv_multi")
+        return
+    routes = {lib.stg_conv_route(C.byref(part[0])) for part in parts}
+    route = _ROUTES[routes.pop()]
+    rec = dict(kind=("dgrad" if m.item[0].transposed else "fwd"), engine=route, flops=sum(part[1] for part in parts),
+               bytes=sum(part[2] for part in parts), shape=tuple(part[3] for part in parts))
+    if flop_log is not None:
+        flop_log.append(rec)
+    if profile is None:
+        check(lib.stg_conv_multi(C.byref(m), _stream()), "stg_conv_multi")
+        return
+    e0, e1 = torch.cuda.Event(enable_timing=True), torch.cuda.Event(enable_timing=True)
+    e0.record()
+    check(lib.stg_conv_multi(C.byref(m), _stream()), "stg_conv_multi")
+    e1.record()
+    rec["ingest"] = _ingest(lib)
+    profile.append(dict(rec, events=(e0, e1), desc=m, fn="stg_conv_multi", args=(), keep=[part[4] for part in parts]))
 
 
 def _ingest(lib) -> float:
diff --git a/ste_gan_b200/passes.py b/ste_gan_b200/passes.py
--- a/ste_gan_b200/passes.py
+++ b/ste_gan_b200/passes.py
@@ -237,21 +237,29 @@
 def _fwd(f: Folded, src: Tensor, B: int, t_src: int, *, phases: int = 1, act: int = ACT_NONE, want_raw: bool = False,
          want_act: bool = False, dup: bool = False, add_post: Optional[Tensor] = None, post_shift: int = 0,
          out_f32: bool = False, lengths: Optional[Tensor] = None, rate: int = 1) -> Tuple[Optional[Tensor], Optional[Tensor], int]:
+    kw, y_raw, y_act, t_dst = _fwd_args(f, src, B, t_src, phases=phases, act=act, want_raw=want_raw, want_act=want_act,
+                                        dup=dup, add_post=add_post, post_shift=post_shift, out_f32=out_f32)
+    ops.conv(**kw, valid_units=lengths, rows_per_unit=rate)
+    return y_raw, y_act, t_dst
+
+
+def _fwd_args(f: Folded, src: Tensor, B: int, t_src: int, *, phases: int = 1, act: int = ACT_NONE, want_raw: bool = False,
+              want_act: bool = False, dup: bool = False, add_post: Optional[Tensor] = None, post_shift: int = 0,
+              out_f32: bool = False) -> Tuple[dict, Optional[Tensor], Optional[Tensor], int]:
     m = f.mod
     t_dst = m.t_out(t_src)
     odt = torch.float32 if out_f32 else f.dtype
     y_raw = torch.empty((B, t_dst * phases, m.out_channels), device=src.device, dtype=odt) if want_raw else None
     y_act = torch.empty((B, t_dst * phases * (2 if dup else 1), m.out_channels), device=src.device, dtype=odt) if want_act else None
     if f.unfold:
-        ops.conv(src, f.wf, n_samples=B, phases=phases, t_src=t_dst, t_dst=t_dst, c_src=f.kp, c_dst=m.out_channels, k=1,
-                 bias=m.bias.data, act=act, dup_rows=dup, add_post=add_post, post_shift=post_shift, y_raw=y_raw, y_act=y_act,
-                 valid_units=lengths, rows_per_unit=rate)
+        kw = dict(src=src, w=f.wf, n_samples=B, phases=phases, t_src=t_dst, t_dst=t_dst, c_src=f.kp, c_dst=m.out_channels, k=1,
+                  bias=m.bias.data, act=act, dup_rows=dup, add_post=add_post, post_shift=post_shift, y_raw=y_raw, y_act=y_act)
     else:
-        ops.conv(src, f.wf, n_samples=B, phases=phases, t_src=t_src, t_dst=t_dst, c_src=m.in_channels, c_dst=m.out_channels,
-                 groups=f.pg, k=m.kernel, dilation=m.dilation, stride=m.stride, pad=m.pad, bias=m.bias.data, act=act,
-                 dup_rows=dup, add_post=add_post, post_shift=post_shift, y_raw=y_raw, y_act=y_act, acct_groups=m.groups,
-                 valid_units=lengths, rows_per_unit=rate)
-    return y_raw, y_act, t_dst
+        kw = dict(src=src, w=f.wf, n_samples=B, phases=phases, t_src=t_src, t_dst=t_dst, c_src=m.in_channels,
+                  c_dst=m.out_channels, groups=f.pg, k=m.kernel, dilation=m.dilation, stride=m.stride, pad=m.pad,
+                  bias=m.bias.data, act=act, dup_rows=dup, add_post=add_post, post_shift=post_shift, y_raw=y_raw, y_act=y_act,
+                  acct_groups=m.groups)
+    return kw, y_raw, y_act, t_dst
 
 
 def _dgrad(f: Folded, dy: Tensor, B: int, t_dy: int, t_x: int, *, phases: int = 1, mask: Optional[Tensor] = None,
@@ -268,14 +276,24 @@
         ops.unfold_bwd(du, dx, n_samples=B, phases=phases, t_src=t_x, t_dst=t_dy, channels=m.in_channels, k=m.kernel,
                        dilation=m.dilation, stride=m.stride, pad=m.pad)
         return dx if out_f32 else ops.cast(dx, f.dtype)
+    kw, dx = _dgrad_args(f, dy, B, t_dy, t_x, phases=phases, mask=mask, mask_mode=mask_mode, add_pre=add_pre,
+                         add_post=add_post, pair_sum=pair_sum, out_f32=out_f32)
+    ops.conv(**kw)
+    return dx
+
+
+def _dgrad_args(f: Folded, dy: Tensor, B: int, t_dy: int, t_x: int, *, phases: int = 1, mask: Optional[Tensor] = None,
+                mask_mode: int = ACT_NONE, add_pre: Optional[Tensor] = None, add_post: Optional[Tensor] = None,
+                pair_sum: bool = False, out_f32: bool = False) -> Tuple[dict, Tensor]:
+    m = f.mod
     rows = t_x // 2 if pair_sum else t_x
     dx = torch.empty((B, rows * phases, m.in_channels), device=dy.device, dtype=torch.float32 if out_f32 else f.dtype)
     fwd_pack = f.dtype == torch.bfloat16 and not (m.groups > 1 and f.wd is not None)
-    ops.conv(dy, f.wf if fwd_pack else f.wd, n_samples=B, phases=phases, t_src=t_dy, t_dst=t_x, c_src=m.out_channels,
-             c_dst=m.in_channels, groups=f.pg, k=m.kernel, dilation=m.dilation, stride=m.stride, pad=m.pad, transposed=True,
-             pair_sum=pair_sum, mask=mask, mask_mode=mask_mode, add_pre=add_pre, add_post=add_post, y_raw=dx,
-             w_fwd_pack=fwd_pack, acct_groups=m.groups)
-    return dx
+    kw = dict(src=dy, w=f.wf if fwd_pack else f.wd, n_samples=B, phases=phases, t_src=t_dy, t_dst=t_x, c_src=m.out_channels,
+              c_dst=m.in_channels, groups=f.pg, k=m.kernel, dilation=m.dilation, stride=m.stride, pad=m.pad, transposed=True,
+              pair_sum=pair_sum, mask=mask, mask_mode=mask_mode, add_pre=add_pre, add_post=add_post, y_raw=dx,
+              w_fwd_pack=fwd_pack, acct_groups=m.groups)
+    return kw, dx
 
 
 def _wgrad(f: Folded, x: Tensor, dy: Tensor, B: int, t_x: int, t_dy: int, ws: _Workspace, phases: int = 1) -> None:
@@ -581,6 +599,11 @@
     return heavy, [i for i in range(len(subs)) if i not in heavy]
 
 
+def _units(subs: Sequence, idx: Sequence[int]) -> List[List[int]]:
+    per = [i for i in idx if subs[i][0] == "P"]
+    return ([per] if per else []) + [[i] for i in idx if subs[i][0] != "P"]
+
+
 def discriminator_forward(model, x: Tensor, dtype: torch.dtype, folds: Dict[int, Folded], side=None,
                           subset: Optional[Sequence[int]] = None, spread: Optional[Sequence] = None):
     x = x.contiguous().float()
@@ -598,55 +621,82 @@
     results: List = [None] * len(subs)
     sub_ctx: List = [None] * len(subs)
 
-    def run(idx: List[int]) -> None:
+    def run_periods(idx: List[int]) -> None:
+        h, t, fmaps, sub = {}, {}, {}, {}
         for i in idx:
-            kind, d = subs[i]
-            fused0 = False
-            if kind == "P":
-                p = d.period
-                t_pad = T + (p - T % p)
-                phases, t = p, t_pad // p
-                l0, f0_ = d.layers[0], folds[id(d.layers[0])]
-                fused0 = (f0_.unfold and dtype == torch.bfloat16 and l0.groups == 1 and l0.dilation == 1 and
-                          l0.out_channels % 8 == 0 and t_pad - T < T)
-                src = None if fused0 else ops.reflect_pad_right(x, t_pad, dtype)
+            d = subs[i][1]
+            p = d.period
+            t_pad = T + (p - T % p)
+            l0, f0 = d.layers[0], folds[id(d.layers[0])]
+            fused0 = (f0.unfold and dtype == torch.bfloat16 and l0.groups == 1 and l0.dilation == 1 and
+                      l0.out_channels % 8 == 0 and t_pad - T < T)
+            t[i] = t_pad // p
+            src = None if fused0 else ops.reflect_pad_right(x, t_pad, dtype)
+            if f0.unfold and not fused0:
+                src = unfold_input(f0, src, B, t[i], p)
+            sub[i] = dict(kind="P", phases=p, inputs=[src], ts=[t[i]], t_in0=T, mod=d)
+            fmaps[i] = []
+            h[i] = src
+            if fused0:
+                h[i], t[i] = ops.period_first_layer(x, f0.wf, l0.bias.data, period=p, c_out=l0.out_channels, k=l0.kernel,
+                                                    stride=l0.stride, pad=l0.pad, slope=0.1)
+                fmaps[i].append(h[i]); sub[i]["inputs"].append(h[i]); sub[i]["ts"].append(t[i])
+                sub[i]["x0"] = x
+        n_layers = len(subs[idx[0]][1].layers) + 1
+        assert len({len(sub[i]["ts"]) for i in idx}) == 1
+        for j in range(len(sub[idx[0]]["ts"]) - 1, n_layers):
+            last = j == n_layers - 1
+            kws = []
+            for i in idx:
+                d = subs[i][1]
+                f = folds[id(d.output if last else d.layers[j])]
+                kw, y_raw, y_act, t[i] = _fwd_args(f, h[i], B, t[i], phases=sub[i]["phases"], act=ACT_NONE if last else ACT_LEAKY,
+                                                   want_raw=last, want_act=not last, out_f32=last)
+                kws.append(kw)
+                h[i] = y_raw if last else y_act
+                fmaps[i].append(h[i]); sub[i]["ts"].append(t[i])
+                if not last:
+                    sub[i]["inputs"].append(h[i])
+            ops.conv_multi(kws)
+        for i in idx:
+            results[i], sub_ctx[i] = fmaps[i], sub[i]
+
+    def run_scale(i: int) -> None:
+        d = subs[i][1]
+        src = ops.cast(scale_in[i], dtype)
+        phases, t = 1, scale_in[i].shape[1]
+        f0 = folds[id(d.layers[0])]
+        if f0.unfold:
+            src = unfold_input(f0, src, B, t, phases)
+        sub = dict(kind="S", phases=phases, inputs=[src], ts=[t], t_in0=scale_in[i].shape[1], mod=d)
+        fmaps = []
+        h = src
+        for layer in d.layers:
+            _, h, t = _fwd(folds[id(layer)], h, B, t, phases=phases, act=ACT_LEAKY, want_act=True)
+            fmaps.append(h); sub["inputs"].append(h); sub["ts"].append(t)
+        logits, _, t = _fwd(folds[id(d.output)], h, B, t, phases=phases, want_raw=True, out_f32=True)
+        sub["ts"].append(t)
+        fmaps.append(logits)
+        sub["x_scale"] = scale_in[i]
+        results[i], sub_ctx[i] = fmaps, sub
+
+    def run(units: List[List[int]]) -> None:
+        for u in units:
+            if subs[u[0]][0] == "P":
+                run_periods(u)
             else:
-                src = ops.cast(scale_in[i], dtype)
-                phases, t = 1, scale_in[i].shape[1]
-            f0 = folds[id(d.layers[0])]
-            if f0.unfold and not fused0:
-                src = unfold_input(f0, src, B, t, phases)
-            sub = dict(kind=kind, phases=phases, inputs=[src], ts=[t], t_in0=scale_in[i].shape[1] if kind == "S" else T, mod=d)
-            fmaps = []
-            h = src
-            layers = list(d.layers)
-            if fused0:
-                l0 = layers[0]
-                h, t = ops.period_first_layer(x, f0.wf, l0.bias.data, period=phases, c_out=l0.out_channels, k=l0.kernel,
-                                              stride=l0.stride, pad=l0.pad, slope=0.1)
-                fmaps.append(h); sub["inputs"].append(h); sub["ts"].append(t)
-                sub["x0"] = x
-                layers = layers[1:]
-            for layer in layers:
-                _, h, t = _fwd(folds[id(layer)], h, B, t, phases=phases, act=ACT_LEAKY, want_act=True)
-                fmaps.append(h); sub["inputs"].append(h); sub["ts"].append(t)
-            logits, _, t = _fwd(folds[id(d.output)], h, B, t, phases=phases, want_raw=True, out_f32=True)
-            sub["ts"].append(t)
-            fmaps.append(logits)
-            if kind == "S":
-                sub["x_scale"] = scale_in[i]
-            results[i], sub_ctx[i] = fmaps, sub
+                run_scale(u[0])
 
     heavy, rest = _heavy_split(subs)
     heavy, rest = [i for i in heavy if i in wanted], [i for i in rest if i in wanted]
+    units = _units(subs, heavy) + _units(subs, rest)
     if spread:
-        todo = heavy + rest
-        lanes = [todo[j::len(spread) + 1] for j in range(len(spread) + 1)]
-        fork_many(list(spread), [(lambda idx=idx: run(idx)) for idx in lanes if idx])
+        lanes = [units[j::len(spread) + 1] for j in range(len(spread) + 1)]
+        fork_many(list(spread), [(lambda u=u: run(u)) for u in lanes if u])
     elif side is not None and heavy and rest:
-        fork_join(side, lambda: run(heavy), lambda: run(rest))
+        fork_join(side, lambda: run(_units(subs, heavy)), lambda: run(_units(subs, rest)))
     else:
-        run(heavy + rest)
+        run(units)
     ctx.subs = sub_ctx
     ctx.keep = (scale_in, xs)
     return results, ctx
@@ -691,51 +741,85 @@
     n_sub = len(ctx.subs)
     scale_grad: List = [None] * n_sub
 
-    def run(idx: List[int]) -> None:
-        for di in idx:
-            sub = ctx.subs[di]
-            if sub is None:
-                continue
-            d, phases, inputs, ts = sub["mod"], sub["phases"], sub["inputs"], sub["ts"]
-            convs = list(d.layers) + [d.output]
-            g = dlogits[di]
-            fm_g = dfmaps[di] if dfmaps is not None else None
-            if g is None and (fm_g is None or all(t is None for t in fm_g)):
-                continue
-            if g is None:
-                g = torch.zeros((B, ts[-1] * phases, 1), device=dev, dtype=dtype)
-            dxin = None
-            for j in reversed(range(len(convs))):
+    def start(di: int):
+        sub = ctx.subs[di]
+        if sub is None:
+            return None
+        g = dlogits[di]
+        fm_g = dfmaps[di] if dfmaps is not None else None
+        if g is None and (fm_g is None or all(t is None for t in fm_g)):
+            return None
+        if g is None:
+            g = torch.zeros((B, sub["ts"][-1] * sub["phases"], 1), device=dev, dtype=dtype)
+        return list(sub["mod"].layers) + [sub["mod"].output], g, fm_g
+
+    def run_scale(di: int) -> None:
+        st = start(di)
+        if st is None:
+            return
+        convs, g, fm_g = st
+        sub = ctx.subs[di]
+        phases, inputs, ts = sub["phases"], sub["inputs"], sub["ts"]
+        for j in reversed(range(len(convs))):
+            f = folds[id(convs[j])]
+            if want_weight_grad:
+                _wgrad(f, inputs[j], g, B, ts[j], ts[j + 1], ws, phases=phases)
+            if j == 0:
+                if want_input_grad:
+                    scale_grad[di] = _dgrad(f, g, B, ts[1], ts[0], phases=phases, out_f32=True)
+                break
+            g = _dgrad(f, g, B, ts[j + 1], ts[j], phases=phases, mask=inputs[j], mask_mode=ACT_LEAKY,
+                       add_pre=fm_g[j - 1] if fm_g is not None else None)
+
+    def run_periods(idx: List[int]) -> None:
+        todo = [(di, st) for di, st in ((di, start(di)) for di in idx) if st is not None]
+        if not todo:
+            return
+        g = {di: st[1] for di, st in todo}
+        for j in reversed(range(len(todo[0][1][0]))):
+            kws, outs = [], {}
+            for di, (convs, _, fm_g) in todo:
+                sub = ctx.subs[di]
+                phases, inputs, ts = sub["phases"], sub["inputs"], sub["ts"]
                 f = folds[id(convs[j])]
                 if want_weight_grad:
                     xin = inputs[j] if inputs[j] is not None else first_layer_input(sub, f, B, dtype)
-                    _wgrad(f, xin, g, B, ts[j], ts[j + 1], ws, phases=phases)
+                    _wgrad(f, xin, g[di], B, ts[j], ts[j + 1], ws, phases=phases)
                 if j == 0:
                     if want_input_grad:
-                        dxin = _dgrad(f, g, B, ts[1], ts[0], phases=phases, out_f32=True)
-                    break
-                g = _dgrad(f, g, B, ts[j + 1], ts[j], phases=phases, mask=inputs[j], mask_mode=ACT_LEAKY,
-                           add_pre=fm_g[j - 1] if fm_g is not None else None)
-            if want_input_grad:
-                if sub["kind"] == "P":
-                    ops.reflect_pad_right_bwd(dxin, T, dx)
-                else:
-                    scale_grad[di] = dxin
-
-    heavy, rest = _heavy_split([(sub["kind"] if sub is not None else "-", None) for sub in ctx.subs])
+                        ops.reflect_pad_right_bwd(_dgrad(f, g[di], B, ts[1], ts[0], phases=phases, out_f32=True), T, dx)
+                    continue
+                kw, outs[di] = _dgrad_args(f, g[di], B, ts[j + 1], ts[j], phases=phases, mask=inputs[j], mask_mode=ACT_LEAKY,
+                                           add_pre=fm_g[j - 1] if fm_g is not None else None)
+                kws.append(kw)
+            if kws:
+                ops.conv_multi(kws)
+                g.update(outs)
+
+    def run(units: List[List[int]]) -> None:
+        for u in units:
+            if ctx.subs[u[0]]["kind"] == "P":
+                run_periods(u)
+            else:
+                run_scale(u[0])
+
+    kinds = [(sub["kind"] if sub is not None else "-", None) for sub in ctx.subs]
+    present = [i for i in range(n_sub) if ctx.subs[i] is not None]
+    heavy, rest = _heavy_split(kinds)
+    heavy, rest = [i for i in heavy if i in present], [i for i in rest if i in present]
     if spread and (plan is not None or not want_weight_grad):
-        h_here = [i for i in heavy if ctx.subs[i] is not None] if side is not None else []
-        todo = [i for i in range(n_sub) if ctx.subs[i] is not None and i not in h_here]
+        h_here = heavy if side is not None else []
+        todo = _units(kinds, [i for i in present if i not in h_here])
         lanes = [l for l in (todo[j::len(spread) + 1] for j in range(len(spread) + 1)) if l]
-        fns = [(lambda idx=idx: run(idx)) for idx in lanes] or [lambda: None]
+        fns = [(lambda u=u: run(u)) for u in lanes] or [lambda: None]
         streams = list(spread)[:len(fns) - 1]
         if h_here:
-            fns.append(lambda: run(h_here)); streams.append(side)
+            fns.append(lambda: run(_units(kinds, h_here))); streams.append(side)
         fork_many(streams, fns)
-    elif side is not None and heavy and any(ctx.subs[i] is not None for i in rest):
-        fork_join(side, lambda: run(heavy), lambda: run(rest))
+    elif side is not None and heavy and rest:
+        fork_join(side, lambda: run(_units(kinds, heavy)), lambda: run(_units(kinds, rest)))
     else:
-        run(list(range(n_sub)))
+        run(_units(kinds, present))
     if want_input_grad:
         carry = None
         for di in reversed([i for i, sub in enumerate(ctx.subs) if sub is not None and sub["kind"] == "S"]):
diff --git a/ste_gan_b200/trainer.py b/ste_gan_b200/trainer.py
--- a/ste_gan_b200/trainer.py
+++ b/ste_gan_b200/trainer.py
@@ -106,8 +106,7 @@
         self.x_pred: Optional[Tensor] = None
         self._side = torch.cuda.Stream(device=dev)
         self._side2 = [torch.cuda.Stream(device=dev), torch.cuda.Stream(device=dev)]
-        self._wg = [torch.cuda.Stream(device=dev) for _ in range(7)]
-        self._ps = [torch.cuda.Stream(device=dev) for _ in range(2)]
+        self._wg = [torch.cuda.Stream(device=dev) for _ in range(5)]
         self._ss = [torch.cuda.Stream(device=dev)]
         self._sn = [torch.cuda.Stream(device=dev) for _ in range(4)]
         self._aux = torch.cuda.Stream(device=dev)
@@ -253,7 +252,7 @@
             return
         _, heavy, p_idx, s_idx = self._split_subs()
         fwd = lambda x, idx: passes.discriminator_forward(self.net_d, x, dt, self._f1, subset=idx,
-                                                          spread=self._ps if idx is p_idx else (self._ss if idx is s_idx else None)) if idx else (None, None)
+                                                          spread=self._ss if idx is s_idx else None) if idx else (None, None)
         x_cat = torch.cat([self.x_pred, self._x_real], 0)
         ((rs, cs), (rp, cp)), (rh, ch) = passes.fork_join(
             self._s2(1), lambda: passes.fork_join(self._s2(0), lambda: fwd(x_cat, p_idx), lambda: fwd(x_cat, s_idx))[::-1],
@@ -298,10 +297,10 @@
         dl_b = [dcat.get(i) for i in range(nd)]
         self.d_plan.zero()
         cur = torch.cuda.current_stream()
-        self.d_plan.async_wgrads({st.cuda_stream: w for st, w in zip((cur, self._side, self._side2[0], self._side2[1], *self._ps, *self._ss), self._wg)})
+        self.d_plan.async_wgrads({st.cuda_stream: w for st, w in zip((cur, self._side, self._side2[0], self._side2[1], *self._ss), self._wg)})
         bwd = lambda ctx, dlog: passes.discriminator_backward(self.net_d, ctx, dlog, None, want_input_grad=False,
                                                               want_weight_grad=True, plan=self.d_plan,
-                                                              spread=self._ps if ctx is cp else (self._ss if ctx is cs else None)) if ctx is not None else None
+                                                              spread=self._ss if ctx is cs else None) if ctx is not None else None
         only = lambda dlog, idx: [dlog[i] if i in idx else None for i in range(nd)]
         self._fork()
         with torch.cuda.stream(self._side):
@@ -309,7 +308,7 @@
         passes.fork_join(self._s2(1), lambda: bwd(cs, only(dl_b, s_idx)), lambda: bwd(cp, only(dl_b, p_idx)))
         early = []
         if self._inline and heavy and self._d_slices is not None:
-            self.d_plan.join_wgrads_of([cur, self._side2[1], *self._ps, *self._ss])
+            self.d_plan.join_wgrads_of([cur, self._side2[1], *self._ss])
             for (i_lo, i_hi), (g_lo, g_hi) in self._d_slices["early"]:
                 self.d_plan.backward_range(i_lo, i_hi, accumulate=False)
                 early.append(self._reduce(self.D.grad[g_lo:g_hi]))
@@ -405,7 +404,7 @@
                 f3 = self._fold_d(refold_d)
                 x_cat = torch.cat([x_pred, x_real], 0)
                 fwd = lambda x, f, idx: passes.discriminator_forward(self.net_d, x, dt, f, subset=idx,
-                                                                     spread=self._ps if idx is p_idx else (self._ss if idx is s_idx else None)) if idx else (None, None)
+                                                                     spread=self._ss if idx is s_idx else None) if idx else (None, None)
                 self._fork()
                 with torch.cuda.stream(self._side):
                     (rs, cs), (rh_f, ch_f) = passes.fork_join(self._s2(0), lambda: fwd(x_cat, f3, s_idx), lambda: fwd(x_pred, f3, heavy))
@@ -441,7 +440,7 @@
             else:
                 dfm = [[None] * (len(fm_f) - 1) for fm_f in res_f]
             dx_d = passes.discriminator_backward(self.net_d, ctx_f, dlog, dfm, want_input_grad=True, want_weight_grad=False,
-                                                 side=self._s2(0), spread=self._ps if self.concurrent_d else None)
+                                                 side=self._s2(0), spread=self._ss if self.concurrent_d else None)
             if td_ev is not None:
                 torch.cuda.current_stream().wait_event(td_ev)
             ops.axpy_f32(dx_pred, dx_d, 1.0)
```
